# ictnlp/StreamSpeech

Measured on AMD Instinct MI355X. Metric: real-time factor (RTFx = audio seconds / wall seconds) + utterances/sec, offline S2ST fr-en, higher is better.
Workload: dtype f32

## Files before the change

include/streamspeech_hip.h:

```cpp
#ifndef STREAMSPEECH_HIP_H
#define STREAMSPEECH_HIP_H

#include <stddef.h>
#include <stdint.h>

#ifdef __cplusplus
extern "C" {
#endif

#define SS_ABI_VERSION 2

typedef struct ss_model ss_model;
typedef struct ss_vocoder ss_vocoder;
typedef struct ss_scratch ss_scratch;
typedef struct ss_stream_pool ss_stream_pool;

typedef struct ss_config {
  int32_t input_feat, conv_channels, conv_kernel;
  int32_t enc_dim, enc_ffn, enc_heads, enc_layers, dw_kernel;
  int32_t src_vocab, tgt_vocab;
  int32_t mt_layers, dec_dim, dec_ffn, dec_heads;
  int32_t t2u_layers, unit_layers, unit_vocab, ctc_upsample;
  int32_t pad, eos, unk;
  int32_t max_rel_pos;
// ... 106 lines not shown
  int32_t history;
  int32_t dst;
  int32_t pad0;
} ss_mp3_stream_seg;

int ss_mp3_stream_synthesize(void* stream, const int16_t* d_q, const ss_mp3_granule* d_rec, int64_t n_rec,
                             const ss_mp3_stream_seg* h_segs, int n_segs, float* const* h_state, float* const* h_dst,
                             const int64_t* h_dst_cap, int n_dst, int mono, void* d_work, size_t* work_bytes);

typedef struct ss_flac_info {
  int32_t sample_rate, channels, bits_per_sample;
  int32_t frames;
  int64_t subframes;
  int64_t samples;
  int64_t total_samples;
  int32_t min_block, max_block;
  uint8_t md5[16];
} ss_flac_info;

enum { SS_FLAC_CONSTANT = 0, SS_FLAC_VERBATIM = 1, SS_FLAC_FIXED = 2, SS_FLAC_LPC = 3 };
enum { SS_FLAC_INDEPENDENT = 0, SS_FLAC_LEFT_SIDE = 1, SS_FLAC_RIGHT_SIDE = 2, SS_FLAC_MID_SIDE = 3 };

typedef struct ss_flac_subframe {
  int64_t res_offset;
  int64_t sample_start;
  int32_t block_size;
  uint8_t type;
  uint8_t order;
  uint8_t bps;
  uint8_t wasted;
  uint8_t shift;
  uint8_t assignment;
  uint8_t precision;
  uint8_t channel;
  int32_t reserved;
  int16_t coef[32];
} ss_flac_subframe;

typedef struct ss_flac_file {
  int64_t rec_offset;
  int64_t out_offset;
  int32_t frames;
  int32_t channels;
  int32_t bps;
  int32_t n_out;
} ss_flac_file;

int ss_flac_streaminfo(const uint8_t* h_data, size_t n_bytes, ss_flac_info* h_info);
int ss_flac_probe(const uint8_t* h_data, size_t n_bytes, ss_flac_info* h_info);
int ss_flac_unpack(const uint8_t* h_data, size_t n_bytes, int64_t cap, int32_t* h_res, ss_flac_subframe* h_rec, int64_t res_cap,
                   ss_flac_info* h_info);
int ss_flac_restore_host(const int32_t* h_res, const ss_flac_subframe* h_rec, int64_t n_rec, const ss_flac_file* h_files, int n_files,
                         int mono, float* h_out, int32_t* h_pcm);
int ss_flac_restore(void* stream, const int32_t* d_res, const ss_flac_subframe* d_rec, int64_t n_rec, int64_t n_res,
                    const ss_flac_file* h_files, int n_files, int mono, float* d_out, int64_t out_floats,
                    void* d_work, size_t* work_bytes);

enum { SS_PCM_F32LE = 0, SS_PCM_S16LE = 1, SS_PCM_ULAW = 2, SS_PCM_ALAW = 3 };

typedef struct ss_pcm_seg {
  int64_t src_offset;
  int64_t dst_offset;
  int32_t frames;
  int32_t fmt, channels, dst;
} ss_pcm_seg;

int ss_pcm_scatter(void* stream, const void* d_stage, int64_t stage_bytes, const ss_pcm_seg* h_segs, int n_segs,
                   float* const* h_dst, const int64_t* h_dst_cap, int n_dst);
int ss_pcm_pack_s16(void* stream, const float* d_src, int64_t n, int16_t* d_out);
int ss_pcm_decode_host(const void* h_src, int fmt, int channels, int64_t frames, float* h_dst);
int ss_pcm_pack_s16_host(const float* h_src, int64_t n, int16_t* h_out);

typedef struct ss_pcm_emit_seg {
  float* carry;
  const float* tail;
  const float* taps;
  int64_t n_before;
  int64_t k0, k1;
  int64_t out_offset;
  int32_t carry_len;
  int32_t n_new;
  int32_t up, down, half;
  int32_t fmt;
  int32_t finished;
  int32_t reserved;
} ss_pcm_emit_seg;

int64_t ss_pcm_emit_count(int64_t n, int up, int down, int half, int finished);
int ss_pcm_emit(void* stream, const ss_pcm_emit_seg* h_segs, int n_segs, void* d_out, int64_t out_bytes);
int ss_pcm_emit_host(const ss_pcm_emit_seg* h_segs, int n_segs, void* h_out, int64_t out_bytes);
int ss_pcm_encode_host(const float* h_src, int64_t n, int fmt, void* h_out);

enum { SS_VAD_IDLE = 0, SS_VAD_SPEECH = 1 };
enum { SS_VAD_START = 1, SS_VAD_END = 2, SS_VAD_FORCED = 4 };

typedef struct ss_vad_state {
  int64_t onset;
  int64_t last_speech;
  int64_t utt_first_frame;
  float floor;
  int32_t mode;
  int32_t run;
  int32_t reserved;
} ss_vad_state;

typedef struct ss_vad_seg {
  const float* hist;
  ss_vad_state* state;
  float* powers;
  int64_t hist_first;
  int64_t n_hist;
  int64_t first_frame;
  int32_t n_frames;
  int32_t H, W;
  float p_abs, p_min, snr, rise;
  int32_t min_speech, end_silence, post_roll, max_frames;
  int32_t reserved;
} ss_vad_seg;

typedef struct ss_vad_result {
  int64_t consumed;
  int64_t start_frame;
  int64_t cut_sample;
  int64_t last_speech;
  int32_t events;
  int32_t mode;
} ss_vad_result;

int ss_vad_scan(void* stream, const ss_vad_seg* h_segs, int n_segs, ss_vad_result* d_results);
int ss_vad_scan_host(const ss_vad_seg* h_segs, int n_segs, ss_vad_result* h_results);

int ss_row_max_logprob(void* stream, const float* d_logits, int rows, int vocab, int mask0, int mask1, int mask2,
                       float* d_out);

int ss_log_softmax(void* stream, const float* d_logits, int rows, int vocab, int mask0, int mask1, int as_probs,
                   float* d_out);

int ss_encoder_out_len(int T);
int ss_encoder_forward(ss_model* m, void* stream, const float* d_fbank, int T, int attn_chunk,
                       int conv_chunk, float* d_enc_out);

int ss_encoder_stream_reset(ss_model* m);
int ss_encoder_stream_set_tail(ss_model* m, int unsettled_fbank_frames);
int ss_encoder_stream_forward(ss_model* m, void* stream, const float* d_fbank, int T, int attn_chunk,
                              int conv_chunk, float* d_enc_out, int32_t* n_final, int32_t* n_computed);
int ss_encoder_stream_set_deferred(ss_model* m, int on);
int ss_encoder_stream_status(ss_model* m, void* stream, int32_t* repeat);

int ss_stream_pool_create(ss_model* m, int max_sessions, int max_rows, ss_stream_pool** out);
void ss_stream_pool_destroy(ss_stream_pool* p);
int ss_stream_pool_reset(ss_stream_pool* p, int slot);
int ss_stream_pool_set_tail(ss_stream_pool* p, int slot, int unsettled_fbank_frames);
int ss_encoder_stream_forward_batch(ss_model* m, void* stream, ss_stream_pool* p, int n, const int32_t* h_slots,
                                    const float* const* h_fbank, const int32_t* h_T, const int32_t* h_attn_chunk,
                                    const int32_t* h_conv_chunk, float* d_enc_packed, int32_t* h_n_final, int32_t* h_n_computed);
int ss_stream_pool_ctc(ss_model* m, void* stream, ss_stream_pool* p, int head, int n, const int32_t* h_slots,
                       const float* d_enc_packed, int32_t* d_raw, int32_t* d_tokens, int32_t* d_index, int32_t* d_counts);
int ss_stream_pool_stats(ss_stream_pool* p, int64_t* launches, int64_t* head_rows);

int ss_ctc_greedy(ss_model* m, void* stream, int head, const float* d_enc_out, int Tp,
                  int32_t* d_raw, int32_t* d_tokens, int32_t* d_index, int32_t* d_count,
                  float* d_logits);

int ss_mt_set_persistent(ss_model* m, int workgroups);
int ss_mt_get_persistent(ss_model* m);

int ss_mt_begin(ss_model* m, void* stream, const float* d_enc_out, int Tp);
int ss_mt_append(ss_model* m, void* stream, const int32_t* d_tokens, int n, int pos0, int ban_eos,
                 int force_eos, float* d_feats, int32_t* d_next, int n_tail_pad);
int ss_mt_greedy(ss_model* m, void* stream, const float* d_enc_out, int Tp, const int32_t* h_prefix,
                 int n_prefix, int max_len, int min_len, int32_t* h_out_tokens, int* h_n_out,
                 float* d_feats, int* h_n_feats);
int ss_mt_truncate(ss_model* m, int len);

int ss_t2u_units(ss_model* m, void* stream, const float* d_mt_feats, int n, int t2u_causal,
                 int mask_eos, int32_t* d_raw, int32_t* d_tokens, int32_t* d_count, float* d_logits,
                 int n_tail_pad);

int ss_vocoder_create(const ss_vocoder_config* cfg, const float* d_blob, size_t blob_floats,
                      const char* const* names, const int64_t* offsets, const int64_t* numels,
                      int n_slots, ss_vocoder** out);
void ss_vocoder_destroy(ss_vocoder* v);
int ss_vocoder_set_bf16x3(ss_vocoder* v, int on);
int ss_vocoder_set_f16(ss_vocoder* v, int on);
int ss_vocoder_forward(ss_vocoder* v, void* stream, const int32_t* d_codes, int K, int dur_prediction,
                       const int32_t* d_forced_dur, float* d_wav, int64_t wav_capacity,
                       int32_t* d_dur, int64_t* h_n_samples);
int ss_vocoder_num_speakers(const ss_vocoder* v);
int ss_vocoder_forward_spkr(ss_vocoder* v, void* stream, const int32_t* d_codes, int K, int dur_prediction,
                            const int32_t* d_forced_dur, float* d_wav, int64_t wav_capacity,
                            int32_t* d_dur, int64_t* h_n_samples, int32_t spkr);

int ss_batch_fbank_cmvn(ss_model* m, void* stream, int B, const float* d_pcm, const int64_t* h_pcm_start,
                        const int32_t* h_n_samples, float pcm_scale, float* d_feat, int32_t* h_T);
int ss_batch_cmvn(ss_model* m, void* stream, const float* d_in, int64_t rows, float* d_out);
int ss_batch_encoder_forward(ss_model* m, void* stream, int B, const float* d_fbank, const int32_t* h_T,
                             int attn_chunk, int conv_chunk, float* d_enc_out, int32_t* h_Tp);
int ss_batch_ctc_greedy(ss_model* m, void* stream, int head, int B, const float* d_enc_out,
                        const int32_t* h_Tp, int32_t* d_raw, int32_t* d_tokens, int32_t* d_index,
                        int32_t* d_counts);
int ss_batch_mt_greedy(ss_model* m, void* stream, int B, const float* d_enc_out, const int32_t* h_Tp,
                       const int32_t* h_max_len, int min_len, int32_t* h_out_tokens, int out_stride,
                       int32_t* h_n_out, float* d_feats, int feat_rows);
int ss_batch_mt_beam(ss_model* m, void* stream, int B, int beam, const float* d_enc_out, const int32_t* h_Tp,
                     const int32_t* h_max_len, int min_len, float unk_penalty, int normalize, int32_t* h_out_tokens,
                     int out_stride, int32_t* h_n_out, float* h_scores, float* h_pos_scores, float* d_feats, int feat_rows);
int ss_batch_mt_continue(ss_model* m, void* stream, int B, const float* d_enc_out, const int32_t* h_Tp, const int32_t* h_prefix,
                         const int32_t* h_n_prefix, const int32_t* h_max_len, int min_len, int32_t* h_out_tokens, int out_stride,
                         int32_t* h_n_out, float* d_feats, int feat_rows, int32_t* h_n_feats);
int ss_batch_mt_continue_plan(int B, const int32_t* h_Tp, const int32_t* h_prefix, const int32_t* h_n_prefix, const int32_t* h_max_len,
                              int min_len, int out_stride, int feat_rows, int max_tgt_pos, int vocab, int eos, int32_t* h_dims,
                              int32_t* h_tables, int64_t tables_cap, int64_t* h_n_tables);
int ss_batch_mt_beam_continue(ss_model* m, void* stream, int B, int beam, const float* d_enc_out, const int32_t* h_Tp,
                              const int32_t* h_prefix, const int32_t* h_n_prefix, const int32_t* h_max_len, int min_len,
                              float unk_penalty, int normalize, int32_t* h_out_tokens, int out_stride, int32_t* h_n_out,
                              float* h_scores, float* h_pos_scores, float* d_feats, int feat_rows);
int ss_batch_mt_beam_continue_plan(int B, int beam, const int32_t* h_Tp, const int32_t* h_prefix, const int32_t* h_n_prefix,
                                   const int32_t* h_max_len, int min_len, int out_stride, int feat_rows, int max_tgt_pos, int vocab,
                                   int eos, int pad, int32_t* h_dims, int32_t* h_tables, int64_t tables_cap, int64_t* h_n_tables);
int ss_batch_fbank_frames(ss_model* m, void* stream, int B, const float* const* h_pcm, const int32_t* h_first, const int32_t* h_n,
                          float pcm_scale, float* const* h_feat);
int ss_batch_fbank_frames_sr(ss_model* m, void* stream, int B, const float* const* h_pcm, const int32_t* h_n_in, const int32_t* h_up,
                             const int32_t* h_down, const float* const* h_taps, const int32_t* h_half_len, const int32_t* h_first,
                             const int32_t* h_n, float pcm_scale, float* const* h_feat);
int ss_fbank_sr_rows(int64_t n_in, int up, int down, int half_len, int32_t* h_n_rows, int32_t* h_n_final);
int ss_batch_t2u_units(ss_model* m, void* stream, int B, const float* d_feats, int feat_rows,
                       const int32_t* h_n, int t2u_causal, int mask_eos, int32_t* d_raw, int32_t* d_tokens,
                       int32_t* d_counts);
int ss_batch_vocoder_forward(ss_vocoder* v, void* stream, int B, const int32_t* d_codes, const int32_t* h_K,
                             int dur_prediction, const int32_t* d_forced_dur, float* d_wav,
                             int64_t wav_capacity, int32_t* d_dur, int64_t* h_wav_start,
                             int64_t* h_n_samples);
int ss_batch_vocoder_forward_spkr(ss_vocoder* v, void* stream, int B, const int32_t* d_codes, const int32_t* h_K,
                                  int dur_prediction, const int32_t* d_forced_dur, float* d_wav,
                                  int64_t wav_capacity, int32_t* d_dur, int64_t* h_wav_start,
                                  int64_t* h_n_samples, const int32_t* h_spkr );
int ss_batch_t2u_units_pad(ss_model* m, void* stream, int B, const float* d_feats, int feat_rows, const int32_t* h_n,
                           const int32_t* h_n_tail_pad, int t2u_causal, int mask_eos, int32_t* d_raw, int32_t* d_tokens,
                           int32_t* d_counts);
int ss_batch_mt_features(ss_model* m, void* stream, int B, const float* d_enc_out, const int32_t* h_Tp, const int32_t* h_tokens,
                         const int32_t* h_n_tokens, const int32_t* h_n_tail_pad, float* d_feats, int feat_rows);
int ss_batch_vocoder_tail(ss_vocoder* v, void* stream, int B, const int32_t* d_codes, const int32_t* h_K, const int32_t* h_n_new,
                          const int32_t* h_ctx, const int32_t* h_rf, int dur_prediction, float* d_out, int64_t out_capacity,
                          int32_t* h_win_first, int32_t* h_dur, int64_t* h_out_start, int64_t* h_n_out);
int ss_batch_vocoder_tail_spkr(ss_vocoder* v, void* stream, int B, const int32_t* d_codes, const int32_t* h_K, const int32_t* h_n_new,
                               const int32_t* h_ctx, const int32_t* h_rf, int dur_prediction, float* d_out, int64_t out_capacity,
                               int32_t* h_win_first, int32_t* h_dur, int64_t* h_out_start, int64_t* h_n_out,
                               const int32_t* h_spkr );

int ss_prof_enable(int cls_mask);
int ss_prof_enable_hi(int cls_mask);
int ss_prof_reset(void);
int ss_prof_read(int cls, double* h_ms_total, double* h_flops_total, int64_t* h_launches,
                 double* h_bytes_total);
int ss_prof_totals(int cls, double* h_flops_total, double* h_bytes_total, int64_t* h_launches);
int ss_prof_read_issued(int cls, double* h_issued_flops_total);
int ss_prof_shape_log(int on);
int ss_prof_shape_dump(char* buf, int cap);
int ss_prof_num_classes(void);
const char* ss_prof_class_name(int cls);

int ss_model_set_pack_invariant(ss_model* m, int on);
int ss_model_get_pack_invariant(ss_model* m);
int ss_debug_canon(int mode);

int ss_debug_last_logits(ss_model* m, void* stream, float* d_out, int64_t cap_floats, int* h_rows, int* h_cols);

int ss_op_ffn_fused(void* stream, const float* dX, int ldx, float* dY, int ldy, const float* ln_g, const float* ln_b,
                    const float* dW1, const float* db1, const float* dW2, const float* db2, float alpha,
                    const float* ln2_g, const float* ln2_b, int M, int D, int F);
int ss_debug_ffn(int grid, int row_tiles_per_wave, int enable);
int ss_debug_rtlin(int grid, int enable);
int ss_debug_conv_c64(int enable);
int ss_debug_conv_c32(int enable);
int ss_debug_conv_c16(int enable);
int64_t ss_debug_enc_step_launches(void);
int ss_op_ln_linear(void* stream, const float* dX, int ldx, const float* ln_g, const float* ln_b, const float* dW,
                    const float* dbias, const float* dR, int ldr, float* dC, int ldc, int M, int N, int K, int act, float alpha,
                    int glu);

int ss_debug_force_tile(int bm, int bn, int ks);
int ss_debug_sk_errors(void);
int ss_debug_attention_split(int v);
int ss_debug_attention_q16(int v);
int ss_debug_enc_step_inject_timeout(ss_model* m);
int ss_debug_scratch_audit(ss_scratch* sc, size_t* booked, size_t* held);
int ss_debug_mt_inject_timeout(ss_model* m);

int ss_op_conv_gemm(void* stream, const float* dA, int lda, const float* dW, const float* dbias,
                    const float* dR, int ldr, const float* dR2, int ldr2, float* dC, int ldc,
                    int M, int N, int Cin, int taps, int dil, int stride, int pad, int in_len,
                    int chunk, int in_act, float in_slope, int act, float alpha, float div, int glu);
typedef struct ss_op_conv_args {
  const float* A; const float* W; const float* bias; const float* R; const float* R2; float* C; float* C2;
  int32_t lda, ldc, ldr, ldr2, ldc2;
  int32_t M, N, Cin, taps, dil, stride, pad, in_len, chunk;
  int32_t in_act; float in_slope;
  int32_t act; float act_slope, alpha, div, c2_slope;
  int32_t glu;
  const int32_t* segs; int32_t nseg, max_seg_out;
  int32_t same_rows;
} ss_op_conv_args;
int ss_op_conv_gemm_ex(void* stream, const ss_op_conv_args* a);
int ss_op_conv_pair(void* stream, const float* dA, int lda, const float* dW1, const float* db1, const float* dW2, const float* db2,
                    float* dC, int ldc, const float* dR2, int ldr2, float div, float* dC2, int ldc2, float c2_slope, int C, int taps,
                    int dil, int M, int in_len, float slope, const int32_t* d_segs, int nseg);
int ss_op_resblock_fused(void* stream, const float* dX, int ldx, const float* const* dW1, const float* const* dB1,
                         const float* const* dW2, const float* const* dB2, const int32_t* dil, float* dY, int ldy, const float* dR2,
                         int ldr2, float div, int C, int taps, int M, float slope, const int32_t* d_segs, int nseg);
int ss_debug_slab(int grid, long long min_rows);
int ss_op_conv_f16(void* stream, const float* dA, const float* dW, const float* dbias, const float* dR, const float* dR2,
                   float* dC, float* dC2, int M, int C, int taps, int dil, int in_act, float in_slope, int act, float div,
                   const int32_t* d_segs, int nseg);
int ss_op_layernorm(void* stream, const float* dx, int ldx, float* dy, int ldy, const float* dg,
                    const float* db, int M, int D, float eps);
int ss_op_attention(void* stream, const float* dQ, int ldq, const float* dK, int ldk, const float* dV,
                    int ldv, float* dO, int ldo, int Tq, int Tk, int H, float scale, int causal,
                    int chunk, const float* dP, int ldp, const float* du, const float* dv);
typedef struct ss_op_attn_args {
  const float* Q; const float* K; const float* V; float* O;
  int32_t ldq, ldk, ldv, ldo;
  int32_t Tq, Tk, H;
  float scale;
  int32_t causal, chunk, q0, k_mask_tail;
  const float* P; int32_t ldp;
  const float* bias_u; const float* bias_v;
  const int32_t* segs; int32_t nseg, max_q, p_tmax;
  const int32_t* seg_tail;
  int32_t no_decode_kernel;
  const int32_t* anc; int32_t anc_ld, anc_slots;
  int32_t use_split;
} ss_op_attn_args;
int ss_op_attention_ex(void* stream, const ss_op_attn_args* a);
typedef struct ss_op_pool_attn_args {
  const float* Qs; float* cache; float* O;
  int32_t ld, ldo, slot_rows;
  const float* P; int32_t ldp, p_tmax;
  const float* bias_u; const float* bias_v;
  const int32_t* sess; const int32_t* qt_pre;
  int32_t nsess, qtiles, H;
  float scale;
} ss_op_pool_attn_args;
int ss_op_attention_pool(void* stream, const ss_op_pool_attn_args* a);
int ss_debug_attention_no_mfma(int v);
int ss_op_dwconv_bn_silu(void* stream, const float* dx, int ldx, float* dy, int ldy, const float* dwt,
                         int K, const float* mean, const float* var, const float* gamma,
                         const float* beta, float eps, int T, int C, int chunk);

int ss_op_masked_argmax(void* stream, const float* logits, int ld, int M, int N, int mask0, int mask1, int mask2, int force,
                        int32_t* ids, const int32_t* row_max_len, int step, int force_id, const int32_t* row_min_len, int ban_id);
int ss_op_ctc_collapse(void* stream, const int32_t* raw, int T, int blank, int pad, int32_t* tokens, int32_t* index, int32_t* count,
                       const int32_t* segs, int nseg);
int ss_op_dur_predict(void* stream, const float* logdur, const int32_t* forced, int K, int32_t* dur, int32_t* cum,
                      const int32_t* segs, int nseg);
int ss_op_repeat_rows(void* stream, const float* emb, const int32_t* cum, int K, int D, float* out, int F, const int32_t* segs,
                      int nseg);
int ss_op_embed_tokens(void* stream, const int32_t* tok, const float* emb, const float* pos_table, float scale, int pos0, float* out,
                       int n, int D, int pos_stride, int pad_id, int vocab);
int ss_op_embed_tokens_rows(void* stream, const int32_t* tok, const float* emb, const float* pos_table, int pos_rows, float scale,
                            int pos0, const int32_t* row_pos, float* out, int n, int D, int pad_id, int vocab);
int ss_op_upsample_add_pos(void* stream, const float* src, int n, int up, const float* pos_row, float pad_value, float* out, int D);
int ss_op_gather_rows(void* stream, const int32_t* idx, const float* table, int D, float* out, int n, int rows);
int ss_op_scatter_rows(void* stream, const int32_t* dst_row, const float* src, int lds, float* dst, int ldd, int D, int n,
                       int dst_rows);
int ss_op_conv_post_tanh(void* stream, const float* x, int T, int C, const float* w, const float* bias, float slope, float* wav,
                         const int32_t* segs, int nseg);
int ss_op_conv_post_tanh_crop(void* stream, const float* x, int C, const float* w, const float* bias, float slope, float* wav,
                              const int32_t* segs, int nseg, int max_keep);
int ss_op_spkr_pre_add(void* stream, const float* x, float* y, int ld, int C0, const float* table, const int32_t* spkr, int spkr0,
                       const int32_t* segs, int nseg, int max_seg_out, int M, int act, float slope);

#define SS_OP_BEAM_CAND 64
int ss_op_beam_topk(void* stream, const float* logits, int R, int V, int k, int t_step, int min_len, const int32_t* max_len,
                    const int32_t* npre, const int32_t* done, const float* cum, int pad, int unk, int eos, float unk_pen,
                    float* cand_s, int32_t* cand_t);
typedef struct ss_op_beam_state {
  int32_t* tok; float* cum; int32_t* anc; float* cand_s; int32_t* cand_t; int32_t* ignore; int32_t* done; int32_t* max_len;
  int32_t* npre;
  int32_t* fin_cnt; float* fin_score; int32_t* fin_len; int32_t* fin_tok; float* fin_pos; int32_t* fin_anc;
} ss_op_beam_state;
int ss_op_beam_merge(void* stream, const ss_op_beam_state* st, int B, int k, int Lc, int V, int t_step, int c0, int eos,
                     int normalize);
int ss_op_beam_prefix_score(void* stream, const float* logits, int rows, int V, const int32_t* ftok, int pad, int unk, float unk_pen,
                            float* lp);
int ss_op_beam_prefix_chain(void* stream, const float* lp, const int32_t* row0, const int32_t* npre, int B, int k, float* cum0,
                            float* pos);

#ifdef __cplusplus
}
#endif
#endif
```

streamspeech_amd/csrc/conv_c64w.hip:

```cpp
#include "slab_common.hpp"

#include <type_traits>

namespace ss {

using u32x4 = __attribute__((ext_vector_type(4))) unsigned;

#ifndef CW_TIMING
#define CW_TIMING 0
#endif
#if CW_TIMING
__device__ unsigned long long g_cw_dbg[1024 * 8];
#define CW_STAMP(k) do { if (t == 0) { const unsigned long long _n = __builtin_amdgcn_s_memtime(); cw_acc[k] += _n - cw_last; cw_last = _n; } } while (0)
#else
#define CW_STAMP(k) do { } while (0)
#endif

namespace {
constexpr int CW_MAXSEG = 256;
constexpr int CW_MAXROWS = 320;
[[maybe_unused]] constexpr int CW_NUM_RECORDS = 0x7ffffff0;
constexpr int cw_bme(int dil) { return dil == 1 ? 256 : dil == 3 ? 252 : 240; }
[[maybe_unused]] __host__ __device__ constexpr int cw_nc(int kind) { return kind == 0 ? 4 : kind == 1 ? 2 : 3; }
[[maybe_unused]] __host__ __device__ constexpr int cw_slot(int kind, int n) { return kind == 0 ? n : kind == 1 ? (n == 0 ? 0 : 3) : (n == 2 ? 3 : n); }
[[maybe_unused]] __host__ __device__ constexpr int cw_ja(int kind, int n) { return kind == 0 ? (n == 3 ? 1 : n) : kind == 1 ? n : (n == 0 ? 0 : 1); }
[[maybe_unused]] __host__ __device__ constexpr int cw_jb(int kind, int n) { return kind == 0 ? (n == 2 ? 1 : n == 3 ? 3 : 2) : kind == 1 ? n : (n == 2 ? 2 : 1); }
[[maybe_unused]] __host__ __device__ constexpr int cw_op(int kind, int n) { return kind == 0 ? (n == 1 ? 1 : -1) : kind == 1 ? 0 : (n == 1 ? 0 : -1); }
}

__global__ void wino_pack_kernel(const float* __restrict__ W, float* __restrict__ WW, int C, int taps, int groups) {
  const int n = C * groups * C;
  for (int idx = blockIdx.x * blockDim.x + threadIdx.x; idx < n; idx += gridDim.x * blockDim.x) {
    const int ci = idx % C, g = (idx / C) % groups, co = idx / (C * groups);
    const float* w = W + (size_t)co * taps * C + ci;
    const float w0 = 3 * g < taps ? w[(size_t)(3 * g) * C] : 0.f;
    const float w1 = 3 * g + 1 < taps ? w[(size_t)(3 * g + 1) * C] : 0.f;
    const float w2 = 3 * g + 2 < taps ? w[(size_t)(3 * g + 2) * C] : 0.f;
    float* o = WW + (size_t)co * groups * 4 * C + (size_t)g * 4 * C + ci;
    const int left = taps - 3 * g;
    if (left >= 3) {
      o[0] = w0;
      o[C] = 0.5f * ((w0 + w1) + w2);
      o[2 * C] = 0.5f * ((w0 - w1) + w2);
      o[3 * C] = w2;
    } else if (left == 2) {
      o[0] = w0; o[C] = w0 + w1; o[2 * C] = 0.f; o[3 * C] = w1;
    } else {
      o[0] = w0; o[C] = 0.f; o[2 * C] = 0.f; o[3 * C] = -w0;
    }
  }
}

template <int DIL, int CH, int TAIL>
__global__ __launch_bounds__(CH >= 128 ? 512 : 256, CH >= 128 ? 1 : CH == 64 ? 2 : 3) void conv_c64w_kernel(const GemmArgs p, const int groups, const int slab_rows) {
#if __HIP_DEVICE_COMPILE__
  constexpr int CS = CH == 256 ? 128 : CH;
  constexpr int KH = CH / CS;
  constexpr int C = CH, LDA = CS + 4, CT = CH >= 64 ? 4 : CH / 16, CB = CS / 16, RING = 2 * CT, TPR = CS / 4;
  constexpr int NT = CH >= 128 ? 512 : 256, RPP = NT / TPR;
  constexpr int NP = (CW_MAXROWS + RPP - 1) / RPP, NPC = CH == 256 ? 10 : NP < 20 ? NP : 20, BME = cw_bme(DIL), NPAIR = BME / 2;
  extern __shared__ __attribute__((aligned(16))) float smem[];
  float* sA = smem;
  int* s_blk = reinterpret_cast<int*>(smem + ((slab_rows * LDA + 3) & ~3));

  const int t = threadIdx.x, lane = t & 63;
  const int wave = __builtin_amdgcn_readfirstlane((t >> 6) & 3);
  const int cs = CH <= 64 ? 0 : __builtin_amdgcn_readfirstlane(t >> 8);
  const int colh = CH == 256 ? (int)((blockIdx.x >> 3) & 1) : 0;
  const int col0 = colh * 128 + cs * 64;
  const int r = lane & 15, g = lane >> 4;
  const int Kw = groups * 4 * C;

  SlabWalk<GemmArgs> w(p, s_blk, BME);
  __syncthreads();
  const int nblocks = w.nblocks();
  const float slope = p.in_act == ACT_LRELU ? p.in_slope : 1.0f;

  const __amdgpu_buffer_rsrc_t rsW = __builtin_amdgcn_make_buffer_rsrc((void*)p.W, 0, CW_NUM_RECORDS, 0x00020000);
  const int vo = (r * Kw + 4 * g) * 4;
  auto wload = [&](int idx, int cc, int ct, int kh) -> f32x4 {
    const int so = __builtin_amdgcn_readfirstlane(((col0 + ct * 16) * Kw + idx * C + kh * CS + cc * 16) * 4);
    const u32x4 v = __builtin_amdgcn_raw_buffer_load_b128(rsW, vo, so, 0);
    return f32x4{__uint_as_float(v[0]), __uint_as_float(v[1]), __uint_as_float(v[2]), __uint_as_float(v[3])};
  };

  int blk = CH == 256 ? (int)((blockIdx.x & 7) + 8 * (blockIdx.x >> 4)) : (int)blockIdx.x;
  const int blk_stride = CH == 256 ? (int)(gridDim.x >> 1) : (int)gridDim.x;
  if (blk >= nblocks) return;
  f32x4 ring[RING];
#pragma unroll
  for (int q = 0; q < RING; ++q) ring[q] = wload(q / CT, 0, q % CT, 0);

  int toff[2];
  bool pv[2];
#pragma unroll
  for (int i = 0; i < 2; ++i) {
    const int pp = wave * 32 + i * 16 + r;
    pv[i] = pp < NPAIR;
    const int pc = pv[i] ? pp : NPAIR - 1;
    toff[i] = 2 * DIL * (pc / DIL) + pc % DIL;
  }

#if CW_TIMING
  unsigned long long cw_acc[4] = {0, 0, 0, 0}, cw_last = __builtin_amdgcn_s_memtime(), cw_begin = cw_last, cw_blocks = 0;
#endif
  for (; blk < nblocks; blk += blk_stride) {
#if CW_TIMING
    ++cw_blocks;
#endif
    w.locate(blk, p.in_len);
    const int m0 = w.m0, seg_lo = w.seg_lo, seg_hi = w.seg_hi;
    const int m_hi = p.nseg > 0 ? seg_hi : min(seg_hi, p.M);
    const bool edge = (m0 - p.pad < seg_lo) || (m0 - p.pad + slab_rows > seg_hi);
    f32x4 acc[4][2][CT];
#pragma unroll
    for (int f = 0; f < 4; ++f)
#pragma unroll
      for (int i = 0; i < 2; ++i)
#pragma unroll
        for (int j = 0; j < CT; ++j) acc[f][i][j] = f32x4{0.f, 0.f, 0.f, 0.f};
#pragma unroll 1
    for (int kh = 0; kh < KH; ++kh) {
    const int kh_wrap = kh + 1 < KH ? kh + 1 : 0;
    __syncthreads();
    CW_STAMP(kh == 0 ? 3 : 1);
#pragma unroll 1
    for (int u0 = 0; u0 < NP; u0 += NPC) {
      f32x4 pre[NPC];
#pragma unroll
      for (int u = 0; u < NPC; ++u) {
        const int rho = t / TPR + RPP * (u0 + u);
        const int gc = min(max(m0 - p.pad + rho, seg_lo), seg_hi - 1);
        pre[u] = *reinterpret_cast<const f32x4*>(p.A + (size_t)gc * p.lda + kh * CS + (t % TPR) * 4);
      }
      float* dst = sA + (t / TPR + RPP * u0) * LDA + (t % TPR) * 4;
#pragma unroll
      for (int u = 0; u < NPC; ++u) {
        const int rho = t / TPR + RPP * (u0 + u);
        f32x4 v = pre[u];
        if (edge) {
          const int gin = m0 - p.pad + rho;
          const bool ok = gin >= seg_lo && gin < seg_hi;
#pragma unroll
          for (int e = 0; e < 4; ++e) v[e] = ok ? v[e] : 0.f;
        }
#pragma unroll
        for (int e = 0; e < 4; ++e) v[e] = fmaxf(v[e], v[e] * slope);
        if (rho < slab_rows) *reinterpret_cast<f32x4*>(dst + u * RPP * LDA) = v;
      }
    }
    __syncthreads();
    CW_STAMP(0);

    const float* pa0 = sA + toff[0] * LDA + 4 * g;
    const float* pa1 = sA + toff[1] * LDA + 4 * g;
    auto rd = [&](const float* base, int j, int cc) -> f32x4 { return *reinterpret_cast<const f32x4*>(base + j * DIL * LDA + cc * 16); };
    auto xform = [&](int op, const f32x4 a, const f32x4 b) -> f32x4 { return op == 1 ? a + b : op == 0 ? a : a - b; };
    f32x4 xa[2];
    xa[0] = xform(-1, rd(pa0, 0, 0), rd(pa0, 2, 0));
    xa[1] = xform(-1, rd(pa1, 0, 0), rd(pa1, 2, 0));
    auto group = [&](auto KIND, const int grp, const int kind_next, const float* pn0, const float* pn1, const int grp_next, const int kh_next) __attribute__((always_inline)) {
      constexpr int K = decltype(KIND)::value, NC = cw_nc(K), NS = CB * NC;
      static_assert(NS % 2 == 0 && NS >= 2, "ring slots keep their parity across groups");
#pragma unroll
      for (int ss = 0; ss < NS; ++ss) {
        const int slot = cw_slot(K, ss % NC);
        f32x4 na0, nb0, na1, nb1;
        if (ss + 1 < NS) {
          const int ccn = (ss + 1) / NC, nn = (ss + 1) % NC;
          na0 = rd(pa0, cw_ja(K, nn), ccn); nb0 = rd(pa0, cw_jb(K, nn), ccn);
          na1 = rd(pa1, cw_ja(K, nn), ccn); nb1 = rd(pa1, cw_jb(K, nn), ccn);
        } else {
          const int jb = kind_next == 0 ? 2 : 1;
          na0 = rd(pn0, 0, 0); nb0 = *reinterpret_cast<const f32x4*>(pn0 + jb * (DIL * LDA));
          na1 = rd(pn1, 0, 0); nb1 = *reinterpret_cast<const f32x4*>(pn1 + jb * (DIL * LDA));
        }
        f32x4 wf[CT];
#pragma unroll
        for (int j = 0; j < CT; ++j) {
          const int q = ss * CT + j;
          wf[j] = ring[q % RING];
          const int s2 = ss + 2;
          if (s2 < NS) ring[q % RING] = wload(grp * 4 + cw_slot(K, s2 % NC), s2 / NC, j, kh);
          else ring[q % RING] = wload(grp_next * 4 + (s2 == NS ? 0 : (kind_next == 1 ? 3 : 1)), 0, j, kh_next);
        }
#pragma unroll
        for (int e = 0; e < 4; ++e)
#pragma unroll
          for (int i = 0; i < 2; ++i)
#pragma unroll
            for (int j = 0; j < CT; ++j)
              acc[slot][i][j] = __builtin_amdgcn_mfma_f32_16x16x4f32(wf[j][e], xa[i][e], acc[slot][i][j], 0, 0, 0);
        if (ss + 1 < NS) {
          xa[0] = xform(cw_op(K, (ss + 1) % NC), na0, nb0);
          xa[1] = xform(cw_op(K, (ss + 1) % NC), na1, nb1);
        } else {
          xa[0] = kind_next == 1 ? na0 : na0 - nb0;
          xa[1] = kind_next == 1 ? na1 : na1 - nb1;
        }
        __builtin_amdgcn_sched_barrier(0);
      }
    };
    constexpr int tail = TAIL;
    const int groups_full = groups - (tail ? 1 : 0);
#pragma unroll 1
    for (int grp = 0; grp < groups_full; ++grp) {
      const bool more = grp + 1 < groups;
      const float* pn0 = more ? pa0 + 3 * DIL * LDA : pa0;
      const float* pn1 = more ? pa1 + 3 * DIL * LDA : pa1;
      group(std::integral_constant<int, 0>{}, grp, (more && grp + 1 == groups_full) ? tail : 0, pn0, pn1, more ? grp + 1 : 0, more ? kh : kh_wrap);
      pa0 = pn0;
      pa1 = pn1;
    }
    if constexpr (TAIL == 1) group(std::integral_constant<int, 1>{}, groups_full, 0, pa0, pa1, 0, kh_wrap);
    if constexpr (TAIL == 2) group(std::integral_constant<int, 2>{}, groups_full, 0, pa0, pa1, 0, kh_wrap);
    CW_STAMP(1);
    }

    int le = lane;
    asm volatile("" : "+v"(le));
    const int g_e = le >> 4;
    const int cole = col0 + g_e * 4;
    f32x4 y[4 * CT];
    int mrow[4];
#pragma unroll
    for (int i = 0; i < 2; ++i) {
#pragma unroll
      for (int j = 0; j < CT; ++j) {
        y[(i * 2) * CT + j] = (acc[0][i][j] + acc[1][i][j]) + acc[2][i][j];
        y[(i * 2 + 1) * CT + j] = (acc[1][i][j] - acc[2][i][j]) - acc[3][i][j];
      }
      mrow[i * 2] = m0 + toff[i];
      mrow[i * 2 + 1] = m0 + toff[i] + DIL;
    }
#pragma unroll
    for (int n = 0; n < 4 * CT; ++n) asm volatile("" : "+v"(y[n]));
    f32x4 bb[CT];
#pragma unroll
    for (int j = 0; j < CT; ++j) bb[j] = f32x4{0.f, 0.f, 0.f, 0.f};
    if (p.bias) {
#pragma unroll
      for (int j = 0; j < CT; ++j) bb[j] = *reinterpret_cast<const f32x4*>(p.bias + cole + j * 16);
    }
    slab_epi_batch(p, y, bb, [&](int q, int n) -> size_t {
      return (size_t)min(mrow[n / CT], m_hi - 1) * (q == 0 ? p.ldr : p.ldr2) + cole + (n % CT) * 16;
    });
#pragma unroll
    for (int q = 0; q < 4; ++q) {
      if (pv[q / 2] && mrow[q] < m_hi) {
#pragma unroll
        for (int j = 0; j < CT; ++j) slab_epi_store<CH >= 128>(p, mrow[q], cole + j * 16, y[q * CT + j]);
      }
    }
    CW_STAMP(2);
  }
#if CW_TIMING
  if (t == 0) {
    unsigned long long* d = g_cw_dbg + (size_t)(blockIdx.x & 1023) * 8;
    d[0] = cw_acc[0]; d[1] = cw_acc[1]; d[2] = cw_acc[2]; d[3] = cw_acc[3]; d[4] = cw_blocks; d[5] = cw_begin; d[6] = __builtin_amdgcn_s_memtime(); d[7] = 1;
  }
#endif
#endif
}

#if CW_TIMING
extern "C" int ss_debug_cw_timing(unsigned long long* h_out, int cap_wgs) {
  const int n = cap_wgs < 1024 ? cap_wgs : 1024;
  if (hipMemcpyFromSymbol(h_out, HIP_SYMBOL(g_cw_dbg), (size_t)n * 8 * sizeof(unsigned long long)) != hipSuccess) return -1;
  static unsigned long long zeros[1024 * 8];
  (void)hipMemcpyToSymbol(HIP_SYMBOL(g_cw_dbg), zeros, sizeof(zeros));
  return n;
}
#endif

void conv_c64w_debug(int enable) { if (enable >= 0) dispatch_edit([enable](Dispatch& d) { d.c64w_on = enable ? 1 : 0; }); }
bool conv_c64w_enabled() { return disp().c64w_on != 0; }
void conv_c128w_debug(int enable) { if (enable >= 0) dispatch_edit([enable](Dispatch& d) { d.c128w_on = enable ? 1 : 0; }); }
bool conv_c128w_enabled() { return disp().c128w_on != 0; }

void conv_c256w_debug(int enable) { if (enable >= 0) dispatch_edit([enable](Dispatch& d) { d.c256w_on = enable ? 1 : 0; }); }
bool conv_c256w_enabled() { return disp().c256w_on != 0; }

static int cw_groups(const GemmArgs& a) { return (a.taps + 2) / 3; }
static size_t cw_lds(const GemmArgs& a, int ch) { return slab_lds_bytes(cw_bme(a.dil) + 3 * cw_groups(a) * a.dil, ch + 4, CW_MAXSEG); }

bool conv_c64w_eligible(const GemmArgs& a) {
  if (!disp().c64w_on || !a.Wwino || a.taps < disp().c64w_min_k || a.taps < 3 || (a.dil != 1 && a.dil != 3 && a.dil != 5) || a.C2) return false;
  if (a.pad != a.dil * (a.taps - 1) / 2) return false;
  if (a.taps <= 8 && a.taps > 3 && a.dil == 5) return false;
  const int slab_rows = cw_bme(a.dil) + 3 * cw_groups(a) * a.dil;
  return slab_rows <= CW_MAXROWS && 2 * cw_lds(a, 64) <= 158 * 1024 && (size_t)cw_groups(a) * 4 * 64 * 64 * 4 < 0x7ff00000ull;
}

bool conv_wide_winograd_eligible(const GemmArgs& a, int ch) {
  if (ch != 128 && ch != 256) return false;
  const Dispatch& d = disp();
  if (!(ch == 128 ? d.c128w_on : d.c256w_on) || !a.Wwino || !slab_conv_ok(a, ch)) return false;
  if (a.taps < 3 || (a.dil != 1 && a.dil != 3 && a.dil != 5) || a.pad != a.dil * (a.taps - 1) / 2) return false;
  if (a.nseg > CW_MAXSEG || a.M < (ch == 128 ? d.c128w_min_rows : d.c256w_min_rows) || !slab_rows_ok(a.M)) return false;
  if (ch == 256 && (size_t)256 * cw_groups(a) * 4 * 256 * 4 >= 0x7ff00000ull) return false;
  const int slab_rows = cw_bme(a.dil) + 3 * cw_groups(a) * a.dil;
  return slab_rows <= CW_MAXROWS && cw_lds(a, 128) <= 160 * 1024;
}

int launch_wino_pack(const float* W, float* WW, int C, int taps, hipStream_t stream) {
  const int groups = (taps + 2) / 3, n = C * groups * C;
  hipLaunchKernelGGL(wino_pack_kernel, dim3((n + 255) / 256), dim3(256), 0, stream, W, WW, C, taps, groups);
  SS_LAUNCH_CHECK();
  return SS_OK;
}

template <int DIL, int CH, int TAIL>
static int launch_cw_t(GemmArgs a, hipStream_t stream) {
  constexpr int BME = cw_bme(DIL);
  const int groups = cw_groups(a);
  const int slab_rows = BME + 3 * groups * DIL;
  const size_t lds = cw_lds(a, CH == 256 ? 128 : CH);
  SS_MAX_LDS_ONCE((&conv_c64w_kernel<DIL, CH, TAIL>), CH >= 128 ? 160 * 1024 : 96 * 1024);
  SkWorkspace* st = nullptr;
  int rc = sk_workspace_acquire(stream, &st);
  if (rc != SS_OK) return rc;
  int grid = slab_grid(CH >= 128 ? 1 : CH == 64 ? 2 : 3, st->cus, a.M, BME, a.nseg);
  if (CH == 256) {
    long long want = std::min<long long>(st->cus, 2 * ((slab_max_blocks(a.M, BME, a.nseg) + 7) / 8 * 8));
    if (disp().slab_grid_cap > 0) want = std::min<long long>(want, disp().slab_grid_cap);
    grid = (int)std::max<long long>(16, want / 16 * 16);
  }
  ProfRec rec{}; bool prof = false;
  rc = prof_begin(a, stream, CH == 64 ? PROF_CONV_C64W : CH == 128 ? PROF_CONV_C128W : CH == 256 ? PROF_CONV_C256W : PROF_CONV_C32W, rec, prof);
  if (rc != SS_OK) return rc;
  a.W = a.Wwino;
  hipLaunchKernelGGL((conv_c64w_kernel<DIL, CH, TAIL>), dim3(grid), dim3(CH >= 128 ? 512 : 256), lds, stream, a, groups, slab_rows);
  SS_LAUNCH_CHECK();
  return prof_end(stream, rec, prof);
}

template <int CH>
static int launch_cw(const GemmArgs& a, hipStream_t stream) {
  if (a.in_act != ACT_NONE && a.in_act != ACT_LRELU) return SS_ERR_ARG;
  const int key = a.dil * 10 + a.taps % 3;
  switch (key) {
    case 10: return launch_cw_t<1, CH, 0>(a, stream);
    case 11: return launch_cw_t<1, CH, 1>(a, stream);
    case 12: return launch_cw_t<1, CH, 2>(a, stream);
    case 30: return launch_cw_t<3, CH, 0>(a, stream);
    case 31: return launch_cw_t<3, CH, 1>(a, stream);
    case 32: return launch_cw_t<3, CH, 2>(a, stream);
    case 50: return launch_cw_t<5, CH, 0>(a, stream);
    case 51: return launch_cw_t<5, CH, 1>(a, stream);
    case 52: return launch_cw_t<5, CH, 2>(a, stream);
    default: return SS_ERR_ARG;
  }
}

int launch_conv_c64w(const GemmArgs& a, hipStream_t stream) {
  if (!conv_c64_eligible(a) || !conv_c64w_eligible(a)) return SS_ERR_ARG;
  return launch_cw<64>(a, stream);
}
void conv_c32w_debug(int enable) { if (enable >= 0) dispatch_edit([enable](Dispatch& d) { d.c32w_on = enable ? 1 : 0; }); }
bool conv_c32w_enabled() { return disp().c32w_on != 0; }
bool conv_c32w_eligible(const GemmArgs& a) {
  if (!disp().c32w_on || !a.Wwino || a.taps < 3 || (a.dil != 1 && a.dil != 3 && a.dil != 5) || a.C2) return false;
  if (a.pad != a.dil * (a.taps - 1) / 2) return false;
  const int slab_rows = cw_bme(a.dil) + 3 * cw_groups(a) * a.dil;
  return slab_rows <= CW_MAXROWS && 3 * cw_lds(a, 32) <= 158 * 1024;
}
int launch_conv_c32w(const GemmArgs& a, hipStream_t stream) {
  if (!conv_c32_eligible(a) || !conv_c32w_eligible(a)) return SS_ERR_ARG;
  return launch_cw<32>(a, stream);
}
int launch_conv_c128w(const GemmArgs& a, hipStream_t stream) {
  if (!conv_wide_winograd_eligible(a, 128)) return SS_ERR_ARG;
  return launch_cw<128>(a, stream);
}
int launch_conv_c256w(const GemmArgs& a, hipStream_t stream) {
  if (!conv_wide_winograd_eligible(a, 256)) return SS_ERR_ARG;
  return launch_cw<256>(a, stream);
}

}
```

streamspeech_amd/csrc/debug_ops.hip:

```cpp
#include "model_internal.hpp"

static int op_bind_wino(GemmArgs& a, void* stream) {
  static thread_local std::map<hipStream_t, DevBuf> wino_tmps;
  DevBuf& wino_tmp = wino_tmps[(hipStream_t)stream];
  const int N = a.N, Cin = a.Cin, taps = a.taps;
  if ((conv_c64w_enabled() && N == 64 && Cin == 64 && taps >= 3 && conv_c64_eligible(a)) ||
      (conv_c128w_enabled() && N == 128 && Cin == 128 && taps >= 3 && a.same_rows && !a.glu) ||
      (conv_c256w_enabled() && N == 256 && Cin == 256 && taps >= 3 && a.same_rows && !a.glu) ||
      (conv_c32w_enabled() && N == 32 && Cin == 32 && taps >= 3 && conv_c32_eligible(a))) {
    RET(wino_tmp.ensure((size_t)N * ((taps + 2) / 3) * 4 * N * sizeof(float)));
    RET(launch_wino_pack(a.W, wino_tmp.f(), N, taps, (hipStream_t)stream));
    a.Wwino = wino_tmp.f();
  }
  return SS_OK;
}

extern "C" int ss_op_conv_gemm(void* stream, const float* dA, int lda, const float* dW, const float* dbias,
                               const float* dR, int ldr, const float* dR2, int ldr2, float* dC, int ldc, int M,
                               int N, int Cin, int taps, int dil, int stride, int pad, int in_len, int chunk,
                               int in_act, float in_slope, int act, float alpha, float div, int glu) {
  GemmArgs a;
  a.A = dA; a.lda = lda; a.W = dW; a.bias = dbias; a.R = dR; a.ldr = ldr; a.R2 = dR2; a.ldr2 = ldr2; a.C = dC; a.ldc = ldc;
  a.M = M; a.N = N; a.Cin = Cin; a.taps = taps; a.dil = dil; a.stride = stride; a.pad = pad; a.in_len = in_len;
  a.chunk = chunk; a.in_act = in_act; a.in_slope = in_slope; a.act = act; a.alpha = alpha; a.div = div; a.glu = glu;
  a.same_rows = (stride == 1 && M == in_len) ? 1 : 0;
  RET(op_bind_wino(a, stream));
  return launch_conv_gemm(a, (hipStream_t)stream);
}

extern "C" int ss_op_conv_gemm_ex(void* stream, const ss_op_conv_args* x) {
  if (!x) return SS_ERR_ARG;
  GemmArgs a;
  a.A = x->A; a.W = x->W; a.bias = x->bias; a.R = x->R; a.R2 = x->R2; a.C = x->C; a.C2 = x->C2;
  a.lda = x->lda; a.ldc = x->ldc; a.ldr = x->ldr; a.ldr2 = x->ldr2; a.ldc2 = x->ldc2;
  a.M = x->M; a.N = x->N; a.Cin = x->Cin; a.taps = x->taps; a.dil = x->dil; a.stride = x->stride; a.pad = x->pad;
  a.in_len = x->in_len; a.chunk = x->chunk;
  a.in_act = x->in_act; a.in_slope = x->in_slope; a.act = x->act; a.act_slope = x->act_slope; a.alpha = x->alpha; a.div = x->div;
  a.c2_slope = x->c2_slope; a.glu = x->glu;
  a.segs = x->segs; a.nseg = x->nseg; a.max_seg_out = x->max_seg_out; a.same_rows = x->same_rows;
  if (a.W && a.N > 0 && a.taps > 0) RET(op_bind_wino(a, stream));
  return launch_conv_gemm(a, (hipStream_t)stream);
}
extern "C" int ss_op_conv_pair(void* stream, const float* dA, int lda, const float* dW1, const float* db1, const float* dW2,
                               const float* db2, float* dC, int ldc, const float* dR2, int ldr2, float div, float* dC2, int ldc2,
                               float c2_slope, int Cch, int taps, int dil, int M, int in_len, float slope, const int32_t* d_segs,
                               int nseg) {
  return launch_conv_pair(dA, lda, dW1, db1, dW2, db2, dC, ldc, dR2, ldr2, div, dC2, ldc2, c2_slope, Cch, taps, dil, M, in_len, slope,
                          d_segs, nseg, (hipStream_t)stream);
}
extern "C" int ss_op_resblock_fused(void* stream, const float* dX, int ldx, const float* const* dW1, const float* const* dB1,
                                    const float* const* dW2, const float* const* dB2, const int32_t* dil, float* dY, int ldy,
                                    const float* dR2, int ldr2, float div, int Cch, int taps, int M, float slope,
                                    const int32_t* d_segs, int nseg) {
  if (!dW1 || !dB1 || !dW2 || !dB2 || !dil) return SS_ERR_ARG;
  return launch_resblock_fused(dX, ldx, dW1, dB1, dW2, dB2, dil, dY, ldy, dR2, ldr2, div, Cch, taps, M, slope, d_segs, nseg,
                               (hipStream_t)stream);
}
extern "C" int ss_debug_slab(int grid, long long min_rows) {
  if (grid < 0) return SS_ERR_ARG;
  slab_debug(grid, min_rows);
  return SS_OK;
}

extern "C" int ss_op_conv_f16(void* stream, const float* dA, const float* dW, const float* dbias, const float* dR, const float* dR2,
                              float* dC, float* dC2, int M, int Cch, int taps, int dil, int in_act, float in_slope, int act, float div,
                              const int32_t* d_segs, int nseg) {
  if (!dA || !dW || !dC || M <= 0 || taps < 1 || dil < 1 || nseg < 0 || (nseg > 0 && !d_segs)) return SS_ERR_ARG;
  if (!(Cch == 64 || Cch == 128 || Cch == 256)) return SS_ERR_ARG;
  static thread_local std::map<hipStream_t, DevBuf> f16_tmps;
  DevBuf& wh = f16_tmps[(hipStream_t)stream];
  RET(wh.ensure(f16_pack_halves(Cch, taps) * sizeof(uint16_t)));
  RET(launch_f16_pack(dW, wh.p, Cch, taps, (hipStream_t)stream));
  GemmArgs a;
  a.A = dA; a.lda = Cch; a.W = dW; a.Wf16 = wh.p; a.bias = dbias; a.R = dR; a.ldr = Cch; a.R2 = dR2; a.ldr2 = Cch;
  a.C = dC; a.ldc = Cch; a.C2 = dC2; a.ldc2 = Cch; a.c2_slope = 0.1f;
  a.M = M; a.N = Cch; a.Cin = Cch; a.taps = taps; a.dil = dil; a.stride = 1; a.pad = dil * (taps - 1) / 2; a.in_len = M;
  a.same_rows = 1; a.in_act = in_act; a.in_slope = in_slope; a.act = act; a.act_slope = 0.1f; a.div = div;
  a.segs = d_segs; a.nseg = nseg;
  return launch_conv_f16(a, (hipStream_t)stream);
}

extern "C" int ss_debug_last_logits(ss_model* m, void* stream, float* d_out, int64_t cap_floats, int* h_rows, int* h_cols) {
  if (!m || !h_rows || !h_cols) return SS_ERR_ARG;
  *h_rows = m->sc->dbg_rows; *h_cols = m->sc->dbg_cols;
  if (!d_out) return SS_OK;
  if (!m->sc->dbg_logits || cap_floats < (int64_t)m->sc->dbg_rows * m->sc->dbg_cols) return SS_ERR_CAPACITY;
  SS_HIP_CHECK(hipMemcpyAsync(d_out, m->sc->dbg_logits, (size_t)m->sc->dbg_rows * m->sc->dbg_cols * sizeof(float), hipMemcpyDeviceToDevice,
                              (hipStream_t)stream));
  return SS_OK;
}

extern "C" int ss_op_ffn_fused(void* stream, const float* dX, int ldx, float* dY, int ldy, const float* ln_g, const float* ln_b,
                               const float* dW1, const float* db1, const float* dW2, const float* db2, float alpha,
                               const float* ln2_g, const float* ln2_b, int M, int D, int F) {
  return launch_ffn_fused(dX, ldx, dY, ldy, ln_g, ln_b, dW1, db1, dW2, db2, alpha, ln2_g, ln2_b, M, D, F, (hipStream_t)stream,
                          canon_mode() == CANON_SEQ);
}
extern "C" int ss_debug_canon(int mode) {
  if (mode < 0 || mode > 2) return SS_ERR_ARG;
  canon_debug_set(mode);
  return SS_OK;
}
extern "C" int ss_op_ln_linear(void* stream, const float* dX, int ldx, const float* ln_g, const float* ln_b, const float* dW,
                               const float* dbias, const float* dR, int ldr, float* dC, int ldc, int M, int N, int K, int act,
                               float alpha, int glu) {
  GemmArgs a;
  a.A = dX; a.lda = ldx; a.W = dW; a.bias = dbias; a.R = dR; a.ldr = ldr; a.C = dC; a.ldc = ldc;
  a.M = M; a.N = N; a.Cin = K; a.in_len = M; a.act = act; a.alpha = alpha; a.glu = glu; a.same_rows = 1;
  a.ln_g = ln_g; a.ln_b = ln_b;
  return launch_conv_gemm(a, (hipStream_t)stream);
}
extern "C" int ss_debug_conv_c64(int enable) {
  if (enable == 4 || enable == 5) { conv_c64w_debug(enable == 5); return SS_OK; }
  if (enable == 6 || enable == 7) { conv_c128w_debug(enable == 7); return SS_OK; }
  if (enable == 8 || enable == 9) { conv_c256w_debug(enable == 9); return SS_OK; }
  conv_c64_debug(enable);
  return SS_OK;
}
extern "C" int ss_debug_conv_c32(int enable) {
  if (enable == 4 || enable == 5) { conv_c32w_debug(enable == 5); return SS_OK; }
  conv_c32_debug(enable);
  return SS_OK;
}
extern "C" int ss_debug_conv_c16(int enable) { conv_c16_debug(enable); return SS_OK; }
extern "C" int64_t ss_debug_enc_step_launches(void) { return (int64_t)enc_step_launch_count(); }
extern "C" int ss_debug_scratch_audit(ss_scratch* sc, size_t* booked, size_t* held) {
  if (!sc || !booked || !held) return SS_ERR_ARG;
  size_t sum = 0;
  bool foreign = false;
  for (DevBuf* b : sc->all()) {
    sum += b->bytes;
    if (b->acct != &sc->acct) foreign = true;
  }
  *booked = sc->acct.used;
  *held = sum;
  return foreign ? SS_ERR_ARG : SS_OK;
}
extern "C" int ss_debug_rtlin(int grid, int enable) {
  if (grid < 0) return SS_ERR_ARG;
  rtlin_debug(grid, enable);
  return SS_OK;
}
extern "C" int ss_debug_ffn(int grid, int row_tiles_per_wave, int enable) {
  if (grid < 0 || row_tiles_per_wave < -1 || row_tiles_per_wave > 4) return SS_ERR_ARG;
  ffn_fused_debug_grid(grid);
  ffn_fused_debug_rows(row_tiles_per_wave);
  if (enable >= 0) dispatch_edit([enable](Dispatch& d) { d.ffn_fusion = enable ? 1 : 0; });
  return SS_OK;
}

extern "C" int ss_op_layernorm(void* stream, const float* dx, int ldx, float* dy, int ldy, const float* dg,
                               const float* db, int M, int D, float eps) {
  return launch_layernorm(dx, ldx, dy, ldy, dg, db, M, D, eps, (hipStream_t)stream);
}

extern "C" int ss_op_masked_argmax(void* stream, const float* logits, int ld, int M, int N, int mask0, int mask1, int mask2, int force,
                                   int32_t* ids, const int32_t* row_max_len, int step, int force_id, const int32_t* row_min_len,
                                   int ban_id) {
  return launch_masked_argmax(logits, ld, M, N, mask0, mask1, mask2, force, ids, (hipStream_t)stream, row_max_len, step, force_id,
                              row_min_len, ban_id);
}
extern "C" int ss_op_ctc_collapse(void* stream, const int32_t* raw, int T, int blank, int pad, int32_t* tokens, int32_t* index,
                                  int32_t* count, const int32_t* segs, int nseg) {
  return launch_ctc_collapse(raw, T, blank, pad, tokens, index, count, (hipStream_t)stream, segs, nseg);
}
extern "C" int ss_op_dur_predict(void* stream, const float* logdur, const int32_t* forced, int K, int32_t* dur, int32_t* cum,
                                 const int32_t* segs, int nseg) {
  return launch_dur_predict(logdur, forced, K, dur, cum, (hipStream_t)stream, segs, nseg);
}
extern "C" int ss_op_repeat_rows(void* stream, const float* emb, const int32_t* cum, int K, int D, float* out, int F,
                                 const int32_t* segs, int nseg) {
  return launch_repeat_rows(emb, cum, K, D, out, F, (hipStream_t)stream, segs, nseg);
}
extern "C" int ss_op_embed_tokens(void* stream, const int32_t* tok, const float* emb, const float* pos_table, float scale, int pos0,
                                  float* out, int n, int D, int pos_stride, int pad_id, int vocab) {
  return launch_embed_tokens(tok, emb, pos_table, scale, pos0, out, n, D, (hipStream_t)stream, pos_stride, pad_id, vocab);
}
extern "C" int ss_op_embed_tokens_rows(void* stream, const int32_t* tok, const float* emb, const float* pos_table, int pos_rows,
                                       float scale, int pos0, const int32_t* row_pos, float* out, int n, int D, int pad_id, int vocab) {
  return launch_embed_tokens_rows(tok, emb, pos_table, pos_rows, scale, pos0, row_pos, out, n, D, (hipStream_t)stream, pad_id, vocab);
}
extern "C" int ss_op_upsample_add_pos(void* stream, const float* src, int n, int up, const float* pos_row, float pad_value, float* out,
                                      int D) {
  return launch_upsample_add_pos(src, n, up, pos_row, pad_value, out, D, (hipStream_t)stream);
}
extern "C" int ss_op_gather_rows(void* stream, const int32_t* idx, const float* table, int D, float* out, int n, int rows) {
  return launch_gather_rows(idx, table, D, out, n, (hipStream_t)stream, rows);
}
extern "C" int ss_op_scatter_rows(void* stream, const int32_t* dst_row, const float* src, int lds, float* dst, int ldd, int D, int n,
                                  int dst_rows) {
  return launch_scatter_rows(dst_row, src, lds, dst, ldd, D, n, dst_rows, (hipStream_t)stream);
}
extern "C" int ss_op_conv_post_tanh(void* stream, const float* x, int T, int C, const float* w, const float* bias, float slope,
                                    float* wav, const int32_t* segs, int nseg) {
  return launch_conv_post_tanh(x, T, C, w, bias, slope, wav, (hipStream_t)stream, segs, nseg);
}
extern "C" int ss_op_conv_post_tanh_crop(void* stream, const float* x, int C, const float* w, const float* bias, float slope, float* wav,
                                         const int32_t* segs, int nseg, int max_keep) {
  return launch_conv_post_tanh_crop(x, C, w, bias, slope, wav, segs, nseg, max_keep, (hipStream_t)stream);
}
extern "C" int ss_op_spkr_pre_add(void* stream, const float* x, float* y, int ld, int C0, const float* table, const int32_t* spkr,
                                   int spkr0, const int32_t* segs, int nseg, int max_seg_out, int M, int act, float slope) {
  return launch_spkr_pre_add(x, y, ld, C0, table, spkr, spkr0, segs, nseg, max_seg_out, M, act, slope, (hipStream_t)stream);
}

static int op_attn_bind_split(AttnArgs& a) {
  static void* scratch = nullptr;
  if (!scratch) {
    SS_HIP_CHECK(hipMalloc(&scratch, attention_split_bytes()));
    SS_HIP_CHECK(hipMemset(scratch, 0, attention_split_bytes()));
  }
  attention_bind_split(a, scratch);
  return SS_OK;
}

extern "C" int ss_op_attention(void* stream, const float* dQ, int ldq, const float* dK, int ldk, const float* dV,
                               int ldv, float* dO, int ldo, int Tq, int Tk, int H, float scale, int causal, int chunk,
                               const float* dP, int ldp, const float* du, const float* dv) {
  AttnArgs a;
  a.Q = dQ; a.ldq = ldq; a.K = dK; a.ldk = ldk; a.V = dV; a.ldv = ldv; a.O = dO; a.ldo = ldo;
  a.Tq = Tq; a.Tk = Tk; a.H = H; a.scale = scale; a.causal = causal; a.chunk = chunk;
  a.P = dP; a.ldp = ldp; a.bias_u = du; a.bias_v = dv;
  if (dP) RET(op_attn_bind_split(a));
  return launch_attention(a, (hipStream_t)stream);
}

extern "C" int ss_op_attention_ex(void* stream, const ss_op_attn_args* x) {
  if (!x) return SS_ERR_ARG;
  AttnArgs a;
  a.Q = x->Q; a.K = x->K; a.V = x->V; a.O = x->O;
  a.ldq = x->ldq; a.ldk = x->ldk; a.ldv = x->ldv; a.ldo = x->ldo;
  a.Tq = x->Tq; a.Tk = x->Tk; a.H = x->H; a.scale = x->scale;
  a.causal = x->causal; a.chunk = x->chunk; a.q0 = x->q0; a.k_mask_tail = x->k_mask_tail;
  a.P = x->P; a.ldp = x->ldp; a.bias_u = x->bias_u; a.bias_v = x->bias_v;
  a.segs = x->segs; a.nseg = x->nseg; a.max_q = x->max_q; a.p_tmax = x->p_tmax;
  a.seg_tail = x->seg_tail;
  a.no_decode_kernel = x->no_decode_kernel;
  a.anc = x->anc; a.anc_ld = x->anc_ld; a.anc_slots = x->anc_slots;
  if (x->use_split) RET(op_attn_bind_split(a));
  return launch_attention(a, (hipStream_t)stream);
}

extern "C" int ss_op_attention_pool(void* stream, const ss_op_pool_attn_args* x) {
  if (!x) return SS_ERR_ARG;
  PoolAttnArgs a;
  a.Qs = x->Qs; a.cache = x->cache; a.O = x->O;
  a.ld = x->ld; a.ldo = x->ldo; a.slot_rows = x->slot_rows;
  a.P = x->P; a.ldp = x->ldp; a.p_tmax = x->p_tmax;
  a.bias_u = x->bias_u; a.bias_v = x->bias_v;
  a.sess = x->sess; a.qt_pre = x->qt_pre;
  a.nsess = x->nsess; a.qtiles = x->qtiles; a.H = x->H; a.scale = x->scale;
  return launch_attention_pool(a, (hipStream_t)stream);
}

extern "C" int ss_debug_attention_split(int v) { attention_debug_split(v); return SS_OK; }
extern "C" int ss_debug_attention_q16(int v) { attention_debug_q16(v); return SS_OK; }
extern "C" int ss_debug_attention_no_mfma(int v) { attention_debug_no_mfma(v); return SS_OK; }

extern "C" int ss_op_dwconv_bn_silu(void* stream, const float* dx, int ldx, float* dy, int ldy, const float* dwt,
                                    int K, const float* mean, const float* var, const float* gamma,
                                    const float* beta, float eps, int T, int C, int chunk) {
  return launch_dwconv_bn_silu(dx, ldx, dy, ldy, dwt, K, mean, var, gamma, beta, eps, T, C, chunk, (hipStream_t)stream);
}

extern "C" int ss_prof_enable(int cls_mask) { prof_enable(cls_mask); return SS_OK; }
extern "C" int ss_prof_enable_hi(int cls_mask) { prof_enable_hi(cls_mask); return SS_OK; }
extern "C" int ss_prof_reset(void) { prof_reset(); return SS_OK; }
extern "C" int ss_prof_read(int cls, double* ms, double* flops, int64_t* launches, double* bytes) {
  long long n = 0;
  int rc = prof_read(cls, ms, flops, &n, bytes);
  if (launches) *launches = n;
  return rc;
}
extern "C" int ss_prof_totals(int cls, double* flops, double* bytes, int64_t* launches) {
  long long n = 0;
  int rc = prof_totals(cls, flops, bytes, &n);
  if (launches) *launches = n;
  return rc;
}
extern "C" int ss_prof_read_issued(int cls, double* issued_flops) { return prof_read_issued(cls, issued_flops); }
extern "C" int ss_prof_shape_log(int on) { prof_shape_log(on); return SS_OK; }
extern "C" int ss_prof_shape_dump(char* buf, int cap) { return prof_shape_dump(buf, cap); }
extern "C" int ss_prof_num_classes(void) { return kNumTileCfg; }
extern "C" const char* ss_prof_class_name(int cls) { return prof_cfg_name(cls); }

extern "C" int ss_debug_force_tile(int bm, int bn, int ks) {
  if (!(bm >= 0 && bm <= 6) && bm != 32 && bm != 64 && bm != 128) return SS_ERR_ARG;
  if (bm == 6 || bm == 0) dispatch_edit([bm](Dispatch& d) { d.no_resblock_fusion = (bm == 6); });
  if (bm == 3 || bm == 0) dispatch_edit([bm](Dispatch& d) { d.no_pair_fusion = (bm == 3); });
  debug_force_tile((bm == 3 || bm == 6) ? 0 : bm, bn, ks);
  return SS_OK;
}
extern "C" int ss_debug_sk_errors(void) { return conv_sk_error_count() + conv_sk2_error_count() + g_mt_timeouts.load(std::memory_order_relaxed); }
```

streamspeech_amd/csrc/dispatch.hpp:

```cpp
#pragma once
#include <functional>

namespace ss {

struct Dispatch {
  int attn_no_mfma = 0;
  int attn_q16 = 1;
  int attn_split = 0;
  int c16_off = 0, c32_off = 0, c64_off = 0;
  long long c16_min_rows = 131072, c32_min_rows = 65536, c64_min_rows = 32768;
  int c64w_on = 1, c128w_on = 1, c256w_on = 1, c32w_on = 1;
  int c64w_min_k = 3;
  long long c128w_min_rows = 65536, c256w_min_rows = 32768;
  int slab_grid_cap = 0;
  int sk_groups = 0;
  int ffn_force_g = 0;
  int ffn_wm = 3, ffn_wm_forced = 0;
  int ffn_fusion = 1;
  int ffn_min_rows = 1000;
  int force_bm = 0, force_bn = 0, force_ks = 0;
  double sk_min_flops = 4e9;
  int no_resblock_fusion = 0, no_pair_fusion = 0;
  int rt_off = 0, rt_min_rows = 193, rt_force_g = 0;
  long long rt_min_units = 4000;
  long long rt_kb_min_units = 256;
  int rt_kb_xmap = 1;
  int rt_kb_uw = 0;
};

const Dispatch& disp();
void dispatch_edit(const std::function<void(Dispatch&)>& fn);

struct CtxDispatch {
  Dispatch d;
  unsigned gen = 0xffffffffu;
  const Dispatch* refresh();
};
struct DispatchScope {
  explicit DispatchScope(const Dispatch* d);
  ~DispatchScope();
  const Dispatch* prev;
};

}
```

streamspeech_amd/csrc/gemm.hip:

```cpp
#include "gemm.hpp"

#include <atomic>
#include <cstdio>
#include <cstdlib>
#include <cstring>
#include <map>
#include <string>
#include <mutex>
#include <tuple>
#include <type_traits>
#include <utility>
#include <vector>

namespace ss {

using f32x4 = __attribute__((ext_vector_type(4))) float;

template <int BM, int BN, int BK, int WM, int WN, int KS, int PD, bool BLK = false>
__global__ __launch_bounds__(256 * KS) void conv_gemm_kernel(const GemmArgs p) {
  static_assert(WM * WN == 4, "4 waves per k-group");
  static_assert(!BLK || KS == 1, "the blocked chain is the KS = 1 form");
  constexpr int LDK = BK + 8;
  constexpr int WTM = BM / WM, WTN = BN / WN;
  constexpr int TM = WTM / 16, TN = WTN / 16;
// ... 490 lines not shown
      float sm = 0.f;
#pragma unroll
      for (int it = 0; it < 8; ++it) {
        xv[it] = f32x4{0.f, 0.f, 0.f, 0.f};
        if (it * 256 < K) xv[it] = *reinterpret_cast<const f32x4*>(xrow + it * 256 + 4 * lane);
        sm += (xv[it][0] + xv[it][1]) + (xv[it][2] + xv[it][3]);
      }
      mean = wave_sum(sm) / (float)K;
      float q = 0.f;
#pragma unroll
      for (int it = 0; it < 8; ++it)
        if (it * 256 < K) {
#pragma unroll
          for (int e = 0; e < 4; ++e) { const float d = xv[it][e] - mean; q += d * d; }
        }
      rstd = 1.0f / sqrtf(wave_sum(q) / (float)K + 1e-5f);
    }
    float a0 = 0.f, a1 = 0.f, a2 = 0.f, a3 = 0.f;
#pragma unroll
    for (int it = 0; it < 8; ++it)
      if (it < nit) {
        f32x4 x = *reinterpret_cast<const f32x4*>(xrow + k0 + it * 256 + 4 * lane);
        if (LNORM) {
          const f32x4 gm = *reinterpret_cast<const f32x4*>(p.ln_g + k0 + it * 256 + 4 * lane);
          const f32x4 bt = *reinterpret_cast<const f32x4*>(p.ln_b + k0 + it * 256 + 4 * lane);
#pragma unroll
          for (int e = 0; e < 4; ++e) x[e] = (x[e] - mean) * rstd * gm[e] + bt[e];
          if (p.ln_out && blockIdx.x == 0 && wave < KS)
            *reinterpret_cast<f32x4*>(p.ln_out + (size_t)m * K + k0 + it * 256 + 4 * lane) = x;
        }
        a0 = fmaf(x[0], wv[it][0], a0); a1 = fmaf(x[1], wv[it][1], a1);
        a2 = fmaf(x[2], wv[it][2], a2); a3 = fmaf(x[3], wv[it][3], a3);
      }
    acc[m] = wave_sum((a0 + a1) + (a2 + a3));
  }
  if (KS > 1) {
    if (lane == 0) {
#pragma unroll
      for (int m = 0; m < MR; ++m) part[wave][m] = acc[m];
    }
    __syncthreads();
    if (ks != 0) return;
#pragma unroll
    for (int m = 0; m < MR; ++m)
#pragma unroll
      for (int s2 = 1; s2 < KS; ++s2) acc[m] += part[wave + s2][m];
  }
  if (lane != 0 || !col_ok) return;
  const float b = p.bias ? p.bias[col] : 0.f;
#pragma unroll
  for (int m = 0; m < MR; ++m) {
    if (m >= p.M) continue;
    float v = acc[m] + b;
    switch (p.act) {
      case ACT_SILU: v = v / (1.0f + expf(-v)); break;
      case ACT_RELU: v = fmaxf(v, 0.f); break;
      default: break;
    }
    v *= p.alpha;
    if (p.R) v += p.R[(size_t)m * p.ldr + col];
    p.C[(size_t)m * p.ldc + col] = v;
  }
}

bool gemv_eligible(const GemmArgs& a) {
  return smallm_eligible(a) && !a.glu && a.M <= 4 && a.Cin % 256 == 0 && a.Cin <= 2048;
}

template <int KS>
static int launch_gemv_ks(const GemmArgs& a, hipStream_t stream) {
  dim3 grid(cdiv(a.N, 4 / KS));
  ProfRec rec{}; bool prof = false;
  int rc = prof_begin(a, stream, PROF_SMALLM_4x1, rec, prof);
  if (rc != SS_OK) return rc;
  if (a.ln_g) hipLaunchKernelGGL((gemv_kernel<4, KS, true>), grid, dim3(256), 0, stream, a);
  else hipLaunchKernelGGL((gemv_kernel<4, KS, false>), grid, dim3(256), 0, stream, a);
  SS_LAUNCH_CHECK();
  return prof_end(stream, rec, prof);
}

static int launch_gemv(const GemmArgs& a, hipStream_t stream) {
  const int kq = a.Cin / 256;
  if (a.N * 1 >= 2048 || kq % 2 != 0) return launch_gemv_ks<1>(a, stream);
  if (a.N * 2 >= 2048 || kq % 4 != 0) return launch_gemv_ks<2>(a, stream);
  return launch_gemv_ks<4>(a, stream);
}

static const char* kTileNames[] = {
    "conv_gemm<128,16,16,4,1>", "conv_gemm<128,32,32,4,1>", "conv_gemm<128,32,16,4,1>", "conv_gemm<16,128,32,1,4>",
    "conv_gemm<16,128,16,1,4>", "conv_gemm<128,128,16,2,2>", "conv_gemm<128,64,32,2,2>", "conv_gemm<64,64,32,2,2>",
    "conv_gemm<64,64,16,2,2>", "conv_gemm<32,64,32,2,2>", "conv_gemm<32,64,16,2,2>", "conv_gemm<32,32,32,2,2>",
    "smallm_gemm<4,1>", "smallm_gemm<2,2>", "smallm_gemm<1,4>", "conv_sk<128,BN,32>",
    "conv_slab<32>", "conv_slab<16>", "conv_sk2<256,128,32>", "conv_sk2_bf16x3<256,128,32>",
    "resblock_fused<32>", "resblock_fused<16>", "ffn_fused<256,2048>", "rt_linear<48,256>", "conv_c64<256,64>", "conv_c32<256,32>", "conv_c16<256,16>", "conv_c64w<256,64>", "conv_c128w<256,128>", "conv_c32w<256,32>", "conv_c256w<256,128>", "rt_linear_kb<48,256>",
    "conv_f16<64>", "conv_f16<128>", "conv_f16<256>"};
static_assert(sizeof(kTileNames) / sizeof(kTileNames[0]) == kNumTileCfg, "one name per ProfCls, in enum order");
static std::atomic<int> g_prof_mask{0};
static std::atomic<int> g_prof_mask_hi{0};
static std::vector<ProfRec> g_prof_recs;
static std::vector<std::pair<hipEvent_t, hipEvent_t>> g_prof_pool;
static std::mutex g_prof_mu;

void prof_enable(int cls_mask) { g_prof_mask.store(cls_mask, std::memory_order_relaxed); }
void prof_enable_hi(int cls_mask) { g_prof_mask_hi.store(cls_mask, std::memory_order_relaxed); }
const char* prof_cfg_name(int cls) { return (cls >= 0 && cls < kNumTileCfg) ? kTileNames[cls] : "?"; }
void prof_reset() {
  for (auto& r : g_prof_recs) g_prof_pool.push_back({r.e0, r.e1});
  g_prof_recs.clear();
}
int prof_read_issued(int cls, double* issued) {
  double v = 0;
  for (auto& r : g_prof_recs) if (r.cls == cls) v += r.issued;
  if (issued) *issued = v;
  return SS_OK;
}
int prof_read(int cls, double* ms_total, double* flops_total, long long* launches, double* bytes_total) {
  double ms = 0, fl = 0, by = 0; long long n = 0;
  for (auto& r : g_prof_recs) {
    if (r.cls != cls) continue;
    if (hipEventSynchronize(r.e1) != hipSuccess) return SS_ERR_HIP;
    float t = 0.f;
    if (hipEventElapsedTime(&t, r.e0, r.e1) != hipSuccess) return SS_ERR_HIP;
    ms += t; fl += r.flops; by += r.bytes; ++n;
  }
  if (ms_total) *ms_total = ms;
  if (flops_total) *flops_total = fl;
  if (launches) *launches = n;
  if (bytes_total) *bytes_total = by;
  return SS_OK;
}

struct ProfTotals { std::atomic<unsigned long long> flops{0}, bytes{0}, launches{0}; };
static ProfTotals g_prof_totals[kNumTileCfg];
static std::mutex g_tot_mu;
struct ShapeTot { long launches = 0; double rows = 0, flops = 0, bytes = 0; };
using ShapeKey = std::tuple<int, int, int, int, int>;
static std::map<ShapeKey, ShapeTot>* g_shapes = nullptr;
static std::string shape_table() {
  std::string out = "class N taps Cin operands launches mean_rows gflop_per_launch mbyte_per_launch\n";
  if (!g_shapes) return out;
  char line[256];
  for (auto& kv : *g_shapes) {
    const ShapeTot& z = kv.second;
    snprintf(line, sizeof line, "%d %d %d %d %d %ld %.0f %.3f %.2f\n", std::get<0>(kv.first), std::get<1>(kv.first), std::get<2>(kv.first),
             std::get<3>(kv.first), std::get<4>(kv.first), z.launches, z.rows / z.launches, z.flops / z.launches * 1e-9, z.bytes / z.launches * 1e-6);
    out += line;
  }
  return out;
}
static void shape_log_dump() {
  const char* path = getenv("SS_SHAPE_LOG");
  FILE* f = path ? fopen(path, "w") : nullptr;
  if (!f) return;
  std::lock_guard<std::mutex> lk(g_tot_mu);
  fputs(shape_table().c_str(), f);
  fclose(f);
}
static std::atomic<int> g_shape_log{getenv("SS_SHAPE_LOG") != nullptr ? 1 : 0};
void prof_shape_log(int on) {
  std::lock_guard<std::mutex> lk(g_tot_mu);
  if (on && g_shapes && !getenv("SS_SHAPE_LOG")) g_shapes->clear();
  g_shape_log.store(on ? 1 : 0, std::memory_order_relaxed);
}
int prof_shape_dump(char* buf, int cap) {
  std::lock_guard<std::mutex> lk(g_tot_mu);
  const std::string t = shape_table();
  if (buf && cap > 0) { const int n = (int)std::min<size_t>(t.size(), (size_t)cap - 1); memcpy(buf, t.data(), n); buf[n] = 0; }
  return (int)t.size() + 1;
}
int prof_totals(int cls, double* flops, double* bytes, long long* launches) {
  if (cls < 0 || cls >= kNumTileCfg) return SS_ERR_ARG;
  if (flops) *flops = (double)g_prof_totals[cls].flops.load(std::memory_order_relaxed);
  if (bytes) *bytes = (double)g_prof_totals[cls].bytes.load(std::memory_order_relaxed);
  if (launches) *launches = (long long)g_prof_totals[cls].launches.load(std::memory_order_relaxed);
  return SS_OK;
}
static void algo_work(const GemmArgs& a, double& flops, double& bytes) {
  flops = a.algo_flops > 0 ? a.algo_flops : 2.0 * (double)a.M * a.N * a.taps * a.Cin;
  const double ncols = a.glu ? a.N / 2 : a.N;
  bytes = 4.0 * ((double)a.N * a.taps * a.Cin + (a.bias ? a.N : 0) + (double)a.in_len * a.Cin +
                 (double)a.M * ncols * (1 + (a.R ? 1 : 0) + (a.R2 ? 1 : 0)));
  if (a.algo_bytes > 0) bytes = a.algo_bytes;
}

static bool prof_cls_winograd(ProfCls cls) { return cls >= PROF_CONV_C64W && cls <= PROF_CONV_C256W; }

int prof_begin(const GemmArgs& a, hipStream_t stream, ProfCls cls, ProfRec& rec, bool& prof) {
  {
    double fl, by;
    algo_work(a, fl, by);
    g_prof_totals[cls].flops.fetch_add((unsigned long long)(fl + 0.5), std::memory_order_relaxed);
    g_prof_totals[cls].bytes.fetch_add((unsigned long long)(by + 0.5), std::memory_order_relaxed);
    g_prof_totals[cls].launches.fetch_add(1ull, std::memory_order_relaxed);
    if (g_shape_log.load(std::memory_order_relaxed)) {
      std::lock_guard<std::mutex> lk(g_tot_mu);
      if (!g_shapes) { g_shapes = new std::map<ShapeKey, ShapeTot>(); if (getenv("SS_SHAPE_LOG")) atexit(shape_log_dump); }
      const int ops = (a.R ? 1 : 0) | (a.R2 ? 2 : 0) | (a.C2 ? 4 : 0) | (a.in_act != ACT_NONE ? 8 : 0) | (a.act != ACT_NONE ? 16 : 0) | (a.glu ? 32 : 0) | (a.nseg > 0 ? 64 : 0);
      ShapeTot& z = (*g_shapes)[ShapeKey(cls, a.N, a.taps, a.Cin, ops)];
      z.launches += 1; z.rows += a.M; z.flops += fl; z.bytes += by;
    }
  }
  prof = cls < 32 ? ((unsigned)g_prof_mask.load(std::memory_order_relaxed) >> cls) & 1u
                  : ((unsigned)g_prof_mask_hi.load(std::memory_order_relaxed) >> (cls - 32)) & 1u;
  if (!prof) return SS_OK;
  std::lock_guard<std::mutex> lk(g_prof_mu);
  if (!g_prof_pool.empty()) { rec.e0 = g_prof_pool.back().first; rec.e1 = g_prof_pool.back().second; g_prof_pool.pop_back(); }
  else { SS_HIP_CHECK(hipEventCreate(&rec.e0)); SS_HIP_CHECK(hipEventCreate(&rec.e1)); }
  rec.cls = cls;
  algo_work(a, rec.flops, rec.bytes);
  rec.issued = (prof_cls_winograd(cls) && a.taps >= 3) ? rec.flops * (4.0 * (a.taps / 3) + (a.taps % 3 ? a.taps % 3 + 1 : 0)) / (2.0 * a.taps) : rec.flops;
  SS_HIP_CHECK(hipEventRecord(rec.e0, stream));
  return SS_OK;
}
int prof_end(hipStream_t stream, ProfRec& rec, bool prof) {
  if (prof) {
    std::lock_guard<std::mutex> lk(g_prof_mu);
    SS_HIP_CHECK(hipEventRecord(rec.e1, stream));
    g_prof_recs.push_back(rec);
  }
  return SS_OK;
}

constexpr int default_pd(int, int) { return 1; }

template <int BM, int BN, int BK, int WM, int WN, int KS = 1, int PD = default_pd(BM, BN), bool BLK = false>
static int launch_cfg(const GemmArgs& a, hipStream_t stream, ProfCls cls) {
  constexpr size_t kLds = (size_t)KS * 2 * (BM + BN) * (BK + 8) * sizeof(float);
  static_assert(kLds <= 160 * 1024, "LDS budget");
  static_assert((size_t)(KS - 1) * BM * BN * sizeof(float) <= kLds, "reduction scratch fits the staging buffers");
  if constexpr (kLds > 64 * 1024) SS_MAX_LDS_ONCE((&conv_gemm_kernel<BM, BN, BK, WM, WN, KS, PD, BLK>), kLds);
  const int mmax = (a.nseg > 0 ? a.max_seg_out : a.M) - a.m_begin;
  dim3 grid(cdiv(mmax, BM), cdiv(a.N, BN), a.nseg > 0 ? a.nseg : 1);
  if (grid.x >= 32 && grid.y * grid.z > 1) grid.x = (grid.x + 7) & ~7u;
  ProfRec rec{}; bool prof = false;
  int rc = prof_begin(a, stream, cls, rec, prof);
  if (rc != SS_OK) return rc;
  hipLaunchKernelGGL((conv_gemm_kernel<BM, BN, BK, WM, WN, KS, PD, BLK>), grid, dim3(256 * KS), kLds, stream, a);
  SS_LAUNCH_CHECK();
  return prof_end(stream, rec, prof);
}

template <int BM, int BN, int BK, int WM, int WN, int MAXKS>
static int launch_cfg_ks(const GemmArgs& a, hipStream_t stream, ProfCls cls, long tiles) {
  const int nk = a.taps * (a.Cin / BK);
  int ks = 1;
  while (ks < MAXKS && tiles * 4 * ks < 1024 && nk / (ks * 2) >= 2) ks *= 2;
  if constexpr (MAXKS >= 4) { if (ks >= 4) return launch_cfg<BM, BN, BK, WM, WN, 4>(a, stream, cls); }
  if constexpr (MAXKS >= 2) { if (ks >= 2) return launch_cfg<BM, BN, BK, WM, WN, 2>(a, stream, cls); }
  return launch_cfg<BM, BN, BK, WM, WN, 1>(a, stream, cls);
}

template <int SK, int WN, bool GLU = false>
static int launch_smallm(const GemmArgs& a, hipStream_t stream, ProfCls cls) {
  dim3 grid((cdiv(a.N, 16 * WN) + 7) & ~7, cdiv(a.M, 16));
  ProfRec rec{}; bool prof = false;
  int rc = prof_begin(a, stream, cls, rec, prof);
  if (rc != SS_OK) return rc;
  if (a.ln_g && a.Cin > 512) return SS_ERR_ARG;
  if (a.ln_g) hipLaunchKernelGGL((smallm_gemm_kernel<SK, WN, true, GLU>), grid, dim3(256), 0, stream, a);
  else hipLaunchKernelGGL((smallm_gemm_kernel<SK, WN, false, GLU>), grid, dim3(256), 0, stream, a);
  SS_LAUNCH_CHECK();
  return prof_end(stream, rec, prof);
}

constexpr size_t SKW_SYNC_BYTES = (16 + 1024) * sizeof(unsigned) + 256;
static std::mutex g_skw_mu;
static std::vector<SkWorkspace*> g_skw_live;
static std::map<std::pair<int, hipStream_t>, SkWorkspace*> g_skw_fallback;
static thread_local SkWorkspace* t_skw = nullptr;

SkWorkspace* sk_workspace_new() {
  SkWorkspace* w = new SkWorkspace();
  std::lock_guard<std::mutex> lk(g_skw_mu);
  g_skw_live.push_back(w);
  return w;
}
void sk_workspace_free(SkWorkspace* w) {
  if (!w) return;
  {
    std::lock_guard<std::mutex> lk(g_skw_mu);
    for (size_t i = 0; i < g_skw_live.size(); ++i)
      if (g_skw_live[i] == w) { g_skw_live.erase(g_skw_live.begin() + i); break; }
  }
  if (w->ws) (void)hipFree(w->ws);
  if (w->sync1) (void)hipFree(w->sync1);
  if (w->sync2) (void)hipFree(w->sync2);
  if (w->sync3) (void)hipFree(w->sync3);
  if (w->dbg) (void)hipFree(w->dbg);
  delete w;
}
namespace {
std::mutex g_disp_mu;
std::atomic<unsigned> g_disp_gen{1};
Dispatch env_defaults() {
  Dispatch d;
  auto I = [](const char* k, int dflt) { const char* e = getenv(k); return e ? atoi(e) : dflt; };
  auto L = [](const char* k, long long dflt) { const char* e = getenv(k); return e ? atoll(e) : dflt; };
  d.attn_split = I("SS_ATTN_NO_SPLIT", 0) ? -1 : 0; d.attn_q16 = I("SS_ATTN_Q16", d.attn_q16);
  d.c16_off = I("SS_NO_CONV_C16", 0) ? 1 : 0; d.c32_off = I("SS_NO_CONV_C32", 0) ? 1 : 0; d.c64_off = I("SS_NO_CONV_C64", 0) ? 1 : 0;
  d.c16_min_rows = L("SS_CONV_C16_MIN_ROWS", d.c16_min_rows); d.c32_min_rows = L("SS_CONV_C32_MIN_ROWS", d.c32_min_rows);
  d.c64_min_rows = L("SS_CONV_C64_MIN_ROWS", d.c64_min_rows);
  d.c64w_on = I("SS_CONV_C64_WINOGRAD", 1); d.c128w_on = I("SS_CONV_C128_WINOGRAD", 1); d.c256w_on = I("SS_CONV_C256_WINOGRAD", 1);
  d.c32w_on = I("SS_CONV_C32_WINOGRAD", 1); d.c64w_min_k = I("SS_CONV_C64_WINOGRAD_MIN_K", 3);
  d.c128w_min_rows = L("SS_CONV_C128_MIN_ROWS", d.c128w_min_rows); d.c256w_min_rows = L("SS_CONV_C256_MIN_ROWS", d.c256w_min_rows);
  if (getenv("SS_FFN_WM")) { d.ffn_wm = I("SS_FFN_WM", 3); d.ffn_wm_forced = 1; }
  d.ffn_fusion = I("SS_NO_FFN_FUSION", 0) ? 0 : 1; d.ffn_min_rows = I("SS_FFN_MIN_ROWS", d.ffn_min_rows);
  if (getenv("SS_SK_MIN_GFLOP")) d.sk_min_flops = 1e9 * atof(getenv("SS_SK_MIN_GFLOP"));
  d.no_resblock_fusion = I("SS_NO_RESBLOCK_FUSION", 0); d.no_pair_fusion = I("SS_NO_PAIR_FUSION", 0);
  d.rt_off = I("SS_NO_RTLIN", 0) ? 1 : 0; d.rt_min_rows = I("SS_RTLIN_MIN_ROWS", d.rt_min_rows); d.rt_min_units = L("SS_RTLIN_MIN_UNITS", d.rt_min_units);
  d.rt_kb_min_units = L("SS_RTLIN_KB_MIN_UNITS", d.rt_kb_min_units); d.rt_kb_uw = I("SS_RTLIN_KB_UW", d.rt_kb_uw); d.rt_kb_xmap = I("SS_RTLIN_KB_XMAP", d.rt_kb_xmap);
  return d;
}
Dispatch& process_settings() { static Dispatch d = env_defaults(); return d; }
thread_local const Dispatch* t_disp = nullptr;
thread_local CtxDispatch t_disp_own;
}
void dispatch_edit(const std::function<void(Dispatch&)>& fn) {
  std::lock_guard<std::mutex> lk(g_disp_mu);
  fn(process_settings());
  g_disp_gen.fetch_add(1, std::memory_order_release);
}
void slab_debug(int grid, long long min_rows) {
  const Dispatch dflt = env_defaults();
  dispatch_edit([=](Dispatch& d) {
    d.slab_grid_cap = grid > 0 ? grid : 0;
    const bool set = min_rows >= 0;
    d.c16_min_rows = set ? min_rows : dflt.c16_min_rows; d.c32_min_rows = set ? min_rows : dflt.c32_min_rows;
    d.c64_min_rows = set ? min_rows : dflt.c64_min_rows;
    d.c128w_min_rows = set ? min_rows : dflt.c128w_min_rows; d.c256w_min_rows = set ? min_rows : dflt.c256w_min_rows;
  });
}
const Dispatch* CtxDispatch::refresh() {
  const unsigned now = g_disp_gen.load(std::memory_order_acquire);
  if (gen != now) {
    std::lock_guard<std::mutex> lk(g_disp_mu);
    d = process_settings();
    gen = g_disp_gen.load(std::memory_order_relaxed);
  }
  return &d;
}
const Dispatch& disp() { return t_disp ? *t_disp : *t_disp_own.refresh(); }
DispatchScope::DispatchScope(const Dispatch* d) : prev(t_disp) { t_disp = d; }
DispatchScope::~DispatchScope() { t_disp = prev; }

SkScope::SkScope(SkWorkspace* w) : prev(t_skw), prev_disp(t_disp) { t_skw = w; t_disp = w ? w->disp.refresh() : nullptr; }
SkScope::~SkScope() { t_skw = prev; t_disp = prev_disp; }

int sk_workspace_acquire(hipStream_t stream, SkWorkspace** out) {
  *out = nullptr;
  int dev = 0;
  SS_HIP_CHECK(hipGetDevice(&dev));
  SkWorkspace* w = t_skw;
  if (!w) {
    std::lock_guard<std::mutex> lk(g_skw_mu);
    SkWorkspace*& slot = g_skw_fallback[std::make_pair(dev, stream)];
    if (!slot) { slot = new SkWorkspace(); g_skw_live.push_back(slot); }
    w = slot;
  }
  if (!w->ws) {
    int cus = 0;
    SS_HIP_CHECK(hipDeviceGetAttribute(&cus, hipDeviceAttributeMultiprocessorCount, dev));
    if (cus <= 0) cus = 256;
    if (cus > 512) cus = 512;
    w->dev = dev; w->cus = cus;
    SS_HIP_CHECK(hipMalloc(&w->ws, (size_t)cus * 256 * 128 * sizeof(float)));
    SS_HIP_CHECK(hipMalloc(&w->sync1, SKW_SYNC_BYTES));
    SS_HIP_CHECK(hipMalloc(&w->sync2, SKW_SYNC_BYTES));
    SS_HIP_CHECK(hipMemsetAsync(w->sync1, 0, SKW_SYNC_BYTES, stream));
    SS_HIP_CHECK(hipMemsetAsync(w->sync2, 0, SKW_SYNC_BYTES, stream));
    SS_HIP_CHECK(hipMalloc(&w->sync3, 4096 * sizeof(unsigned)));
    SS_HIP_CHECK(hipMemsetAsync(w->sync3, 0, 4096 * sizeof(unsigned), stream));
    SS_HIP_CHECK(hipStreamSynchronize(stream));
  } else if (w->dev != dev) {
    return SS_ERR_ARG;
  }
  *out = w;
  return SS_OK;
}

int device_cus(int& cus) {
  static std::mutex mu;
  static int n[128] = {0};
  int dev = 0;
  SS_HIP_CHECK(hipGetDevice(&dev));
  if (dev < 0 || dev >= 128) return SS_ERR_ARG;
  std::lock_guard<std::mutex> lk(mu);
  if (n[dev] == 0) {
    int v = 0;
    SS_HIP_CHECK(hipDeviceGetAttribute(&v, hipDeviceAttributeMultiprocessorCount, dev));
    n[dev] = v > 0 ? v : 256;
  }
  cus = n[dev];
  return SS_OK;
}

bool slab_layout_ok(const GemmArgs& a) {
  return a.same_rows && a.stride == 1 && a.chunk == 0 && !a.glu && !a.ln_g && a.lda == a.Cin && (a.ldc & 3) == 0 &&
         (!a.R || (a.ldr & 3) == 0) && (!a.R2 || (a.ldr2 & 3) == 0) && (!a.C2 || (a.ldc2 & 3) == 0);
}
bool slab_conv_ok(const GemmArgs& a, int c) {
  return slab_layout_ok(a) && !a.x3 && a.Cin == c && a.N == c &&
         (a.in_act == ACT_NONE || (a.in_act == ACT_LRELU && a.in_slope > 0.f && a.in_slope < 1.f)) &&
         (a.act == ACT_NONE || a.act == ACT_LRELU);
}

int sk_workspace_error_count() {
  std::lock_guard<std::mutex> lk(g_skw_mu);
  int total = 0;
  for (SkWorkspace* w : g_skw_live)
    for (unsigned* sy : {w->sync1, w->sync2}) {
      unsigned v = 0;
      if (sy && hipMemcpy(&v, sy + 8, sizeof(v), hipMemcpyDeviceToHost) == hipSuccess) total += (int)v;
    }
  return total;
}

void debug_force_tile(int bm, int bn, int ks) {
  dispatch_edit([=](Dispatch& d) { d.force_bm = bm; d.force_bn = bn; d.force_ks = ks; d.sk_groups = (bm == 1 && bn == 8); });
}
bool debug_tile_forced() { return disp().force_bm != 0; }

static thread_local int t_canon = CANON_NONE;
CanonScope::CanonScope(int mode) : prev(t_canon) { t_canon = mode; }
CanonScope::~CanonScope() { t_canon = prev; }
int canon_mode() { return t_canon; }
void canon_debug_set(int mode) { t_canon = mode; }

static bool smallm_shape_ok(const GemmArgs& a) {
  const bool glu_ok = !a.glu || (a.N % 32 == 0 && a.act == ACT_NONE && a.alpha == 1.f && !a.R);
  return a.taps == 1 && a.stride == 1 && a.pad == 0 && glu_ok && a.nseg == 0 && a.chunk == 0 && a.in_act == ACT_NONE && !a.R2 &&
         !a.C2 && a.div == 0.f && !a.ln_out && (a.act == ACT_NONE || a.act == ACT_SILU || a.act == ACT_RELU) && a.M > 0 &&
         a.M <= 1024 && a.Cin % 64 == 0 && (a.lda & 3) == 0 && (!a.ln_g || a.Cin <= 512);
}

static int launch_canon(const GemmArgs& a, hipStream_t stream) {
  const int M = a.nseg > 0 ? a.max_seg_out : a.M;
  const bool k32 = (a.Cin % 32) == 0;
  const int nseg = a.nseg > 0 ? a.nseg : 1;
  if (a.ln_out) return SS_ERR_ARG;
  if (a.canon == CANON_SMALLM) {
    if (!smallm_shape_ok(a)) return SS_ERR_ARG;
    if (a.glu) return launch_smallm<2, 2, true>(a, stream, PROF_SMALLM_2x2);
    if (a.Cin >= 1024 || a.N <= 4096) return launch_smallm<4, 1>(a, stream, PROF_SMALLM_4x1);
    return launch_smallm<2, 2>(a, stream, PROF_SMALLM_2x2);
  }
  if (a.seg_mb || a.seg_A) {
    if (a.nseg <= 0 || a.ln_g) return SS_ERR_ARG;
    return k32 ? launch_cfg<32, 64, 32, 2, 2, 1, 1, true>(a, stream, PROF_GEMM_32x64x32) : launch_cfg<32, 64, 16, 2, 2, 1, 1, true>(a, stream, PROF_GEMM_32x64x16);
  }
  if (rtlin_shape_ok(a) && (a.ln_g || rtlin_eligible(a))) return launch_rtlin(a, stream);
  if (a.ln_g) return SS_ERR_ARG;
  if (rtlin_kb_eligible(a)) return launch_rtlin_kb(a, stream);
  if (a.N <= 16) return launch_cfg<128, 16, 16, 4, 1, 1, 1, true>(a, stream, PROF_GEMM_128x16x16);
  if (a.N <= 32 && !a.glu) return k32 ? launch_cfg<128, 32, 32, 4, 1, 1, 1, true>(a, stream, PROF_GEMM_128x32x32) : launch_cfg<128, 32, 16, 4, 1, 1, 1, true>(a, stream, PROF_GEMM_128x32x16);
  if (M <= 16) return k32 ? launch_cfg<16, 128, 32, 1, 4, 1, 1, true>(a, stream, PROF_GEMM_16x128x32) : launch_cfg<16, 128, 16, 1, 4, 1, 1, true>(a, stream, PROF_GEMM_16x128x16);
  const long t3264 = (long)cdiv(M, 32) * cdiv(a.N, 64) * nseg;
  if (!k32) return launch_cfg<32, 64, 16, 2, 2, 1, 1, true>(a, stream, PROF_GEMM_32x64x16);
  if (a.glu || t3264 >= 768) return launch_cfg<32, 64, 32, 2, 2, 1, 1, true>(a, stream, PROF_GEMM_32x64x32);
  return launch_cfg<32, 32, 32, 2, 2, 1, 1, true>(a, stream, PROF_GEMM_32x32x32);
}

bool smallm_eligible(const GemmArgs& a) {
  if (disp().force_bm > 1) return false;
  const int M = a.nseg > 0 ? a.max_seg_out : a.M;
  const bool glu_ok = !a.glu || (a.N % 32 == 0 && a.act == ACT_NONE && a.alpha == 1.f && !a.R);
  const bool plain_linear = a.taps == 1 && a.stride == 1 && a.pad == 0 && glu_ok && a.nseg == 0 && a.chunk == 0 &&
                            a.in_act == ACT_NONE && !a.R2 && !a.C2 && a.div == 0.f &&
                            (a.act == ACT_NONE || a.act == ACT_SILU || a.act == ACT_RELU);
  static const int max_rows = getenv("SS_SMALLM_MAX_ROWS") ? atoi(getenv("SS_SMALLM_MAX_ROWS")) : 192;
  return plain_linear && M <= max_rows && M > 0 && a.Cin % 64 == 0 && (a.lda & 3) == 0;
}


int launch_conv_gemm(const GemmArgs& a_in, hipStream_t stream) {
  GemmArgs a = a_in;
  const int M = a.nseg > 0 ? a.max_seg_out : a.M;
  if (M <= 0 || a.N <= 0) return SS_OK;
  if (a.Wf16) return launch_conv_f16(a, stream);
  if (a.Cin % 16 != 0 || (a.lda & 3) != 0 || a.taps < 1) return SS_ERR_ARG;
  if (a.glu && (a.N % 32 != 0 || a.C2)) return SS_ERR_ARG;
  const bool k32 = (a.Cin % 32) == 0;
  const int nseg = a.nseg > 0 ? a.nseg : 1;
  if (a.canon == CANON_NONE) a.canon = t_canon;
  if (a.canon != CANON_NONE && !disp().force_bm) { a.m_begin = 0; return launch_canon(a, stream); }
  if (a.seg_mb || a.seg_A) return SS_ERR_ARG;
  if (a.m_begin > 0) {
    if (a.nseg > 0 || a.m_begin >= a.M || a.ln_g || a.ln_out || a.N <= 32) return SS_ERR_ARG;
    const long t = (long)cdiv(a.M - a.m_begin, 32) * cdiv(a.N, 64);
    if (k32 && t >= 768) return launch_cfg<32, 64, 32, 2, 2, 1>(a, stream, PROF_GEMM_32x64x32);
    return k32 ? launch_cfg_ks<32, 64, 32, 2, 2, 4>(a, stream, PROF_GEMM_32x64x32, t) : launch_cfg_ks<32, 64, 16, 2, 2, 4>(a, stream, PROF_GEMM_32x64x16, t);
  }
  if ((!disp().force_bm || a.ln_out) && gemv_eligible(a)) return launch_gemv(a, stream);
  if (a.ln_out) return SS_ERR_ARG;
  if (smallm_eligible(a)) {
    if (a.glu) return launch_smallm<2, 2, true>(a, stream, PROF_SMALLM_2x2);
    const long wgs16 = (long)cdiv(M, 16) * cdiv(a.N, 16);
    if (a.Cin >= 1024 || wgs16 <= 1024) return launch_smallm<4, 1>(a, stream, PROF_SMALLM_4x1);
    if (wgs16 <= 4096) return launch_smallm<2, 2>(a, stream, PROF_SMALLM_2x2);
    return launch_smallm<1, 4>(a, stream, PROF_SMALLM_1x4);
  }
  if (!disp().force_bm && conv_c64_eligible(a)) return conv_c64w_eligible(a) ? launch_conv_c64w(a, stream) : launch_conv_c64(a, stream);
  if (!disp().force_bm && conv_wide_winograd_eligible(a, 128)) return launch_conv_c128w(a, stream);
  if (!disp().force_bm && conv_wide_winograd_eligible(a, 256)) return launch_conv_c256w(a, stream);
  if (!disp().force_bm && conv_c32_eligible(a)) return conv_c32w_eligible(a) ? launch_conv_c32w(a, stream) : launch_conv_c32(a, stream);
  if (!disp().force_bm && conv_c16_eligible(a)) return launch_conv_c16(a, stream);
  if (!disp().force_bm && rtlin_eligible(a)) return launch_rtlin(a, stream);
  if (a.ln_g) return SS_ERR_ARG;
  if (disp().force_bm == 1 && conv_sk_eligible(a)) return launch_conv_sk(a, stream, disp().force_ks);
  if (disp().force_bm == 4 && conv_sk2_eligible(a)) return launch_conv_sk2(a, stream, disp().force_ks);
  if (disp().force_bm == 5 && conv_sk2_eligible(a)) { GemmArgs b = a; b.x3 = 1; return launch_conv_sk2(b, stream, disp().force_ks); }
  if (!disp().force_bm && conv_sk_eligible(a) && 2.0 * (double)a.M * a.N * a.taps * a.Cin >= disp().sk_min_flops) {
    const long long nk = (long long)a.taps * (a.Cin / 32);
    const bool wide = a.N % 128 == 0;
    const long long units = (long long)cdiv(a.M, 128) * (a.N / (wide ? 128 : 64)) * nk;
    static const long long min_units = getenv("SS_SK_MIN_UNITS") ? atoll(getenv("SS_SK_MIN_UNITS")) : 12 * 512;
    static const bool no_sk2 = getenv("SS_NO_SK2") && atoi(getenv("SS_NO_SK2"));
    static const int sk2_min_k64 = getenv("SS_SK2_MINK64") ? atoi(getenv("SS_SK2_MINK64")) : 192;
    if (!no_sk2 && conv_sk2_eligible(a) && (wide ? units >= min_units : a.taps * a.Cin >= sk2_min_k64)) return launch_conv_sk2(a, stream);
    if (wide ? units >= min_units : a.taps * a.Cin >= 448) return launch_conv_sk(a, stream);
  }
  if (disp().force_bm && a.N > 32 && k32) {
    const int f = disp().force_bm * 10000 + (disp().force_bn % 100) * 100 + disp().force_ks;
    switch (f) {
#define SS_CASE(BM_, BN_, KS_, PD_, CLS_) case BM_ * 10000 + BN_ * 100 + KS_ * 10 + PD_: return launch_cfg<BM_, BN_, 32, 2, 2, KS_, PD_>(a, stream, CLS_);
      SS_CASE(64, 64, 1, 1, PROF_GEMM_64x64x32) SS_CASE(64, 64, 1, 2, PROF_GEMM_64x64x32) SS_CASE(64, 64, 1, 3, PROF_GEMM_64x64x32)
      SS_CASE(64, 64, 2, 2, PROF_GEMM_64x64x32) SS_CASE(64, 64, 2, 3, PROF_GEMM_64x64x32)
      SS_CASE(32, 64, 1, 1, PROF_GEMM_32x64x32) SS_CASE(32, 64, 1, 2, PROF_GEMM_32x64x32) SS_CASE(32, 64, 1, 3, PROF_GEMM_32x64x32) SS_CASE(32, 64, 1, 4, PROF_GEMM_32x64x32)
      SS_CASE(32, 64, 2, 3, PROF_GEMM_32x64x32) SS_CASE(32, 64, 4, 3, PROF_GEMM_32x64x32)
      SS_CASE(32, 32, 1, 1, PROF_GEMM_32x32x32) SS_CASE(32, 32, 1, 2, PROF_GEMM_32x32x32) SS_CASE(32, 32, 1, 3, PROF_GEMM_32x32x32) SS_CASE(32, 32, 1, 4, PROF_GEMM_32x32x32)
      SS_CASE(32, 32, 2, 3, PROF_GEMM_32x32x32) SS_CASE(32, 32, 4, 3, PROF_GEMM_32x32x32)
#undef SS_CASE
      case 128 * 10000 + 28 * 100 + 11: return launch_cfg<128, 128, 16, 2, 2, 1, 1>(a, stream, PROF_GEMM_128x128x16);
      case 128 * 10000 + 64 * 100 + 11: return launch_cfg<128, 64, 32, 2, 2, 1, 1>(a, stream, PROF_GEMM_128x64x32);
      default: break;
    }
  }
  if (disp().force_bm != 2 && conv_slab_eligible(a) && a.M >= 2048) return launch_conv_slab(a, stream);
  if (a.N <= 16) return launch_cfg_ks<128, 16, 16, 4, 1, 2>(a, stream, PROF_GEMM_128x16x16, (long)cdiv(M, 128) * nseg);
  if (a.N <= 32 && !a.glu) {
    const long tl = (long)cdiv(M, 128) * nseg;
    return k32 ? launch_cfg_ks<128, 32, 32, 4, 1, 2>(a, stream, PROF_GEMM_128x32x32, tl) : launch_cfg_ks<128, 32, 16, 4, 1, 2>(a, stream, PROF_GEMM_128x32x16, tl);
  }
  if (M <= 16) {
    return k32 ? launch_cfg<16, 128, 32, 1, 4>(a, stream, PROF_GEMM_16x128x32) : launch_cfg<16, 128, 16, 1, 4>(a, stream, PROF_GEMM_16x128x16);
  }
  const long t128 = (long)cdiv(M, 128) * cdiv(a.N, 128) * nseg;
  const long t3232 = (long)cdiv(M, 32) * cdiv(a.N, 32) * nseg;
  const long t3264 = (long)cdiv(M, 32) * cdiv(a.N, 64) * nseg;
  (void)t128;
  if (k32 && t3264 >= 768) return launch_cfg<32, 64, 32, 2, 2, 1>(a, stream, PROF_GEMM_32x64x32);
  if (!k32 || a.glu) {
    return k32 ? launch_cfg_ks<32, 64, 32, 2, 2, 4>(a, stream, PROF_GEMM_32x64x32, t3264) : launch_cfg_ks<32, 64, 16, 2, 2, 4>(a, stream, PROF_GEMM_32x64x16, t3264);
  }
  const int nk = a.taps * (a.Cin / 32);
  if (t3232 >= 700 || nk < 4) return launch_cfg<32, 32, 32, 2, 2, 1>(a, stream, PROF_GEMM_32x32x32);
  if (t3232 >= 300 || nk < 8) return launch_cfg<32, 32, 32, 2, 2, 2>(a, stream, PROF_GEMM_32x32x32);
  return launch_cfg<32, 32, 32, 2, 2, 4>(a, stream, PROF_GEMM_32x32x32);
}

}
```

streamspeech_amd/csrc/gemm.hpp:

```cpp
#pragma once
#include "common.hpp"
#include "dispatch.hpp"

namespace ss {

struct GemmArgs {
  const float* A = nullptr;
  const float* W = nullptr;
  const float* Wwino = nullptr;
  const void* Wf16 = nullptr;
  const float* bias = nullptr;
  const float* R = nullptr;
  const float* R2 = nullptr;
  float* C = nullptr;
  int lda = 0, ldc = 0, ldr = 0, ldr2 = 0;
  int M = 0, N = 0, Cin = 0;
  int taps = 1, dil = 1, stride = 1, pad = 0;
  int in_len = 0;
  int chunk = 0;
  int m_begin = 0;
  int in_act = ACT_NONE;
  float in_slope = 0.1f;
  int act = ACT_NONE;
  float alpha = 1.0f;
  float div = 0.0f;
  float act_slope = 0.1f;
  float* C2 = nullptr;
  int ldc2 = 0;
  float c2_slope = 0.1f;
  int glu = 0;
  const int* segs = nullptr;
  int nseg = 0;
  int max_seg_out = 0;
  const int* seg_mb = nullptr;
  const float* const* seg_A = nullptr;
  double algo_flops = 0.0;
  double algo_bytes = 0.0;
  const float* ln_g = nullptr;
  const float* ln_b = nullptr;
  float* ln_out = nullptr;
  int same_rows = 0;
  int x3 = 0;
  int canon = 0;
};
constexpr int CANON_NONE = 0, CANON_SEQ = 1, CANON_SMALLM = 2;
constexpr int CANON_KBLOCK = 64;
struct CanonScope {
  explicit CanonScope(int mode);
  ~CanonScope();
  int prev;
};
int canon_mode();
void canon_debug_set(int mode);

enum ProfCls : int {
  PROF_GEMM_128x16x16 = 0, PROF_GEMM_128x32x32 = 1, PROF_GEMM_128x32x16 = 2, PROF_GEMM_16x128x32 = 3, PROF_GEMM_16x128x16 = 4,
  PROF_GEMM_128x128x16 = 5, PROF_GEMM_128x64x32 = 6, PROF_GEMM_64x64x32 = 7, PROF_GEMM_64x64x16 = 8, PROF_GEMM_32x64x32 = 9,
  PROF_GEMM_32x64x16 = 10, PROF_GEMM_32x32x32 = 11,
  PROF_SMALLM_4x1 = 12, PROF_SMALLM_2x2 = 13, PROF_SMALLM_1x4 = 14,
  PROF_CONV_SK = 15, PROF_CONV_SLAB32 = 16, PROF_CONV_SLAB16 = 17, PROF_CONV_SK2 = 18, PROF_CONV_SK2_BF16X3 = 19,
  PROF_RESBLOCK32 = 20, PROF_RESBLOCK16 = 21, PROF_FFN = 22, PROF_RTLIN = 23,
  PROF_CONV_C64 = 24, PROF_CONV_C32 = 25, PROF_CONV_C16 = 26,
  PROF_CONV_C64W = 27, PROF_CONV_C128W = 28, PROF_CONV_C32W = 29, PROF_CONV_C256W = 30,
  PROF_RTLIN_KB = 31,
  PROF_CONV_F16_64 = 32, PROF_CONV_F16_128 = 33, PROF_CONV_F16_256 = 34,
};
constexpr int kNumTileCfg = PROF_CONV_F16_256 + 1;
void prof_enable(int cls_mask);
void prof_enable_hi(int cls_mask);
void prof_reset();
int prof_read(int cls, double* ms_total, double* flops_total, long long* launches, double* bytes_total = nullptr);
const char* prof_cfg_name(int cls);
int prof_totals(int cls, double* flops, double* bytes, long long* launches);
int prof_read_issued(int cls, double* issued_flops_total);
void prof_shape_log(int on);
int prof_shape_dump(char* buf, int cap);

struct ProfRec { hipEvent_t e0, e1; double flops, bytes, issued; int cls; };
int prof_begin(const GemmArgs& a, hipStream_t stream, ProfCls cls, ProfRec& rec, bool& prof);
int prof_end(hipStream_t stream, ProfRec& rec, bool prof);

struct SkWorkspace {
  int dev = -1, cus = 0;
  float* ws = nullptr;
  unsigned* sync1 = nullptr;
  unsigned* sync2 = nullptr;
  unsigned* sync3 = nullptr;
  unsigned base1[8] = {0, 0, 0, 0, 0, 0, 0, 0}, epoch1 = 0;
  unsigned base2 = 0, epoch2 = 0;
  unsigned long long* dbg = nullptr;
  CtxDispatch disp;
};
SkWorkspace* sk_workspace_new();
void sk_workspace_free(SkWorkspace* w);
struct SkScope {
  explicit SkScope(SkWorkspace* w);
  ~SkScope();
  SkWorkspace* prev;
  const Dispatch* prev_disp;
};
int sk_workspace_acquire(hipStream_t stream, SkWorkspace** out);
int sk_workspace_error_count();

bool conv_sk_eligible(const GemmArgs& a);
int launch_conv_sk(const GemmArgs& a, hipStream_t stream, int g_force = 0);
int conv_sk_error_count();
void conv_sk_set_groups(int on);

bool conv_sk2_eligible(const GemmArgs& a);
int launch_conv_sk2(const GemmArgs& a, hipStream_t stream, int g_force = 0);
int conv_sk2_error_count();

inline bool slab_rows_ok(long long rows) { return rows > 0 && rows < (1ll << 30); }

inline size_t slab_lds_bytes(int slab_rows, int lda, int maxseg) {
  return (size_t)((slab_rows * lda + 3) & ~3) * sizeof(float) + (maxseg + 2) * sizeof(int);
}
inline long long slab_max_blocks(int M, int bm, int nseg) { return (long long)cdiv(M, bm) + (nseg > 0 ? nseg : 1); }
inline int slab_grid(int occ, int cus, int M, int bm, int nseg) {
  const long long g = std::min<long long>((long long)occ * cus, std::max<long long>(1, slab_max_blocks(M, bm, nseg)));
  const int cap = disp().slab_grid_cap;
  return (int)(cap > 0 ? std::min<long long>(g, cap) : g);
}
void slab_debug(int grid, long long min_rows);
bool slab_layout_ok(const GemmArgs& a);
bool slab_conv_ok(const GemmArgs& a, int c);
int device_cus(int& cus);

bool conv_slab_eligible(const GemmArgs& a);
int launch_conv_slab(const GemmArgs& a, hipStream_t stream);

bool conv_pair_eligible(int C, int taps, int dil, int lda, int ldc, int nseg, long long M);
int launch_conv_pair(const float* A, int lda, const float* W1, const float* b1, const float* W2, const float* b2, float* C,
                     int ldc, const float* R2, int ldr2, float div, float* C2, int ldc2, float c2_slope, int Cch, int taps,
                     int dil, int M, int in_len, float slope, const int* segs, int nseg, hipStream_t stream);

bool resblock_fused_eligible(int C, int taps, const int* dil, int ldx, int ldy, int nseg, long long M);
int launch_resblock_fused(const float* X, int ldx, const float* const* W1, const float* const* B1, const float* const* W2,
                          const float* const* B2, const int* dil, float* Y, int ldy, const float* R2, int ldr2, float div, int C,
                          int taps, int M, float slope, const int* segs, int nseg, hipStream_t stream);

bool conv_c64_eligible(const GemmArgs& a);
bool conv_c64_enabled();
int launch_conv_c64(const GemmArgs& a, hipStream_t stream);
bool conv_c64w_eligible(const GemmArgs& a);
int launch_conv_c64w(const GemmArgs& a, hipStream_t stream);
int launch_wino_pack(const float* W, float* WW, int C, int taps, hipStream_t stream);
void conv_c64w_debug(int enable);
bool conv_c64w_enabled();
bool conv_wide_winograd_eligible(const GemmArgs& a, int ch);
int launch_conv_c128w(const GemmArgs& a, hipStream_t stream);
void conv_c128w_debug(int enable);
bool conv_c128w_enabled();
int launch_conv_c256w(const GemmArgs& a, hipStream_t stream);
void conv_c256w_debug(int enable);
bool conv_c256w_enabled();
bool conv_c32w_eligible(const GemmArgs& a);
int launch_conv_c32w(const GemmArgs& a, hipStream_t stream);
void conv_c32w_debug(int enable);
bool conv_c32w_enabled();
void conv_c64_debug(int enable);

bool conv_c32_eligible(const GemmArgs& a);
bool conv_c32_enabled();
int launch_conv_c32(const GemmArgs& a, hipStream_t stream);
void conv_c32_debug(int enable);

bool conv_c16_eligible(const GemmArgs& a);
bool conv_c16_enabled();
int launch_conv_c16(const GemmArgs& a, hipStream_t stream);
void conv_c16_debug(int enable);

bool conv_f16_eligible(const GemmArgs& a);
bool conv_f16_geometry_ok(int C, int taps, int dil);
int launch_conv_f16(const GemmArgs& a, hipStream_t stream);
size_t f16_pack_halves(int C, int taps);
int launch_f16_pack(const float* W, void* Wf, int C, int taps, hipStream_t stream);

bool rtlin_eligible(const GemmArgs& a);
bool rtlin_shape_ok(const GemmArgs& a);
int launch_rtlin(const GemmArgs& a, hipStream_t stream);
void rtlin_debug(int grid, int enable);
bool rtlin_kb_shape_ok(const GemmArgs& a);
bool rtlin_kb_eligible(const GemmArgs& a);
int launch_rtlin_kb(const GemmArgs& a, hipStream_t stream);

bool ffn_fused_eligible(int D, int F, int act, int M, int ldx, int ldy, bool canon = false);
int launch_ffn_fused(const float* X, int ldx, float* Y, int ldy, const float* ln_g, const float* ln_b, const float* W1,
                     const float* b1, const float* W2, const float* b2, float alpha, const float* ln2_g, const float* ln2_b,
                     int M, int D, int F, hipStream_t stream, int canon = 0);
void ffn_fused_debug_grid(int g);
void ffn_fused_debug_rows(int wm);

bool gemv_eligible(const GemmArgs& a);
bool smallm_eligible(const GemmArgs& a);

void debug_force_tile(int bm, int bn, int ks);
bool debug_tile_forced();

int launch_conv_gemm(const GemmArgs& a, hipStream_t stream);

}
```

streamspeech_amd/csrc/vocoder.hip:

```cpp
#include "model_internal.hpp"

#include <cstdint>
#include <tuple>


namespace {
struct WinoShared { DevBuf buf; size_t floats = 0; int refs = 0; };
struct WinoKey {
  int dev; const float* blob; uint64_t sig;
  bool operator<(const WinoKey& o) const { return std::tie(dev, blob, sig) < std::tie(o.dev, o.blob, o.sig); }
};
std::mutex g_wino_mu;
std::map<WinoKey, WinoShared> g_wino;
inline uint64_t fnv(uint64_t h, uint64_t v) { for (int i = 0; i < 8; ++i) { h ^= (v >> (8 * i)) & 0xff; h *= 1099511628211ull; } return h; }
uint64_t blob_sig(const ss_vocoder* v, const float* d_blob) {
  const ss_vocoder_config* cfg = &v->cfg;
  uint64_t sig = fnv(fnv(fnv(14695981039346656037ull, (uint64_t)cfg->upsample_initial_channel), (uint64_t)cfg->n_up), (uint64_t)cfg->n_res);
  for (int j = 0; j < cfg->n_res; ++j) sig = fnv(sig, (uint64_t)cfg->resblock_kernel_sizes[j]);
  for (size_t i = 0; i < v->rb_c1.size(); ++i) sig = fnv(fnv(sig, (uint64_t)(v->rb_c1[i].w - d_blob)), (uint64_t)(v->rb_c2[i].w - d_blob));
  return sig;
}
std::mutex g_f16_mu;
std::map<WinoKey, WinoShared> g_f16;
bool f16_stage(int ch) { return ch == 64 || ch == 128 || ch == 256; }
// ... 6 lines not shown
  ss_vocoder* v = new ss_vocoder();
  v->cfg = *cfg;
  v->blob = d_blob;
  v->sc = new ss_scratch();
  int rc = v->wt.build(d_blob, blob_floats, names, offsets, numels, n_slots);
  if (rc != SS_OK) { scratch_unref(v->sc); delete v; return rc; }
  WeightTable& w = v->wt;
  const int E = cfg->embedding_dim, Hd = cfg->dur_hidden, kd = cfg->dur_kernel;
  v->dict = w.get("voc.dict", (int64_t)cfg->num_embeddings * E);
  v->dur_c1 = {w.get("voc.dur.conv1.w", (int64_t)Hd * kd * E), w.get("voc.dur.conv1.b", Hd)};
  v->dur_ln1 = {w.get("voc.dur.ln1.g", Hd), w.get("voc.dur.ln1.b", Hd)};
  v->dur_c2 = {w.get("voc.dur.conv2.w", (int64_t)Hd * kd * Hd), w.get("voc.dur.conv2.b", Hd)};
  v->dur_ln2 = {w.get("voc.dur.ln2.g", Hd), w.get("voc.dur.ln2.b", Hd)};
  v->dur_proj = {w.get("voc.dur.proj.w", Hd), w.get("voc.dur.proj.b", 1)};
  const int C0 = cfg->upsample_initial_channel;
  v->pre = {w.get("voc.pre.w", (int64_t)C0 * 7 * cfg->model_in_dim), w.get("voc.pre.b", C0)};
  int C = C0;
  for (int i = 0; i < cfg->n_up; ++i) {
    const int Co = C / 2, st = cfg->upsample_rates[i];
    v->ups.push_back({w.get("voc.up" + std::to_string(i) + ".w", (int64_t)st * Co * 3 * C),
                      w.get("voc.up" + std::to_string(i) + ".b", (int64_t)st * Co)});
    for (int j = 0; j < cfg->n_res; ++j) {
      const int kr = cfg->resblock_kernel_sizes[j];
      for (int dd = 0; dd < 3; ++dd) {
        const std::string p = "voc.rb" + std::to_string(i * cfg->n_res + j);
        v->rb_c1.push_back({w.get(p + ".c1." + std::to_string(dd) + ".w", (int64_t)Co * kr * Co),
                            w.get(p + ".c1." + std::to_string(dd) + ".b", Co)});
        v->rb_c2.push_back({w.get(p + ".c2." + std::to_string(dd) + ".w", (int64_t)Co * kr * Co),
                            w.get(p + ".c2." + std::to_string(dd) + ".b", Co)});
      }
    }
    C = Co;
  }
  v->post = {w.get("voc.post.w", (int64_t)7 * C), w.get("voc.post.b", 1)};
  {
    auto it = w.map.find("voc.spkr.table");
    if (it != w.map.end()) {
      const int64_t per = (int64_t)16 * C0;
      if (it->second.n <= 0 || it->second.n % per || it->second.n / per > INT32_MAX || (C0 & 3)) { scratch_unref(v->sc); delete v; return SS_ERR_ARG; }
      v->spk_table = it->second.p;
      v->n_spk = (int)(it->second.n / per);
    }
  }
  if (!w.missing.empty()) { scratch_unref(v->sc); delete v; return SS_ERR_MISSING_WEIGHT; }
  {
    auto wino_stage = [](int ch) { return ch == 32 || ch == 64 || ch == 128 || ch == 256; };
    size_t need = 0;
    int Cs = C0;
    for (int i = 0; i < cfg->n_up; ++i) {
      Cs /= 2;
      if (wino_stage(Cs)) for (int j = 0; j < cfg->n_res; ++j) need += 6 * (size_t)Cs * ((cfg->resblock_kernel_sizes[j] + 2) / 3) * 4 * Cs;
    }
    if (need) {
      int dev = 0;
      if (hipGetDevice(&dev) != hipSuccess) { scratch_unref(v->sc); delete v; return SS_ERR_HIP; }
      std::lock_guard<std::mutex> lk(g_wino_mu);
      const WinoKey key{dev, d_blob, blob_sig(v, d_blob)};
      WinoShared& sh = g_wino[key];
      const bool fresh = sh.refs == 0;
      if (!fresh && sh.floats != need) { scratch_unref(v->sc); delete v; return SS_ERR_ARG; }
      if (fresh) {
        rc = sh.buf.ensure(need * sizeof(float));
        if (rc != SS_OK) { g_wino.erase(key); scratch_unref(v->sc); delete v; return rc; }
        sh.floats = need;
      }
      float* dst = sh.buf.f();
      Cs = C0;
      for (int i = 0; i < cfg->n_up && rc == SS_OK; ++i) {
        Cs /= 2;
        if (!wino_stage(Cs)) continue;
        for (int j = 0; j < cfg->n_res && rc == SS_OK; ++j) {
          const int kr = cfg->resblock_kernel_sizes[j];
          const size_t n = (size_t)Cs * ((kr + 2) / 3) * 4 * Cs;
          for (int dd = 0; dd < 3 && rc == SS_OK; ++dd) {
            const int idx = (i * cfg->n_res + j) * 3 + dd;
            if (fresh) rc = launch_wino_pack(v->rb_c1[idx].w, dst, Cs, kr, nullptr);
            v->rb_c1[idx].ww = dst; dst += n;
            if (fresh && rc == SS_OK) rc = launch_wino_pack(v->rb_c2[idx].w, dst, Cs, kr, nullptr);
            v->rb_c2[idx].ww = dst; dst += n;
          }
        }
      }
      if (fresh && rc == SS_OK && hipDeviceSynchronize() != hipSuccess) rc = SS_ERR_HIP;
      if (rc != SS_OK) {
        if (fresh) { sh.buf.release(); g_wino.erase(key); }
        scratch_unref(v->sc); delete v; return rc;
      }
      ++sh.refs;
      v->wino = sh.buf.f(); v->wino_key = d_blob;
    }
  }
  *out = v;
  return SS_OK;
}

extern "C" int ss_vocoder_num_speakers(const ss_vocoder* v) { return v ? v->n_spk : 0; }

extern "C" int ss_vocoder_set_bf16x3(ss_vocoder* v, int on) {
  if (!v) return SS_ERR_ARG;
  v->x3 = on ? 1 : 0;
  return SS_OK;
}

static int f16_take(ss_vocoder* v) {
  const ss_vocoder_config& c = v->cfg;
  size_t need = 0;
  for (int i = 0, Cs = c.upsample_initial_channel; i < c.n_up; ++i) {
    Cs /= 2;
    if (f16_stage(Cs)) for (int j = 0; j < c.n_res; ++j) need += 6 * f16_pack_halves(Cs, c.resblock_kernel_sizes[j]);
  }
  if (!need) return SS_OK;
  for (int i = 0, Cs = c.upsample_initial_channel; i < c.n_up; ++i) {
    Cs /= 2;
    if (!f16_stage(Cs)) continue;
    for (int j = 0; j < c.n_res; ++j)
      for (int dd = 0; dd < 3; ++dd)
        if (!conv_f16_geometry_ok(Cs, c.resblock_kernel_sizes[j], c.resblock_dilations[j][dd]) ||
            !conv_f16_geometry_ok(Cs, c.resblock_kernel_sizes[j], 1))
          return SS_ERR_ARG;
  }
  int dev = 0;
  if (hipGetDevice(&dev) != hipSuccess) return SS_ERR_HIP;
  std::lock_guard<std::mutex> lk(g_f16_mu);
  const WinoKey key{dev, v->blob, blob_sig(v, v->blob)};
  WinoShared& sh = g_f16[key];
  const bool fresh = sh.refs == 0;
  if (!fresh && sh.floats != need) return SS_ERR_ARG;
  int rc = SS_OK;
  if (fresh) {
    rc = sh.buf.ensure(need * sizeof(uint16_t));
    if (rc != SS_OK) { g_f16.erase(key); return rc; }
    sh.floats = need;
  }
  char* dst = static_cast<char*>(sh.buf.p);
  std::vector<ConvW> rb1 = v->rb_c1, rb2 = v->rb_c2;
  for (int i = 0, Cs = c.upsample_initial_channel; i < c.n_up && rc == SS_OK; ++i) {
    Cs /= 2;
    if (!f16_stage(Cs)) continue;
    for (int j = 0; j < c.n_res && rc == SS_OK; ++j) {
      const int kr = c.resblock_kernel_sizes[j];
      const size_t n = f16_pack_halves(Cs, kr) * sizeof(uint16_t);
      for (int dd = 0; dd < 3 && rc == SS_OK; ++dd) {
        const int idx = (i * c.n_res + j) * 3 + dd;
        if (fresh) rc = launch_f16_pack(rb1[idx].w, dst, Cs, kr, nullptr);
        rb1[idx].wh = dst; dst += n;
        if (fresh && rc == SS_OK) rc = launch_f16_pack(rb2[idx].w, dst, Cs, kr, nullptr);
        rb2[idx].wh = dst; dst += n;
      }
    }
  }
  if (fresh && rc == SS_OK && hipDeviceSynchronize() != hipSuccess) rc = SS_ERR_HIP;
  if (rc != SS_OK) {
    if (fresh) { sh.buf.release(); g_f16.erase(key); }
    return rc;
  }
  ++sh.refs;
  v->rb_c1.swap(rb1); v->rb_c2.swap(rb2);
  v->f16w = sh.buf.p;
  return SS_OK;
}

extern "C" int ss_vocoder_set_f16(ss_vocoder* v, int on) {
  if (!v) return SS_ERR_ARG;
  if (on && !v->f16w) RET(f16_take(v));
  v->f16 = on ? 1 : 0;
  return SS_OK;
}

extern "C" void ss_vocoder_destroy(ss_vocoder* v) {
  if (!v) return;
  if (v->f16w) {
    std::lock_guard<std::mutex> lk(g_f16_mu);
    for (auto it = g_f16.begin(); it != g_f16.end(); ++it)
      if (it->first.blob == v->blob && it->second.buf.p == v->f16w) {
        if (--it->second.refs == 0) { it->second.buf.release(); g_f16.erase(it); }
        break;
      }
  }
  if (v->wino_key) {
    std::lock_guard<std::mutex> lk(g_wino_mu);
    for (auto it = g_wino.begin(); it != g_wino.end(); ++it)
      if (it->first.blob == v->wino_key && it->second.buf.f() == v->wino) {
        if (--it->second.refs == 0) { it->second.buf.release(); g_wino.erase(it); }
        break;
      }
  }
  scratch_unref(v->sc);
  delete v;
}

extern "C" int ss_vocoder_bind_scratch(ss_vocoder* v, ss_scratch* sc) {
  if (!v || !sc) return SS_ERR_ARG;
  if (sc != v->sc) {
    sc->refs.fetch_add(1);
    scratch_unref(v->sc);
    v->sc = sc;
  }
  return SS_OK;
}

struct GenBufs { float *bx, *bt, *br, *bs, *bxa, *bra, *bsa, *br2; };
struct SpkSel { const int* seg = nullptr; int one = 0; int max_frames = 0; };

template <class ConvFn, class StageFn, class GeomFn>
static int hifigan_stack(const ss_vocoder* v, hipStream_t s, ConvFn&& conv, StageFn&& on_stage, GeomFn&& geom,
                         const float* frames, int Ft, const GenBufs& b, int* out_scale, int* out_C, const SpkSel* spk = nullptr) {
  const ss_vocoder_config& c = v->cfg;
  const bool f16 = v->f16 && v->f16w;
  const bool x3 = v->x3 && !f16;
  auto slab_stage = [&](int channels) {
    if (x3 || !(channels == 64 ? conv_c64_enabled() : channels == 32 ? conv_c32_enabled() : channels == 16 ? conv_c16_enabled() : false)) return false;
    long long rows = Ft; int ch = c.upsample_initial_channel; bool found = false;
    for (int i = 0; i < c.n_up && !found; ++i) { rows *= c.upsample_rates[i]; ch /= 2; found = ch == channels; }
    if (!found || rows >= (1ll << 30)) return false;
    GemmArgs probe;
    probe.same_rows = 1; probe.Cin = probe.N = probe.lda = probe.ldc = channels; probe.taps = 3; probe.dil = 1; probe.pad = 1;
    probe.M = probe.in_len = (int)rows; probe.in_act = ACT_LRELU;
    return channels == 64 ? conv_c64_eligible(probe) : channels == 32 ? conv_c32_eligible(probe) : conv_c16_eligible(probe);
  };
  const bool c64 = slab_stage(64), c32 = slab_stage(32), c16 = slab_stage(16);
  auto wino_slab_stage = [&](int channels) {
    if (f16 || x3 || !(channels == 128 ? conv_c128w_enabled() : conv_c256w_enabled())) return false;
    long long rows = Ft; int ch = c.upsample_initial_channel, stage = -1;
    for (int i = 0; i < c.n_up && stage < 0; ++i) { rows *= c.upsample_rates[i]; ch /= 2; if (ch == channels) stage = i; }
    if (stage < 0 || rows >= (1ll << 30)) return false;
    int sc = 1, gM = 0, gnseg = 0; const int* gsegs = nullptr;
    for (int i = 0; i <= stage; ++i) sc *= c.upsample_rates[i];
    geom(sc, gM, gsegs, gnseg);
    for (int j = 0; j < c.n_res; ++j)
      for (int dd = 0; dd < 3; ++dd)
        for (int which = 0; which < 2; ++which) {
          const int idx = (stage * c.n_res + j) * 3 + dd;
          GemmArgs probe;
          probe.same_rows = 1; probe.Cin = probe.N = probe.lda = probe.ldc = probe.ldr = probe.ldr2 = probe.ldc2 = channels;
          probe.taps = c.resblock_kernel_sizes[j]; probe.dil = which ? 1 : c.resblock_dilations[j][dd];
          probe.pad = probe.dil * (probe.taps - 1) / 2; probe.M = probe.in_len = gM; probe.nseg = gnseg; probe.in_act = ACT_LRELU;
          probe.Wwino = which ? v->rb_c2[idx].ww : v->rb_c1[idx].ww;
          if (!conv_wide_winograd_eligible(probe, channels)) return false;
        }
    return true;
  };
  const bool c128 = wino_slab_stage(128), c256 = wino_slab_stage(256);
  auto preact = [c64, c128, c256, f16](int channels) {
    return channels >= 64 && !(c64 && channels == 64) && !(c128 && channels == 128) && !(c256 && channels == 256) && !(f16 && f16_stage(channels));
  };
  auto up_preact = [c64](int channels) { return channels >= 64 && !(c64 && channels == 64); };
  auto mk = [x3, f16](const float* A, int Cin, const ConvW& cw, int Cout, int k, int dil, float* Cc, int ldc) {
    GemmArgs a;
    a.A = A; a.lda = Cin; a.W = cw.w; a.Wwino = cw.ww; a.bias = cw.b; a.C = Cc; a.ldc = ldc; a.ldr = ldc; a.ldr2 = ldc; a.ldc2 = ldc;
    a.N = Cout; a.Cin = Cin; a.taps = k; a.dil = dil; a.stride = 1; a.pad = dil * (k - 1) / 2; a.same_rows = 1;
    a.x3 = x3;
    if (f16) a.Wf16 = cw.wh;
    return a;
  };
  int scale = 1, C = c.upsample_initial_channel;
  RET(on_stage(scale));
  {
    GemmArgs a = mk(frames, c.model_in_dim, v->pre, C, 7, 1, b.bx, C);
    if (up_preact(C) && !spk) a.C2 = b.bxa;
    if (f16) a.canon = CANON_SEQ;
    RET(conv(a, scale));
    if (spk) {
      int gM = 0, gnseg = 0; const int* gsegs = nullptr;
      geom(scale, gM, gsegs, gnseg);
      const bool pa0 = up_preact(C);
      RET(launch_spkr_pre_add(b.bx, pa0 ? b.bxa : b.bx, C, C, v->spk_table, spk->seg, spk->one, gsegs, gnseg, spk->max_frames, gM, pa0 ? 1 : 0,
                              0.1f, s));
    }
  }
  for (int i = 0; i < c.n_up; ++i) {
    const int st = c.upsample_rates[i], Co = C / 2;
    const bool pa_in = up_preact(C), pa = preact(Co);
    {
      GemmArgs a = mk(pa_in ? b.bxa : b.bx, C, v->ups[i], st * Co, 3, 1, b.bs, st * Co);
      if (!pa_in) { a.in_act = ACT_LRELU; a.in_slope = 0.1f; }
      if (pa) a.C2 = b.bsa;
      a.algo_flops = 2.0 * Ft * scale * C * Co * c.upsample_kernel_sizes[i];
      if (f16 && Co >= 64) a.canon = CANON_SEQ;
      RET(conv(a, scale));
    }
    scale *= st; C = Co;
    RET(on_stage(scale));
    const bool pa_next = (i + 1 < c.n_up) && up_preact(C);
    for (int j = 0; j < c.n_res; ++j) {
      const int kr = c.resblock_kernel_sizes[j];
      int gM = 0, gnseg = 0; const int* gsegs = nullptr;
      geom(scale, gM, gsegs, gnseg);
      static const int c32_min_k = getenv("SS_CONV_C32_MIN_K") ? atoi(getenv("SS_CONV_C32_MIN_K")) : 7;
      static const int c16_min_k = getenv("SS_CONV_C16_MIN_K") ? atoi(getenv("SS_CONV_C16_MIN_K")) : 11;
      const bool per_conv = (c32 && C == 32 && kr >= c32_min_k) || (c16 && C == 16 && kr >= c16_min_k);
      if (!pa && !per_conv && !disp().no_resblock_fusion && resblock_fused_eligible(C, kr, c.resblock_dilations[j], C, C, gnseg, gM)) {
        const float *W1[3], *B1[3], *W2[3], *B2[3];
        for (int dd = 0; dd < 3; ++dd) {
          const int idx = (i * c.n_res + j) * 3 + dd;
          W1[dd] = v->rb_c1[idx].w; B1[dd] = v->rb_c1[idx].b; W2[dd] = v->rb_c2[idx].w; B2[dd] = v->rb_c2[idx].b;
        }
        RET(launch_resblock_fused(b.bs, C, W1, B1, W2, B2, c.resblock_dilations[j], b.bx, C, j > 0 ? b.bx : nullptr, C,
                                  j == c.n_res - 1 ? (float)c.n_res : 0.f, C, kr, gM, 0.1f, gsegs, gnseg, s));
        continue;
      }
      const bool fuse = !pa && !per_conv && !disp().no_pair_fusion && kr == 3 &&
                        conv_pair_eligible(C, kr, c.resblock_dilations[j][2], C, C, gnseg, gM);
      const float* cur = b.bs;
      for (int dd = 0; dd < 3; ++dd) {
        const int idx = (i * c.n_res + j) * 3 + dd;
        if (fuse) {
          float* out = dd == 0 ? b.br : dd == 1 ? b.br2 : b.bx;
          const float* R2 = (dd == 2 && j > 0) ? b.bx : nullptr;
          const float div = (dd == 2 && j == c.n_res - 1) ? (float)c.n_res : 0.f;
          RET(launch_conv_pair(cur, C, v->rb_c1[idx].w, v->rb_c1[idx].b, v->rb_c2[idx].w, v->rb_c2[idx].b, out, C, R2, C, div,
                               nullptr, C, 0.1f, C, kr, c.resblock_dilations[j][dd], gM, gM, 0.1f, gsegs, gnseg, s));
          cur = out;
          continue;
        }
        const float* rin = dd == 0 ? b.bs : b.br;
        const float* rin_act = dd == 0 ? b.bsa : b.bra;
        GemmArgs a1 = mk(pa ? rin_act : rin, C, v->rb_c1[idx], C, kr, c.resblock_dilations[j][dd], b.bt, C);
        if (pa) { a1.act = ACT_LRELU; a1.act_slope = 0.1f; }
        else { a1.in_act = ACT_LRELU; a1.in_slope = 0.1f; }
        RET(conv(a1, scale));
        GemmArgs a2 = mk(b.bt, C, v->rb_c2[idx], C, kr, 1, dd < 2 ? b.br : b.bx, C);
        if (!pa) { a2.in_act = ACT_LRELU; a2.in_slope = 0.1f; }
        a2.R = rin;
        if (dd < 2) {
          if (pa) a2.C2 = b.bra;
        } else {
          a2.R2 = j == 0 ? nullptr : b.bx;
          a2.div = (j == c.n_res - 1) ? (float)c.n_res : 0.f;
          if (pa_next && j == c.n_res - 1) a2.C2 = b.bxa;
        }
        RET(conv(a2, scale));
      }
    }
  }
  *out_scale = scale; *out_C = C;
  return SS_OK;
}

static int conv1d(hipStream_t s, const float* A, int T, int Cin, const ConvW& cw, int Cout, int k, int dil,
                  float* C, int in_act, float slope, int act, const float* R, const float* R2, float div) {
  GemmArgs a;
  a.A = A; a.lda = Cin; a.W = cw.w; a.bias = cw.b; a.C = C; a.ldc = Cout; a.R = R; a.ldr = Cout; a.R2 = R2; a.ldr2 = Cout;
  a.M = T; a.N = Cout; a.Cin = Cin; a.taps = k; a.dil = dil; a.stride = 1; a.pad = dil * (k - 1) / 2; a.in_len = T;
  a.in_act = in_act; a.in_slope = slope; a.act = act; a.div = div; a.same_rows = 1;
  return launch_conv_gemm(a, s);
}

static bool spkr_args_ok(const ss_vocoder* v, bool have, const int32_t* h_spkr, int B) {
  if (!have) return v->n_spk == 0;
  if (v->n_spk == 0 || !h_spkr) return false;
  for (int b = 0; b < B; ++b)
    if (h_spkr[b] < 0 || h_spkr[b] >= v->n_spk) return false;
  return true;
}

static int vocoder_forward(ss_vocoder* v, void* stream, const int32_t* d_codes, int K, int dur_prediction,
                           const int32_t* d_forced_dur, float* d_wav, int64_t wav_capacity,
                           int32_t* d_dur, int64_t* h_n_samples, const int32_t* h_spkr) {
  if (!v || K <= 0 || !d_codes || !d_wav || !d_dur) return SS_ERR_ARG;
  if (!spkr_args_ok(v, h_spkr != nullptr, h_spkr, 1)) return SS_ERR_ARG;
  SkScope sk_scope(v->sc->skws);
  hipStream_t s = (hipStream_t)stream;
  const ss_vocoder_config& c = v->cfg;
  const int E = c.embedding_dim, Hd = c.dur_hidden;
  RET(v->sc->v_small.ensure(((size_t)K * (E + 2 * Hd + 1) + 2 * (K + 2)) * sizeof(float)));
  float* emb = v->sc->v_small.f();
  float* t1 = emb + (size_t)K * E;
  float* t2 = t1 + (size_t)K * Hd;
  float* logdur = t2 + (size_t)K * Hd;
  int* cum = reinterpret_cast<int*>(logdur + K);
  int* ones = cum + K + 1;
  RET(launch_gather_rows(d_codes, v->dict, E, emb, K, s, v->cfg.num_embeddings));
  const int* forced = d_forced_dur;
  if (!forced && dur_prediction) {
    RET(conv1d(s, emb, K, E, v->dur_c1, Hd, c.dur_kernel, 1, t1, ACT_NONE, 0.f, ACT_RELU, nullptr, nullptr, 0.f));
    RET(launch_layernorm(t1, Hd, t1, Hd, v->dur_ln1.g, v->dur_ln1.b, K, Hd, 1e-5f, s));
    RET(conv1d(s, t1, K, Hd, v->dur_c2, Hd, c.dur_kernel, 1, t2, ACT_NONE, 0.f, ACT_RELU, nullptr, nullptr, 0.f));
    RET(launch_layernorm(t2, Hd, t2, Hd, v->dur_ln2.g, v->dur_ln2.b, K, Hd, 1e-5f, s));
    RET(conv1d(s, t2, K, Hd, v->dur_proj, 1, 1, 1, logdur, ACT_NONE, 0.f, ACT_NONE, nullptr, nullptr, 0.f));
  } else if (!forced) {
    SS_HIP_CHECK(hipMemsetD32Async(reinterpret_cast<hipDeviceptr_t>(ones), 1, K, s));
    forced = ones;
  }
  RET(launch_dur_predict(logdur, forced, K, d_dur, cum, s));
  int total = 0;
  SS_HIP_CHECK(hipMemcpyAsync(&total, cum + K, sizeof(int), hipMemcpyDeviceToHost, s));
  SS_HIP_CHECK(hipStreamSynchronize(s));
  const int Fr = total;
  int hop = 1;
  for (int i = 0; i < c.n_up; ++i) hop *= c.upsample_rates[i];
  const int64_t S = (int64_t)Fr * hop;
  if (h_n_samples) *h_n_samples = S;
  if (S > wav_capacity) return SS_ERR_CAPACITY;
  if (Fr <= 0) return SS_OK;

  size_t stage_max = (size_t)Fr * c.upsample_initial_channel;
  {
    int T = Fr, C = c.upsample_initial_channel;
    for (int i = 0; i < c.n_up; ++i) { T *= c.upsample_rates[i]; C /= 2; stage_max = std::max(stage_max, (size_t)T * C); }
  }
  RET(v->sc->v_ws.ensure((8 * stage_max + (size_t)Fr * E) * sizeof(float)));
  float* frames = v->sc->v_ws.f();
  GenBufs gb;
  gb.bx = frames + (size_t)Fr * E;
  gb.bt = gb.bx + stage_max;
  gb.br = gb.bt + stage_max;
  gb.bs = gb.br + stage_max;
  gb.bxa = gb.bs + stage_max;
  gb.bra = gb.bxa + stage_max;
  gb.bsa = gb.bra + stage_max;
  gb.br2 = gb.bsa + stage_max;
  RET(launch_repeat_rows(emb, cum, K, E, frames, Fr, s));
  int T = 1, C = 0;
  SpkSel sel;
  if (h_spkr) { sel.one = h_spkr[0]; sel.max_frames = Fr; }
  RET(hifigan_stack(v, s, [&](GemmArgs& a, int scale) { a.M = Fr * scale; a.in_len = Fr * scale; return launch_conv_gemm(a, s); },
                    [](int) { return SS_OK; },
                    [&](int scale, int& M, const int*& segs, int& nseg) { M = Fr * scale; segs = nullptr; nseg = 0; },
                    frames, Fr, gb, &T, &C, h_spkr ? &sel : nullptr));
  T *= Fr;
  float* bx = gb.bx;
  return launch_conv_post_tanh(bx, T, C, v->post.w, v->post.b, 0.01f, d_wav, s);
}

extern "C" int ss_vocoder_forward(ss_vocoder* v, void* stream, const int32_t* d_codes, int K, int dur_prediction,
                                  const int32_t* d_forced_dur, float* d_wav, int64_t wav_capacity,
                                  int32_t* d_dur, int64_t* h_n_samples) {
  return vocoder_forward(v, stream, d_codes, K, dur_prediction, d_forced_dur, d_wav, wav_capacity, d_dur, h_n_samples, nullptr);
}

extern "C" int ss_vocoder_forward_spkr(ss_vocoder* v, void* stream, const int32_t* d_codes, int K, int dur_prediction,
                                       const int32_t* d_forced_dur, float* d_wav, int64_t wav_capacity,
                                       int32_t* d_dur, int64_t* h_n_samples, int32_t spkr) {
  return vocoder_forward(v, stream, d_codes, K, dur_prediction, d_forced_dur, d_wav, wav_capacity, d_dur, h_n_samples, &spkr);
}


static int batch_vocoder_forward(ss_vocoder* v, void* stream, int B, const int32_t* d_codes, const int32_t* h_K,
                                 int dur_prediction, const int32_t* d_forced_dur, float* d_wav,
                                 int64_t wav_capacity, int32_t* d_dur, int64_t* h_wav_start,
                                 int64_t* h_n_samples, bool with_spkr, const int32_t* h_spkr) {
  if (!v || B <= 0 || !d_codes || !d_wav || !d_dur) return SS_ERR_ARG;
  if (!spkr_args_ok(v, with_spkr, h_spkr, B)) return SS_ERR_ARG;
  SkScope sk_scope(v->sc->skws);
  hipStream_t s = (hipStream_t)stream;
  const ss_vocoder_config& c = v->cfg;
  const int E = c.embedding_dim, Hd = c.dur_hidden;
  for (int b = 0; b < B; ++b)
    if (h_K[b] <= 0) return SS_ERR_ARG;
  const Offsets ok = prefix(h_K, B);
  const int Kt = ok.total;
  RET(v->sc->v_small.ensure(((size_t)Kt * (E + 2 * Hd + 1) + 2 * (Kt + B + 2)) * sizeof(float)));
  float* emb = v->sc->v_small.f();
  float* t1 = emb + (size_t)Kt * E;
  float* t2 = t1 + (size_t)Kt * Hd;
  float* logdur = t2 + (size_t)Kt * Hd;
  int* cum = reinterpret_cast<int*>(logdur + Kt);
  int* ones = cum + Kt + B + 1;
  std::vector<int> tk(6 * B);
  for (int b = 0; b < B; ++b) {
    int* a = &tk[4 * b]; a[0] = ok.off[b]; a[1] = h_K[b]; a[2] = ok.off[b]; a[3] = h_K[b];
    tk[4 * B + 2 * b] = ok.off[b]; tk[4 * B + 2 * b + 1] = h_K[b];
  }
  RET(v->sc->v_segs.ensure((6 * B + 16 * B + (with_spkr ? B : 0)) * sizeof(int)));
  int* dk = (int*)v->sc->v_segs.p;
  RET(upload(s, dk, tk));
  RET(launch_gather_rows(d_codes, v->dict, E, emb, Kt, s, v->cfg.num_embeddings));
  const int* forced = d_forced_dur;
  auto sconv = [&](const float* A, int Cin, const ConvW& cw, int Cout, int k, float* Cc, int act) {
    GemmArgs a;
    a.A = A; a.lda = Cin; a.W = cw.w; a.bias = cw.b; a.C = Cc; a.ldc = Cout; a.N = Cout; a.Cin = Cin; a.taps = k;
    a.pad = (k - 1) / 2; a.act = act; a.segs = dk; a.nseg = B; a.max_seg_out = ok.mx; a.M = Kt; a.in_len = Kt;
    a.canon = CANON_SEQ;
    return launch_conv_gemm(a, s);
  };
  if (!forced && dur_prediction) {
    RET(sconv(emb, E, v->dur_c1, Hd, c.dur_kernel, t1, ACT_RELU));
    RET(launch_layernorm(t1, Hd, t1, Hd, v->dur_ln1.g, v->dur_ln1.b, Kt, Hd, 1e-5f, s));
    RET(sconv(t1, Hd, v->dur_c2, Hd, c.dur_kernel, t2, ACT_RELU));
    RET(launch_layernorm(t2, Hd, t2, Hd, v->dur_ln2.g, v->dur_ln2.b, Kt, Hd, 1e-5f, s));
    RET(sconv(t2, Hd, v->dur_proj, 1, 1, logdur, ACT_NONE));
  } else if (!forced) {
    std::vector<int> one(Kt, 1);
    RET(upload(s, ones, one));
    forced = ones;
  }
  RET(launch_dur_predict(logdur, forced, 0, d_dur, cum, s, dk + 4 * B, B));
  std::vector<int> hcum(Kt + B);
  SS_HIP_CHECK(hipMemcpyAsync(hcum.data(), cum, (size_t)(Kt + B) * sizeof(int), hipMemcpyDeviceToHost, s));
  SS_HIP_CHECK(hipStreamSynchronize(s));
  int hop = 1;
  for (int i = 0; i < c.n_up; ++i) hop *= c.upsample_rates[i];
  std::vector<int> Fr(B);
  for (int b = 0; b < B; ++b) Fr[b] = hcum[ok.off[b] + b + h_K[b]];
  const Offsets of = prefix(Fr.data(), B);
  for (int b = 0; b < B; ++b) { h_wav_start[b] = (int64_t)of.off[b] * hop; h_n_samples[b] = (int64_t)Fr[b] * hop; }
  if ((int64_t)of.total * hop > wav_capacity) return SS_ERR_CAPACITY;
  if (of.total <= 0) return SS_OK;
  const int Ft = of.total;

  size_t stage_max = (size_t)Ft * c.upsample_initial_channel;
  {
    int T = Ft, C = c.upsample_initial_channel;
    for (int i = 0; i < c.n_up; ++i) { T *= c.upsample_rates[i]; C /= 2; stage_max = std::max(stage_max, (size_t)T * C); }
  }
  RET(v->sc->v_ws.ensure((8 * stage_max + (size_t)Ft * E) * sizeof(float)));
  float* frames = v->sc->v_ws.f();
  GenBufs gb;
  gb.bx = frames + (size_t)Ft * E;
  gb.bt = gb.bx + stage_max;
  gb.br = gb.bt + stage_max;
  gb.bs = gb.br + stage_max;
  gb.bxa = gb.bs + stage_max;
  gb.bra = gb.bxa + stage_max;
  gb.bsa = gb.bra + stage_max;
  gb.br2 = gb.bsa + stage_max;
  int* dseg = dk + 6 * B;
  int* drep = dseg + 4 * B;
  int* dwav = drep + 4 * B;
  auto stage_segs = [&](int scale) {
    std::vector<int> t(4 * B);
    for (int b = 0; b < B; ++b) { t[4 * b] = of.off[b] * scale; t[4 * b + 1] = Fr[b] * scale; t[4 * b + 2] = t[4 * b]; t[4 * b + 3] = t[4 * b + 1]; }
    return upload(s, dseg, t);
  };
  {
    std::vector<int> t(4 * B);
    for (int b = 0; b < B; ++b) { t[4 * b] = ok.off[b]; t[4 * b + 1] = h_K[b]; t[4 * b + 2] = of.off[b]; t[4 * b + 3] = Fr[b]; }
    RET(upload(s, drep, t));
  }
  RET(launch_repeat_rows(emb, cum, 0, E, frames, of.mx, s, drep, B));
  SpkSel sel;
  if (with_spkr) {
    int* dspk = dk + 6 * B + 16 * B;
    RET(upload(s, dspk, std::vector<int>(h_spkr, h_spkr + B)));
    sel.seg = dspk; sel.max_frames = of.mx;
  }
  int scale = 1, C = 0;
  RET(hifigan_stack(v, s,
                    [&](GemmArgs& a, int sc) {
                      a.segs = dseg; a.nseg = B; a.max_seg_out = of.mx * sc; a.M = Ft * sc; a.in_len = Ft * sc;
                      return launch_conv_gemm(a, s);
                    },
                    stage_segs,
                    [&](int sc, int& M, const int*& segs, int& nseg) { M = Ft * sc; segs = dseg; nseg = B; },
                    frames, Ft, gb, &scale, &C, with_spkr ? &sel : nullptr));
  float* bx = gb.bx;
  {
    std::vector<int> t(2 * B);
    for (int b = 0; b < B; ++b) { t[2 * b] = of.off[b] * scale; t[2 * b + 1] = Fr[b] * scale; }
    RET(upload(s, dwav, t));
  }
  return launch_conv_post_tanh(bx, of.mx * scale, C, v->post.w, v->post.b, 0.01f, d_wav, s, dwav, B);
}

extern "C" int ss_batch_vocoder_forward(ss_vocoder* v, void* stream, int B, const int32_t* d_codes, const int32_t* h_K,
                                        int dur_prediction, const int32_t* d_forced_dur, float* d_wav,
                                        int64_t wav_capacity, int32_t* d_dur, int64_t* h_wav_start,
                                        int64_t* h_n_samples) {
  return batch_vocoder_forward(v, stream, B, d_codes, h_K, dur_prediction, d_forced_dur, d_wav, wav_capacity, d_dur, h_wav_start,
                               h_n_samples, false, nullptr);
}

extern "C" int ss_batch_vocoder_forward_spkr(ss_vocoder* v, void* stream, int B, const int32_t* d_codes, const int32_t* h_K,
                                             int dur_prediction, const int32_t* d_forced_dur, float* d_wav,
                                             int64_t wav_capacity, int32_t* d_dur, int64_t* h_wav_start,
                                             int64_t* h_n_samples, const int32_t* h_spkr) {
  return batch_vocoder_forward(v, stream, B, d_codes, h_K, dur_prediction, d_forced_dur, d_wav, wav_capacity, d_dur, h_wav_start,
                               h_n_samples, true, h_spkr);
}


static int batch_vocoder_tail(ss_vocoder* v, void* stream, int B, const int32_t* d_codes, const int32_t* h_K,
                              const int32_t* h_n_new, const int32_t* h_ctx, const int32_t* h_rf, int dur_prediction,
                              float* d_out, int64_t out_capacity, int32_t* h_win_first, int32_t* h_dur, int64_t* h_out_start,
                              int64_t* h_n_out, bool with_spkr, const int32_t* h_spkr) {
  if (!v || B <= 0 || B > 32768 || !d_codes || !h_K || !h_n_new || !h_ctx || !h_rf || !d_out || !h_win_first || !h_dur ||
      !h_out_start || !h_n_out)
    return SS_ERR_ARG;
  if (!spkr_args_ok(v, with_spkr, h_spkr, B)) return SS_ERR_ARG;
  const ss_vocoder_config& c = v->cfg;
  const int E = c.embedding_dim, Hd = c.dur_hidden;
  for (int b = 0; b < B; ++b)
    if (h_K[b] <= 0 || h_n_new[b] <= 0 || h_n_new[b] > h_K[b] || h_ctx[b] < 0 || (h_ctx[b] > 0 && h_rf[b] < 0)) return SS_ERR_ARG;
  const Offsets ok = prefix(h_K, B);
  std::vector<int> cu, cl, csrc, fall(B, -1);
  for (int b = 0; b < B; ++b) {
    const bool win = h_ctx[b] > 0 && h_K[b] > h_n_new[b] + h_ctx[b];
    const int first = win ? h_K[b] - (h_n_new[b] + h_ctx[b]) : 0;
    csrc.push_back(ok.off[b] + first); cl.push_back(h_K[b] - first);
  }
  for (int b = 0; b < B; ++b)
    if (cl[b] < h_K[b]) { fall[b] = (int)cl.size(); csrc.push_back(ok.off[b]); cl.push_back(h_K[b]); }
  const int S = (int)cl.size();
  const Offsets oc = prefix(cl.data(), S);
  const int Kc = oc.total;
  cu.assign(oc.off.begin(), oc.off.end() - 1);
  const size_t n_small = (size_t)ok.total * E + (size_t)Kc * (E + 2 * Hd + 1) + 3 * ((size_t)Kc + S + 2);
  RET(v->sc->v_small.ensure(n_small * sizeof(float)));
  RET(v->sc->v_segs.ensure(((size_t)Kc + 6 * S + 12 * B + (with_spkr ? B : 0)) * sizeof(int)));
  SkScope sk_scope(v->sc->skws);
  hipStream_t s = (hipStream_t)stream;
  float* emb_all = v->sc->v_small.f();
  float* emb = emb_all + (size_t)ok.total * E;
  float* t1 = emb + (size_t)Kc * E;
  float* t2 = t1 + (size_t)Kc * Hd;
  float* logdur = t2 + (size_t)Kc * Hd;
  int* dur = reinterpret_cast<int*>(logdur + Kc);
  int* cum = dur + Kc;
  int* aux = cum + Kc + S + 2;
  int* dk = (int*)v->sc->v_segs.p;
  {
    std::vector<int> tk((size_t)Kc + 6 * S);
    for (int z = 0; z < S; ++z) {
      for (int i = 0; i < cl[z]; ++i) tk[cu[z] + i] = csrc[z] + i;
      int* a = &tk[Kc + 4 * z]; a[0] = cu[z]; a[1] = cl[z]; a[2] = cu[z]; a[3] = cl[z];
      tk[Kc + 4 * S + 2 * z] = cu[z]; tk[Kc + 4 * S + 2 * z + 1] = cl[z];
    }
    RET(upload(s, dk, tk));
  }
  const int* dmap = dk;
  const int* dconv = dk + Kc;
  const int* ddur = dconv + 4 * S;
  RET(launch_gather_rows(d_codes, v->dict, E, emb_all, ok.total, s, v->cfg.num_embeddings));
  RET(launch_gather_rows(dmap, emb_all, E, emb, Kc, s, ok.total));
  const int* forced = nullptr;
  if (dur_prediction) {
    int mx = 0;
    for (int z = 0; z < S; ++z) mx = std::max(mx, cl[z]);
    auto sconv = [&](const float* A, int Cin, const ConvW& cw, int Cout, int k, float* Cc, int act) {
      GemmArgs a;
      a.A = A; a.lda = Cin; a.W = cw.w; a.bias = cw.b; a.C = Cc; a.ldc = Cout; a.N = Cout; a.Cin = Cin; a.taps = k;
      a.pad = (k - 1) / 2; a.act = act; a.segs = dconv; a.nseg = S; a.max_seg_out = mx; a.M = Kc; a.in_len = Kc;
      a.canon = CANON_SEQ;
      return launch_conv_gemm(a, s);
// ... 130 lines not shown
```

streamspeech_amd/lib.py:

```python
import ctypes as C
import os

_HERE = os.path.dirname(os.path.abspath(__file__))
LIB_PATH = os.environ.get("SS_HIP_LIB") or os.path.join(_HERE, "libstreamspeech_hip.so")


class SSConfig(C.Structure):
    _fields_ = [(n, C.c_int32) for n in (
        "input_feat", "conv_channels", "conv_kernel", "enc_dim", "enc_ffn", "enc_heads", "enc_layers",
        "dw_kernel", "src_vocab", "tgt_vocab", "mt_layers", "dec_dim", "dec_ffn", "dec_heads",
        "t2u_layers", "unit_layers", "unit_vocab", "ctc_upsample", "pad", "eos", "unk",
        "max_rel_pos", "max_tgt_pos")]


class SSVocoderConfig(C.Structure):
    _fields_ = [
        ("num_embeddings", C.c_int32), ("embedding_dim", C.c_int32), ("model_in_dim", C.c_int32),
        ("upsample_initial_channel", C.c_int32),
        ("n_up", C.c_int32), ("upsample_rates", C.c_int32 * 8), ("upsample_kernel_sizes", C.c_int32 * 8),
        ("n_res", C.c_int32), ("resblock_kernel_sizes", C.c_int32 * 4), ("resblock_dilations", (C.c_int32 * 3) * 4),
        ("dur_hidden", C.c_int32), ("dur_kernel", C.c_int32)]


_vp, _i, _f, _i64 = C.c_void_p, C.c_int, C.c_float, C.c_int64


class SSPcmSeg(C.Structure):
    _fields_ = [("src_offset", C.c_int64), ("dst_offset", C.c_int64), ("frames", C.c_int32), ("fmt", C.c_int32),
                ("channels", C.c_int32), ("dst", C.c_int32)]


class SSPcmEmitSeg(C.Structure):
    _fields_ = [("carry", _vp), ("tail", _vp), ("taps", _vp), ("n_before", C.c_int64), ("k0", C.c_int64), ("k1", C.c_int64),
                ("out_offset", C.c_int64), ("carry_len", C.c_int32), ("n_new", C.c_int32), ("up", C.c_int32), ("down", C.c_int32),
                ("half", C.c_int32), ("fmt", C.c_int32), ("finished", C.c_int32), ("reserved", C.c_int32)]


class SSVadState(C.Structure):
    _fields_ = [("onset", C.c_int64), ("last_speech", C.c_int64), ("utt_first_frame", C.c_int64), ("floor", C.c_float),
                ("mode", C.c_int32), ("run", C.c_int32), ("reserved", C.c_int32)]


class SSVadSeg(C.Structure):
    _fields_ = [("hist", _vp), ("state", _vp), ("powers", _vp), ("hist_first", C.c_int64), ("n_hist", C.c_int64),
                ("first_frame", C.c_int64), ("n_frames", C.c_int32), ("H", C.c_int32), ("W", C.c_int32),
                ("p_abs", C.c_float), ("p_min", C.c_float), ("snr", C.c_float), ("rise", C.c_float),
                ("min_speech", C.c_int32), ("end_silence", C.c_int32), ("post_roll", C.c_int32), ("max_frames", C.c_int32),
                ("reserved", C.c_int32)]


class SSVadResult(C.Structure):
    _fields_ = [("consumed", C.c_int64), ("start_frame", C.c_int64), ("cut_sample", C.c_int64), ("last_speech", C.c_int64),
                ("events", C.c_int32), ("mode", C.c_int32)]


class SSOpAttnArgs(C.Structure):
    _fields_ = [
        ("Q", _vp), ("K", _vp), ("V", _vp), ("O", _vp),
        ("ldq", C.c_int32), ("ldk", C.c_int32), ("ldv", C.c_int32), ("ldo", C.c_int32),
        ("Tq", C.c_int32), ("Tk", C.c_int32), ("H", C.c_int32),
        ("scale", _f),
        ("causal", C.c_int32), ("chunk", C.c_int32), ("q0", C.c_int32), ("k_mask_tail", C.c_int32),
        ("P", _vp), ("ldp", C.c_int32),
        ("bias_u", _vp), ("bias_v", _vp),
        ("segs", _vp), ("nseg", C.c_int32), ("max_q", C.c_int32), ("p_tmax", C.c_int32),
        ("seg_tail", _vp),
        ("no_decode_kernel", C.c_int32),
        ("anc", _vp), ("anc_ld", C.c_int32), ("anc_slots", C.c_int32),
        ("use_split", C.c_int32)]


class SSOpConvArgs(C.Structure):
    _fields_ = [
        ("A", _vp), ("W", _vp), ("bias", _vp), ("R", _vp), ("R2", _vp), ("C", _vp), ("C2", _vp),
        ("lda", C.c_int32), ("ldc", C.c_int32), ("ldr", C.c_int32), ("ldr2", C.c_int32), ("ldc2", C.c_int32),
        ("M", C.c_int32), ("N", C.c_int32), ("Cin", C.c_int32), ("taps", C.c_int32), ("dil", C.c_int32), ("stride", C.c_int32),
        ("pad", C.c_int32), ("in_len", C.c_int32), ("chunk", C.c_int32),
        ("in_act", C.c_int32), ("in_slope", _f),
        ("act", C.c_int32), ("act_slope", _f), ("alpha", _f), ("div", _f), ("c2_slope", _f),
        ("glu", C.c_int32),
        ("segs", _vp), ("nseg", C.c_int32), ("max_seg_out", C.c_int32),
        ("same_rows", C.c_int32)]


class SSOpPoolAttnArgs(C.Structure):
    _fields_ = [
        ("Qs", _vp), ("cache", _vp), ("O", _vp),
        ("ld", C.c_int32), ("ldo", C.c_int32), ("slot_rows", C.c_int32),
        ("P", _vp), ("ldp", C.c_int32), ("p_tmax", C.c_int32),
        ("bias_u", _vp), ("bias_v", _vp),
        ("sess", _vp), ("qt_pre", _vp),
        ("nsess", C.c_int32), ("qtiles", C.c_int32), ("H", C.c_int32),
        ("scale", _f)]

class SSOpBeamState(C.Structure):
    _fields_ = [(n, _vp) for n in (
        "tok", "cum", "anc", "cand_s", "cand_t", "ignore", "done", "max_len", "npre",
        "fin_cnt", "fin_score", "fin_len", "fin_tok", "fin_pos", "fin_anc")]


SS_OP_BEAM_CAND = 64

SIGNATURES = {
    "ss_abi_version": (_i, []),
    "ss_error_string": (C.c_char_p, [_i]),
    "ss_model_create": (_i, [C.POINTER(SSConfig), _vp, C.c_size_t, C.POINTER(C.c_char_p), C.POINTER(_i64),
                             C.POINTER(_i64), _i, C.POINTER(_vp)]),
    "ss_model_destroy": (None, [_vp]),
    "ss_scratch_create": (_i, [C.POINTER(_vp)]),
    "ss_scratch_destroy": (None, [_vp]),
    "ss_scratch_set_cap": (_i, [_vp, C.c_size_t]),
    "ss_scratch_trim": (_i, [_vp, C.c_size_t]),
    "ss_scratch_bytes": (C.c_size_t, [_vp]),
    "ss_model_bind_scratch": (_i, [_vp, _vp]),
    "ss_vocoder_bind_scratch": (_i, [_vp, _vp]),
    "ss_fbank_num_frames": (_i, [_i]),
    "ss_fbank_cmvn": (_i, [_vp, _vp, _vp, _i, _f, _vp, C.POINTER(_i)]),
    "ss_encoder_out_len": (_i, [_i]),
    "ss_resample": (_i, [_vp, _vp, _i64, _i, _i, _vp, _i, _vp, _i64]),
    "ss_mp3_probe": (_i, [_vp, C.c_size_t, _vp]),
    "ss_mp3_unpack": (_i, [_vp, C.c_size_t, _i64, _vp, _vp, _vp]),
    "ss_mp3_synthesize": (_i, [_vp, _vp, _vp, _i64, _vp, _i, _i, _vp, _i64, _vp, C.POINTER(C.c_size_t)]),
    "ss_mp3_stream_create": (_i, [_i, C.POINTER(_vp)]),
    "ss_mp3_stream_destroy": (None, [_vp]),
    "ss_mp3_stream_reset": (_i, [_vp]),
    "ss_mp3_stream_bound": (_i64, [_vp, C.c_size_t]),
    "ss_mp3_stream_push": (_i, [_vp, _vp, C.c_size_t, _i, _i64, _vp, _vp, _vp, C.POINTER(_i64), _vp]),
    "ss_mp3_stream_query": (_i, [_vp, _vp]),
    "ss_mp3_stream_copy": (_i, [_vp, _vp]),
    "ss_mp3_stream_synthesize": (_i, [_vp, _vp, _vp, _i64, _vp, _i, C.POINTER(_vp), C.POINTER(_vp), C.POINTER(_i64), _i, _i, _vp,
                                      C.POINTER(C.c_size_t)]),
    "ss_flac_streaminfo": (_i, [_vp, C.c_size_t, _vp]),
    "ss_flac_probe": (_i, [_vp, C.c_size_t, _vp]),
    "ss_flac_unpack": (_i, [_vp, C.c_size_t, _i64, _vp, _vp, _i64, _vp]),
    "ss_flac_restore_host": (_i, [_vp, _vp, _i64, _vp, _i, _i, _vp, _vp]),
    "ss_flac_restore": (_i, [_vp, _vp, _vp, _i64, _i64, _vp, _i, _i, _vp, _i64, _vp, C.POINTER(C.c_size_t)]),
    "ss_pcm_scatter": (_i, [_vp, _vp, _i64, _vp, _i, C.POINTER(_vp), C.POINTER(_i64), _i]),
    "ss_pcm_pack_s16": (_i, [_vp, _vp, _i64, _vp]),
    "ss_pcm_decode_host": (_i, [_vp, _i, _i, _i64, _vp]),
    "ss_pcm_pack_s16_host": (_i, [_vp, _i64, _vp]),
    "ss_pcm_emit_count": (_i64, [_i64, _i, _i, _i, _i]),
    "ss_pcm_emit": (_i, [_vp, _vp, _i, _vp, _i64]),
    "ss_pcm_emit_host": (_i, [_vp, _i, _vp, _i64]),
    "ss_pcm_encode_host": (_i, [_vp, _i64, _i, _vp]),
    "ss_vad_scan": (_i, [_vp, _vp, _i, _vp]),
    "ss_vad_scan_host": (_i, [_vp, _i, _vp]),
    "ss_row_max_logprob": (_i, [_vp, _vp, _i, _i, _i, _i, _i, _vp]),
    "ss_log_softmax": (_i, [_vp, _vp, _i, _i, _i, _i, _i, _vp]),
    "ss_encoder_forward": (_i, [_vp, _vp, _vp, _i, _i, _i, _vp]),
    "ss_encoder_stream_reset": (_i, [_vp]),
    "ss_encoder_stream_set_tail": (_i, [_vp, _i]),
    "ss_encoder_stream_set_deferred": (_i, [_vp, _i]),
    "ss_encoder_stream_status": (_i, [_vp, _vp, _vp]),
    "ss_debug_enc_step_inject_timeout": (_i, [_vp]),
    "ss_encoder_stream_forward": (_i, [_vp, _vp, _vp, _i, _i, _i, _vp, C.POINTER(C.c_int32), C.POINTER(C.c_int32)]),
    "ss_ctc_greedy": (_i, [_vp, _vp, _i, _vp, _i, _vp, _vp, _vp, _vp, _vp]),
    "ss_stream_pool_create": (_i, [_vp, _i, _i, C.POINTER(_vp)]),
    "ss_stream_pool_destroy": (None, [_vp]),
    "ss_stream_pool_reset": (_i, [_vp, _i]),
    "ss_stream_pool_set_tail": (_i, [_vp, _i, _i]),
    "ss_encoder_stream_forward_batch": (_i, [_vp, _vp, _vp, _i, C.POINTER(C.c_int32), C.POINTER(_vp), C.POINTER(C.c_int32),
                                             C.POINTER(C.c_int32), C.POINTER(C.c_int32), _vp, C.POINTER(C.c_int32),
                                             C.POINTER(C.c_int32)]),
    "ss_stream_pool_ctc": (_i, [_vp, _vp, _vp, _i, _i, C.POINTER(C.c_int32), _vp, _vp, _vp, _vp, _vp]),
    "ss_stream_pool_stats": (_i, [_vp, C.POINTER(_i64), C.POINTER(_i64)]),
    "ss_mt_begin": (_i, [_vp, _vp, _vp, _i]),
    "ss_mt_set_persistent": (_i, [_vp, _i]),
    "ss_model_set_pack_invariant": (_i, [_vp, _i]),
    "ss_model_get_pack_invariant": (_i, [_vp]),
    "ss_debug_canon": (_i, [_i]),
    "ss_mt_get_persistent": (_i, [_vp]),
    "ss_debug_mt_inject_timeout": (_i, [_vp]),
    "ss_mt_append": (_i, [_vp, _vp, _vp, _i, _i, _i, _i, _vp, _vp, _i]),
    "ss_mt_truncate": (_i, [_vp, _i]),
    "ss_mt_greedy": (_i, [_vp, _vp, _vp, _i, C.POINTER(C.c_int32), _i, _i, _i, C.POINTER(C.c_int32), C.POINTER(_i),
                          _vp, C.POINTER(_i)]),
    "ss_t2u_units": (_i, [_vp, _vp, _vp, _i, _i, _i, _vp, _vp, _vp, _vp, _i]),
    "ss_vocoder_create": (_i, [C.POINTER(SSVocoderConfig), _vp, C.c_size_t, C.POINTER(C.c_char_p),
                               C.POINTER(_i64), C.POINTER(_i64), _i, C.POINTER(_vp)]),
    "ss_vocoder_destroy": (None, [_vp]),
    "ss_vocoder_set_bf16x3": (_i, [_vp, _i]),
    "ss_vocoder_set_f16": (_i, [_vp, _i]),
    "ss_vocoder_forward": (_i, [_vp, _vp, _vp, _i, _i, _vp, _vp, _i64, _vp, C.POINTER(_i64)]),
    "ss_vocoder_num_speakers": (_i, [_vp]),
    "ss_vocoder_forward_spkr": (_i, [_vp, _vp, _vp, _i, _i, _vp, _vp, _i64, _vp, C.POINTER(_i64), C.c_int32]),
    "ss_batch_vocoder_forward_spkr": (_i, [_vp, _vp, _i, _vp, C.POINTER(C.c_int32), _i, _vp, _vp, _i64, _vp,
                                           C.POINTER(_i64), C.POINTER(_i64), C.POINTER(C.c_int32)]),
    "ss_batch_vocoder_tail_spkr": (_i, [_vp, _vp, _i, _vp, C.POINTER(C.c_int32), C.POINTER(C.c_int32), C.POINTER(C.c_int32),
                                        C.POINTER(C.c_int32), _i, _vp, _i64, C.POINTER(C.c_int32), C.POINTER(C.c_int32),
                                        C.POINTER(_i64), C.POINTER(_i64), C.POINTER(C.c_int32)]),
    "ss_batch_fbank_cmvn": (_i, [_vp, _vp, _i, _vp, C.POINTER(_i64), C.POINTER(C.c_int32), _f, _vp, C.POINTER(C.c_int32)]),
    "ss_batch_cmvn": (_i, [_vp, _vp, _vp, _i64, _vp]),
    "ss_batch_encoder_forward": (_i, [_vp, _vp, _i, _vp, C.POINTER(C.c_int32), _i, _i, _vp, C.POINTER(C.c_int32)]),
    "ss_batch_ctc_greedy": (_i, [_vp, _vp, _i, _i, _vp, C.POINTER(C.c_int32), _vp, _vp, _vp, _vp]),
    "ss_batch_mt_greedy": (_i, [_vp, _vp, _i, _vp, C.POINTER(C.c_int32), C.POINTER(C.c_int32), _i,
                                C.POINTER(C.c_int32), _i, C.POINTER(C.c_int32), _vp, _i]),
    "ss_batch_mt_beam": (_i, [_vp, _vp, _i, _i, _vp, C.POINTER(C.c_int32), C.POINTER(C.c_int32), _i, _f, _i,
                              C.POINTER(C.c_int32), _i, C.POINTER(C.c_int32), C.POINTER(_f), C.POINTER(_f), _vp, _i]),
    "ss_batch_mt_continue": (_i, [_vp, _vp, _i, _vp, C.POINTER(C.c_int32), C.POINTER(C.c_int32), C.POINTER(C.c_int32),
                                  C.POINTER(C.c_int32), _i, C.POINTER(C.c_int32), _i, C.POINTER(C.c_int32), _vp, _i,
                                  C.POINTER(C.c_int32)]),
    "ss_batch_mt_continue_plan": (_i, [_i, C.POINTER(C.c_int32), C.POINTER(C.c_int32), C.POINTER(C.c_int32),
                                       C.POINTER(C.c_int32), _i, _i, _i, _i, _i, _i, C.POINTER(C.c_int32), C.POINTER(C.c_int32),
                                       _i64, C.POINTER(_i64)]),
    "ss_batch_mt_beam_continue": (_i, [_vp, _vp, _i, _i, _vp, C.POINTER(C.c_int32), C.POINTER(C.c_int32), C.POINTER(C.c_int32),
                                       C.POINTER(C.c_int32), _i, _f, _i, C.POINTER(C.c_int32), _i, C.POINTER(C.c_int32),
                                       C.POINTER(_f), C.POINTER(_f), _vp, _i]),
    "ss_batch_mt_beam_continue_plan": (_i, [_i, _i, C.POINTER(C.c_int32), C.POINTER(C.c_int32), C.POINTER(C.c_int32),
                                            C.POINTER(C.c_int32), _i, _i, _i, _i, _i, _i, _i, C.POINTER(C.c_int32),
                                            C.POINTER(C.c_int32), _i64, C.POINTER(_i64)]),
    "ss_batch_fbank_frames": (_i, [_vp, _vp, _i, C.POINTER(_vp), C.POINTER(C.c_int32), C.POINTER(C.c_int32), _f,
                                   C.POINTER(_vp)]),
    "ss_batch_fbank_frames_sr": (_i, [_vp, _vp, _i, C.POINTER(_vp), C.POINTER(C.c_int32), C.POINTER(C.c_int32), C.POINTER(C.c_int32),
                                      C.POINTER(_vp), C.POINTER(C.c_int32), C.POINTER(C.c_int32), C.POINTER(C.c_int32), _f,
                                      C.POINTER(_vp)]),
    "ss_fbank_sr_rows": (_i, [_i64, _i, _i, _i, C.POINTER(C.c_int32), C.POINTER(C.c_int32)]),
    "ss_batch_t2u_units": (_i, [_vp, _vp, _i, _vp, _i, C.POINTER(C.c_int32), _i, _i, _vp, _vp, _vp]),
    "ss_batch_vocoder_forward": (_i, [_vp, _vp, _i, _vp, C.POINTER(C.c_int32), _i, _vp, _vp, _i64, _vp,
                                      C.POINTER(_i64), C.POINTER(_i64)]),
    "ss_batch_t2u_units_pad": (_i, [_vp, _vp, _i, _vp, _i, C.POINTER(C.c_int32), C.POINTER(C.c_int32), _i, _i, _vp, _vp, _vp]),
    "ss_batch_mt_features": (_i, [_vp, _vp, _i, _vp, C.POINTER(C.c_int32), C.POINTER(C.c_int32), C.POINTER(C.c_int32),
                                  C.POINTER(C.c_int32), _vp, _i]),
    "ss_batch_vocoder_tail": (_i, [_vp, _vp, _i, _vp, C.POINTER(C.c_int32), C.POINTER(C.c_int32), C.POINTER(C.c_int32),
                                   C.POINTER(C.c_int32), _i, _vp, _i64, C.POINTER(C.c_int32), C.POINTER(C.c_int32),
                                   C.POINTER(_i64), C.POINTER(_i64)]),
    "ss_prof_enable": (_i, [_i]),
    "ss_prof_enable_hi": (_i, [_i]),
    "ss_prof_reset": (_i, []),
    "ss_prof_read": (_i, [_i, C.POINTER(C.c_double), C.POINTER(C.c_double), C.POINTER(_i64), C.POINTER(C.c_double)]),
    "ss_prof_totals": (_i, [_i, C.POINTER(C.c_double), C.POINTER(C.c_double), C.POINTER(_i64)]),
    "ss_prof_read_issued": (_i, [_i, C.POINTER(C.c_double)]),
    "ss_prof_shape_log": (_i, [_i]),
    "ss_prof_shape_dump": (_i, [C.c_char_p, _i]),
    "ss_prof_num_classes": (_i, []),
    "ss_prof_class_name": (C.c_char_p, [_i]),
    "ss_debug_force_tile": (_i, [_i, _i, _i]),
    "ss_op_ffn_fused": (_i, [_vp, _vp, _i, _vp, _i, _vp, _vp, _vp, _vp, _vp, _vp, _f, _vp, _vp, _i, _i, _i]),
    "ss_debug_ffn": (_i, [_i, _i, _i]),
    "ss_debug_rtlin": (_i, [_i, _i]),
    "ss_debug_conv_c64": (_i, [_i]),
    "ss_debug_conv_c32": (_i, [_i]),
    "ss_debug_conv_c16": (_i, [_i]),
    "ss_debug_enc_step_launches": (_i64, []),
    "ss_debug_scratch_audit": (_i, [_vp, C.POINTER(C.c_size_t), C.POINTER(C.c_size_t)]),
    "ss_op_ln_linear": (_i, [_vp, _vp, _i, _vp, _vp, _vp, _vp, _vp, _i, _vp, _i, _i, _i, _i, _i, _f, _i]),
    "ss_debug_last_logits": (_i, [_vp, _vp, _vp, _i64, C.POINTER(_i), C.POINTER(_i)]),
    "ss_debug_sk_errors": (_i, []),
    "ss_debug_attention_split": (_i, [_i]),
    "ss_debug_attention_q16": (_i, [_i]),
    "ss_op_conv_gemm": (_i, [_vp, _vp, _i, _vp, _vp, _vp, _i, _vp, _i, _vp, _i, _i, _i, _i, _i, _i, _i, _i, _i, _i,
                             _i, _f, _i, _f, _f, _i]),
    "ss_op_conv_gemm_ex": (_i, [_vp, C.POINTER(SSOpConvArgs)]),
    "ss_op_conv_pair": (_i, [_vp, _vp, _i, _vp, _vp, _vp, _vp, _vp, _i, _vp, _i, _f, _vp, _i, _f, _i, _i, _i, _i, _i, _f, _vp, _i]),
    "ss_op_resblock_fused": (_i, [_vp, _vp, _i, _vp, _vp, _vp, _vp, _vp, _vp, _i, _vp, _i, _f, _i, _i, _i, _f, _vp, _i]),
    "ss_debug_slab": (_i, [_i, C.c_longlong]),
    "ss_op_conv_f16": (_i, [_vp, _vp, _vp, _vp, _vp, _vp, _vp, _vp, _i, _i, _i, _i, _i, _f, _i, _f, _vp, _i]),
    "ss_op_layernorm": (_i, [_vp, _vp, _i, _vp, _i, _vp, _vp, _i, _i, _f]),
    "ss_op_attention": (_i, [_vp, _vp, _i, _vp, _i, _vp, _i, _vp, _i, _i, _i, _i, _f, _i, _i, _vp, _i, _vp, _vp]),
    "ss_op_attention_ex": (_i, [_vp, C.POINTER(SSOpAttnArgs)]),
    "ss_op_attention_pool": (_i, [_vp, C.POINTER(SSOpPoolAttnArgs)]),
    "ss_debug_attention_no_mfma": (_i, [_i]),
    "ss_op_dwconv_bn_silu": (_i, [_vp, _vp, _i, _vp, _i, _vp, _i, _vp, _vp, _vp, _vp, _f, _i, _i, _i]),
    "ss_op_masked_argmax": (_i, [_vp, _vp, _i, _i, _i, _i, _i, _i, _i, _vp, _vp, _i, _i, _vp, _i]),
    "ss_op_ctc_collapse": (_i, [_vp, _vp, _i, _i, _i, _vp, _vp, _vp, _vp, _i]),
    "ss_op_dur_predict": (_i, [_vp, _vp, _vp, _i, _vp, _vp, _vp, _i]),
    "ss_op_repeat_rows": (_i, [_vp, _vp, _vp, _i, _i, _vp, _i, _vp, _i]),
    "ss_op_embed_tokens": (_i, [_vp, _vp, _vp, _vp, _f, _i, _vp, _i, _i, _i, _i, _i]),
    "ss_op_embed_tokens_rows": (_i, [_vp, _vp, _vp, _vp, _i, _f, _i, _vp, _vp, _i, _i, _i, _i]),
    "ss_op_upsample_add_pos": (_i, [_vp, _vp, _i, _i, _vp, _f, _vp, _i]),
    "ss_op_gather_rows": (_i, [_vp, _vp, _vp, _i, _vp, _i, _i]),
    "ss_op_scatter_rows": (_i, [_vp, _vp, _vp, _i, _vp, _i, _i, _i, _i]),
    "ss_op_conv_post_tanh": (_i, [_vp, _vp, _i, _i, _vp, _vp, _f, _vp, _vp, _i]),
    "ss_op_conv_post_tanh_crop": (_i, [_vp, _vp, _i, _vp, _vp, _f, _vp, _vp, _i, _i]),
    "ss_op_spkr_pre_add": (_i, [_vp, _vp, _vp, _i, _i, _vp, _vp, _i, _vp, _i, _i, _i, _i, _f]),
    "ss_op_beam_topk": (_i, [_vp, _vp, _i, _i, _i, _i, _i, _vp, _vp, _vp, _vp, _i, _i, _i, _f, _vp, _vp]),
    "ss_op_beam_merge": (_i, [_vp, C.POINTER(SSOpBeamState), _i, _i, _i, _i, _i, _i, _i, _i]),
    "ss_op_beam_prefix_score": (_i, [_vp, _vp, _i, _i, _vp, _i, _i, _f, _vp]),
    "ss_op_beam_prefix_chain": (_i, [_vp, _vp, _vp, _vp, _i, _i, _vp, _vp]),
}

_lib = None


SS_ERR_ARG = 2
SS_ERR_CAPACITY = 4
SS_ERR_SCRATCH_CAP = 5
SS_ERR_STREAM_REPEAT = 8


class StreamSpeechHipError(RuntimeError):

    def __init__(self, msg, code=None):
        super().__init__(msg)
        self.code = code


def load():
    global _lib
    if _lib is not None:
        return _lib
    if not os.path.exists(LIB_PATH):
        raise StreamSpeechHipError(
            f"{LIB_PATH} not found: build it with streamspeech_amd/csrc/build.sh "
            "(or __graft_entry__.build()).  There is no CPU fallback for the product path.")
    import torch
    lib = C.CDLL(LIB_PATH)
    for name, (res, args) in SIGNATURES.items():
        try:
            fn = getattr(lib, name)
        except AttributeError as e:
            raise StreamSpeechHipError(f"{LIB_PATH} does not export {name}") from e
        fn.restype = res
        fn.argtypes = args
    if lib.ss_abi_version() != 2:
        raise StreamSpeechHipError("ABI version mismatch")
    _lib = lib
    return lib


def check(rc: int, what: str = ""):
    if rc != 0:
        msg = load().ss_error_string(rc).decode()
        raise StreamSpeechHipError(f"{what} failed: {msg} (code {rc})", rc)
```

Before: 6347.

## Fuse vocoder resblock conv pairs into one Winograd kernel with halo recompute

Result: no change. 6380, median of 6 (+0.5%).

```diff
diff --git a/include/streamspeech_hip.h b/include/streamspeech_hip.h
--- a/include/streamspeech_hip.h
+++ b/include/streamspeech_hip.h
@@ -432,6 +432,7 @@
   int32_t same_rows;
 } ss_op_conv_args;
 int ss_op_conv_gemm_ex(void* stream, const ss_op_conv_args* a);
+int ss_op_conv_wino_pair(void* stream, const ss_op_conv_args* c1, const ss_op_conv_args* c2);
 int ss_op_conv_pair(void* stream, const float* dA, int lda, const float* dW1, const float* db1, const float* dW2, const float* db2,
                     float* dC, int ldc, const float* dR2, int ldr2, float div, float* dC2, int ldc2, float c2_slope, int C, int taps,
                     int dil, int M, int in_len, float slope, const int32_t* d_segs, int nseg);
diff --git a/streamspeech_amd/csrc/conv_c64w.hip b/streamspeech_amd/csrc/conv_c64w.hip
--- a/streamspeech_amd/csrc/conv_c64w.hip
+++ b/streamspeech_amd/csrc/conv_c64w.hip
@@ -10,7 +10,7 @@
 #define CW_TIMING 0
 #endif
 #if CW_TIMING
-__device__ unsigned long long g_cw_dbg[1024 * 8];
+__device__ unsigned long long g_cw_dbg[1024 * 12];
 #define CW_STAMP(k) do { if (t == 0) { const unsigned long long _n = __builtin_amdgcn_s_memtime(); cw_acc[k] += _n - cw_last; cw_last = _n; } } while (0)
 #else
 #define CW_STAMP(k) do { } while (0)
@@ -51,11 +51,13 @@
   }
 }
 
-template <int DIL, int CH, int TAIL>
-__global__ __launch_bounds__(CH >= 128 ? 512 : 256, CH >= 128 ? 1 : CH == 64 ? 2 : 3) void conv_c64w_kernel(const GemmArgs p, const int groups, const int slab_rows) {
+template <int DIL, int CH, int TAIL, bool PAIR>
+__device__ __forceinline__ void cw_body(const GemmArgs& p, const GemmArgs& p2, const int groups, const int slab_rows, const int halo) {
 #if __HIP_DEVICE_COMPILE__
+  static_assert(!PAIR || CH == 64 || CH == 128, "the fused pair exists at 64 and 128 channels");
   constexpr int CS = CH == 256 ? 128 : CH;
   constexpr int KH = CH / CS;
+  constexpr int KHL = PAIR ? 2 : KH;
   constexpr int C = CH, LDA = CS + 4, CT = CH >= 64 ? 4 : CH / 16, CB = CS / 16, RING = 2 * CT, TPR = CS / 4;
   constexpr int NT = CH >= 128 ? 512 : 256, RPP = NT / TPR;
   constexpr int NP = (CW_MAXROWS + RPP - 1) / RPP, NPC = CH == 256 ? 10 : NP < 20 ? NP : 20, BME = cw_bme(DIL), NPAIR = BME / 2;
@@ -71,16 +73,20 @@
   const int r = lane & 15, g = lane >> 4;
   const int Kw = groups * 4 * C;
 
-  SlabWalk<GemmArgs> w(p, s_blk, BME);
+  const GemmArgs& pe = PAIR ? p2 : p;
+  const int out_rows = PAIR ? BME - 2 * halo : BME;
+  SlabWalk<GemmArgs> w(pe, s_blk, out_rows);
   __syncthreads();
   const int nblocks = w.nblocks();
   const float slope = p.in_act == ACT_LRELU ? p.in_slope : 1.0f;
+  [[maybe_unused]] const float slope2 = p2.in_act == ACT_LRELU ? p2.in_slope : 1.0f;
 
   const __amdgpu_buffer_rsrc_t rsW = __builtin_amdgcn_make_buffer_rsrc((void*)p.W, 0, CW_NUM_RECORDS, 0x00020000);
+  [[maybe_unused]] const __amdgpu_buffer_rsrc_t rsW2 = __builtin_amdgcn_make_buffer_rsrc((void*)p2.W, 0, CW_NUM_RECORDS, 0x00020000);
   const int vo = (r * Kw + 4 * g) * 4;
-  auto wload = [&](int idx, int cc, int ct, int kh) -> f32x4 {
+  auto wload = [&](const __amdgpu_buffer_rsrc_t rs, int idx, int cc, int ct, int kh) -> f32x4 {
     const int so = __builtin_amdgcn_readfirstlane(((col0 + ct * 16) * Kw + idx * C + kh * CS + cc * 16) * 4);
-    const u32x4 v = __builtin_amdgcn_raw_buffer_load_b128(rsW, vo, so, 0);
+    const u32x4 v = __builtin_amdgcn_raw_buffer_load_b128(rs, vo, so, 0);
     return f32x4{__uint_as_float(v[0]), __uint_as_float(v[1]), __uint_as_float(v[2]), __uint_as_float(v[3])};
   };
 
@@ -89,7 +95,7 @@
   if (blk >= nblocks) return;
   f32x4 ring[RING];
 #pragma unroll
-  for (int q = 0; q < RING; ++q) ring[q] = wload(q / CT, 0, q % CT, 0);
+  for (int q = 0; q < RING; ++q) ring[q] = wload(rsW, q / CT, 0, q % CT, 0);
 
   int toff[2];
   bool pv[2];
@@ -100,28 +106,30 @@
     const int pc = pv[i] ? pp : NPAIR - 1;
     toff[i] = 2 * DIL * (pc / DIL) + pc % DIL;
   }
+  [[maybe_unused]] int toff2[2];
+  [[maybe_unused]] bool pv2[2];
+  if constexpr (PAIR) {
+#pragma unroll
+    for (int i = 0; i < 2; ++i) {
+      const int pp = wave * 32 + i * 16 + r, np2 = out_rows / 2;
+      pv2[i] = pp < np2;
+      toff2[i] = 2 * (pv2[i] ? pp : np2 - 1) + halo - p2.pad;
+    }
+  }
 
 #if CW_TIMING
-  unsigned long long cw_acc[4] = {0, 0, 0, 0}, cw_last = __builtin_amdgcn_s_memtime(), cw_begin = cw_last, cw_blocks = 0;
+  unsigned long long cw_acc[6] = {0, 0, 0, 0, 0, 0}, cw_last = __builtin_amdgcn_s_memtime(), cw_begin = cw_last, cw_blocks = 0;
 #endif
   for (; blk < nblocks; blk += blk_stride) {
 #if CW_TIMING
     ++cw_blocks;
 #endif
-    w.locate(blk, p.in_len);
+    w.locate(blk, pe.in_len);
     const int m0 = w.m0, seg_lo = w.seg_lo, seg_hi = w.seg_hi;
-    const int m_hi = p.nseg > 0 ? seg_hi : min(seg_hi, p.M);
-    const bool edge = (m0 - p.pad < seg_lo) || (m0 - p.pad + slab_rows > seg_hi);
-    f32x4 acc[4][2][CT];
-#pragma unroll
-    for (int f = 0; f < 4; ++f)
-#pragma unroll
-      for (int i = 0; i < 2; ++i)
-#pragma unroll
-        for (int j = 0; j < CT; ++j) acc[f][i][j] = f32x4{0.f, 0.f, 0.f, 0.f};
-#pragma unroll 1
-    for (int kh = 0; kh < KH; ++kh) {
-    const int kh_wrap = kh + 1 < KH ? kh + 1 : 0;
+    const int m_hi = pe.nseg > 0 ? seg_hi : min(seg_hi, pe.M);
+    const int m1 = PAIR ? m0 - halo : m0;
+    const bool edge = (m1 - p.pad < seg_lo) || (m1 - p.pad + slab_rows > seg_hi);
+    auto stage = [&](const int kh) __attribute__((always_inline)) {
     __syncthreads();
     CW_STAMP(kh == 0 ? 3 : 1);
 #pragma unroll 1
@@ -130,7 +138,7 @@
 #pragma unroll
       for (int u = 0; u < NPC; ++u) {
         const int rho = t / TPR + RPP * (u0 + u);
-        const int gc = min(max(m0 - p.pad + rho, seg_lo), seg_hi - 1);
+        const int gc = min(max(m1 - p.pad + rho, seg_lo), seg_hi - 1);
         pre[u] = *reinterpret_cast<const f32x4*>(p.A + (size_t)gc * p.lda + kh * CS + (t % TPR) * 4);
       }
       float* dst = sA + (t / TPR + RPP * u0) * LDA + (t % TPR) * 4;
@@ -139,7 +147,7 @@
         const int rho = t / TPR + RPP * (u0 + u);
         f32x4 v = pre[u];
         if (edge) {
-          const int gin = m0 - p.pad + rho;
+          const int gin = m1 - p.pad + rho;
           const bool ok = gin >= seg_lo && gin < seg_hi;
 #pragma unroll
           for (int e = 0; e < 4; ++e) v[e] = ok ? v[e] : 0.f;
@@ -151,15 +159,70 @@
     }
     __syncthreads();
     CW_STAMP(0);
-
-    const float* pa0 = sA + toff[0] * LDA + 4 * g;
-    const float* pa1 = sA + toff[1] * LDA + 4 * g;
-    auto rd = [&](const float* base, int j, int cc) -> f32x4 { return *reinterpret_cast<const f32x4*>(base + j * DIL * LDA + cc * 16); };
+    };
+    if constexpr (PAIR) stage(0);
+    f32x4 acc[4][2][CT];
+#pragma unroll
+    for (int f = 0; f < 4; ++f)
+#pragma unroll
+      for (int i = 0; i < 2; ++i)
+#pragma unroll
+        for (int j = 0; j < CT; ++j) acc[f][i][j] = f32x4{0.f, 0.f, 0.f, 0.f};
+#pragma unroll 1
+    for (int kh = 0; kh < KHL; ++kh) {
+    const int kh_wrap = kh + 1 < KHL ? kh + 1 : 0;
+    if constexpr (!PAIR) {
+      stage(kh);
+    } else if (kh != 0) {
+      __syncthreads();
+      int lh = lane;
+      asm volatile("" : "+v"(lh));
+      const int colh_ = col0 + (lh >> 4) * 4;
+      f32x4 b1[CT];
+#pragma unroll
+      for (int j = 0; j < CT; ++j) b1[j] = f32x4{0.f, 0.f, 0.f, 0.f};
+      if (p.bias) {
+#pragma unroll
+        for (int j = 0; j < CT; ++j) b1[j] = *reinterpret_cast<const f32x4*>(p.bias + colh_ + j * 16);
+      }
+#pragma unroll
+      for (int i = 0; i < 2; ++i) {
+        const int g0 = m1 + toff[i];
+        const bool ok0 = g0 >= seg_lo && g0 < seg_hi, ok1 = g0 + DIL >= seg_lo && g0 + DIL < seg_hi;
+        float* d0 = sA + toff[i] * LDA + colh_;
+#pragma unroll
+        for (int j = 0; j < CT; ++j) {
+          f32x4 y0 = (acc[0][i][j] + acc[1][i][j]) + acc[2][i][j];
+          f32x4 y1 = (acc[1][i][j] - acc[2][i][j]) - acc[3][i][j];
+          y0 += b1[j];
+          y1 += b1[j];
+#pragma unroll
+          for (int e = 0; e < 4; ++e) {
+            y0[e] = ok0 ? fmaxf(y0[e], y0[e] * slope2) : 0.f;
+            y1[e] = ok1 ? fmaxf(y1[e], y1[e] * slope2) : 0.f;
+          }
+          if (pv[i]) {
+            *reinterpret_cast<f32x4*>(d0 + j * 16) = y0;
+            *reinterpret_cast<f32x4*>(d0 + DIL * LDA + j * 16) = y1;
+          }
+#pragma unroll
+          for (int f = 0; f < 4; ++f) acc[f][i][j] = f32x4{0.f, 0.f, 0.f, 0.f};
+        }
+      }
+      __syncthreads();
+      CW_STAMP(4);
+    }
+    const __amdgpu_buffer_rsrc_t rs_cur = (PAIR && kh) ? rsW2 : rsW, rs_wrap = (PAIR && !kh) ? rsW2 : rsW;
+    const int khw = PAIR ? 0 : kh, khw_wrap = PAIR ? 0 : kh_wrap;
+    const int dstr = (PAIR && DIL != 1 && kh) ? LDA : DIL * LDA;
+    const float* pa0 = sA + ((PAIR && kh) ? toff2[0] : toff[0]) * LDA + 4 * g;
+    const float* pa1 = sA + ((PAIR && kh) ? toff2[1] : toff[1]) * LDA + 4 * g;
+    auto rd = [&](const float* base, int j, int cc) -> f32x4 { return *reinterpret_cast<const f32x4*>(base + j * dstr + cc * 16); };
     auto xform = [&](int op, const f32x4 a, const f32x4 b) -> f32x4 { return op == 1 ? a + b : op == 0 ? a : a - b; };
     f32x4 xa[2];
     xa[0] = xform(-1, rd(pa0, 0, 0), rd(pa0, 2, 0));
     xa[1] = xform(-1, rd(pa1, 0, 0), rd(pa1, 2, 0));
-    auto group = [&](auto KIND, const int grp, const int kind_next, const float* pn0, const float* pn1, const int grp_next, const int kh_next) __attribute__((always_inline)) {
+    auto group = [&](auto KIND, const int grp, const int kind_next, const float* pn0, const float* pn1, const int grp_next, const int kh_next, const __amdgpu_buffer_rsrc_t rs_next) __attribute__((always_inline)) {
       constexpr int K = decltype(KIND)::value, NC = cw_nc(K), NS = CB * NC;
       static_assert(NS % 2 == 0 && NS >= 2, "ring slots keep their parity across groups");
 #pragma unroll
@@ -172,8 +235,8 @@
           na1 = rd(pa1, cw_ja(K, nn), ccn); nb1 = rd(pa1, cw_jb(K, nn), ccn);
         } else {
           const int jb = kind_next == 0 ? 2 : 1;
-          na0 = rd(pn0, 0, 0); nb0 = *reinterpret_cast<const f32x4*>(pn0 + jb * (DIL * LDA));
-          na1 = rd(pn1, 0, 0); nb1 = *reinterpret_cast<const f32x4*>(pn1 + jb * (DIL * LDA));
+          na0 = rd(pn0, 0, 0); nb0 = *reinterpret_cast<const f32x4*>(pn0 + jb * dstr);
+          na1 = rd(pn1, 0, 0); nb1 = *reinterpret_cast<const f32x4*>(pn1 + jb * dstr);
         }
         f32x4 wf[CT];
 #pragma unroll
@@ -181,8 +244,8 @@
           const int q = ss * CT + j;
           wf[j] = ring[q % RING];
           const int s2 = ss + 2;
-          if (s2 < NS) ring[q % RING] = wload(grp * 4 + cw_slot(K, s2 % NC), s2 / NC, j, kh);
-          else ring[q % RING] = wload(grp_next * 4 + (s2 == NS ? 0 : (kind_next == 1 ? 3 : 1)), 0, j, kh_next);
+          if (s2 < NS) ring[q % RING] = wload(rs_cur, grp * 4 + cw_slot(K, s2 % NC), s2 / NC, j, khw);
+          else ring[q % RING] = wload(rs_next, grp_next * 4 + (s2 == NS ? 0 : (kind_next == 1 ? 3 : 1)), 0, j, kh_next);
         }
 #pragma unroll
         for (int e = 0; e < 4; ++e)
@@ -206,15 +269,16 @@
 #pragma unroll 1
     for (int grp = 0; grp < groups_full; ++grp) {
       const bool more = grp + 1 < groups;
-      const float* pn0 = more ? pa0 + 3 * DIL * LDA : pa0;
-      const float* pn1 = more ? pa1 + 3 * DIL * LDA : pa1;
-      group(std::integral_constant<int, 0>{}, grp, (more && grp + 1 == groups_full) ? tail : 0, pn0, pn1, more ? grp + 1 : 0, more ? kh : kh_wrap);
+      const float* pn0 = more ? pa0 + 3 * dstr : pa0;
+      const float* pn1 = more ? pa1 + 3 * dstr : pa1;
+      group(std::integral_constant<int, 0>{}, grp, (more && grp + 1 == groups_full) ? tail : 0, pn0, pn1, more ? grp + 1 : 0, more ? khw : khw_wrap,
+            (PAIR && !more) ? rs_wrap : rs_cur);
       pa0 = pn0;
       pa1 = pn1;
     }
-    if constexpr (TAIL == 1) group(std::integral_constant<int, 1>{}, groups_full, 0, pa0, pa1, 0, kh_wrap);
-    if constexpr (TAIL == 2) group(std::integral_constant<int, 2>{}, groups_full, 0, pa0, pa1, 0, kh_wrap);
-    CW_STAMP(1);
+    if constexpr (TAIL == 1) group(std::integral_constant<int, 1>{}, groups_full, 0, pa0, pa1, 0, khw_wrap, rs_wrap);
+    if constexpr (TAIL == 2) group(std::integral_constant<int, 2>{}, groups_full, 0, pa0, pa1, 0, khw_wrap, rs_wrap);
+    CW_STAMP((PAIR && kh) ? 5 : 1);
     }
 
     int le = lane;
@@ -230,44 +294,56 @@
         y[(i * 2) * CT + j] = (acc[0][i][j] + acc[1][i][j]) + acc[2][i][j];
         y[(i * 2 + 1) * CT + j] = (acc[1][i][j] - acc[2][i][j]) - acc[3][i][j];
       }
-      mrow[i * 2] = m0 + toff[i];
-      mrow[i * 2 + 1] = m0 + toff[i] + DIL;
+      const int et = PAIR ? toff2[i] - (halo - p2.pad) : toff[i];
+      mrow[i * 2] = m0 + et;
+      mrow[i * 2 + 1] = m0 + et + (PAIR ? 1 : DIL);
     }
 #pragma unroll
     for (int n = 0; n < 4 * CT; ++n) asm volatile("" : "+v"(y[n]));
     f32x4 bb[CT];
 #pragma unroll
     for (int j = 0; j < CT; ++j) bb[j] = f32x4{0.f, 0.f, 0.f, 0.f};
-    if (p.bias) {
-#pragma unroll
-      for (int j = 0; j < CT; ++j) bb[j] = *reinterpret_cast<const f32x4*>(p.bias + cole + j * 16);
-    }
-    slab_epi_batch(p, y, bb, [&](int q, int n) -> size_t {
-      return (size_t)min(mrow[n / CT], m_hi - 1) * (q == 0 ? p.ldr : p.ldr2) + cole + (n % CT) * 16;
+    if (pe.bias) {
+#pragma unroll
+      for (int j = 0; j < CT; ++j) bb[j] = *reinterpret_cast<const f32x4*>(pe.bias + cole + j * 16);
+    }
+    slab_epi_batch(pe, y, bb, [&](int q, int n) -> size_t {
+      return (size_t)min(mrow[n / CT], m_hi - 1) * (q == 0 ? pe.ldr : pe.ldr2) + cole + (n % CT) * 16;
     });
 #pragma unroll
     for (int q = 0; q < 4; ++q) {
-      if (pv[q / 2] && mrow[q] < m_hi) {
-#pragma unroll
-        for (int j = 0; j < CT; ++j) slab_epi_store<CH >= 128>(p, mrow[q], cole + j * 16, y[q * CT + j]);
+      if ((PAIR ? pv2[q / 2] : pv[q / 2]) && mrow[q] < m_hi) {
+#pragma unroll
+        for (int j = 0; j < CT; ++j) slab_epi_store<CH >= 128>(pe, mrow[q], cole + j * 16, y[q * CT + j]);
       }
     }
     CW_STAMP(2);
   }
 #if CW_TIMING
   if (t == 0) {
-    unsigned long long* d = g_cw_dbg + (size_t)(blockIdx.x & 1023) * 8;
-    d[0] = cw_acc[0]; d[1] = cw_acc[1]; d[2] = cw_acc[2]; d[3] = cw_acc[3]; d[4] = cw_blocks; d[5] = cw_begin; d[6] = __builtin_amdgcn_s_memtime(); d[7] = 1;
-  }
-#endif
-#endif
+    unsigned long long* d = g_cw_dbg + (size_t)(blockIdx.x & 1023) * 12;
+#pragma unroll
+    for (int k = 0; k < 6; ++k) d[k] = cw_acc[k];
+    d[6] = cw_blocks; d[7] = cw_begin; d[8] = __builtin_amdgcn_s_memtime(); d[9] = 1;
+  }
+#endif
+#endif
+}
+
+template <int DIL, int CH, int TAIL>
+__global__ __launch_bounds__(CH >= 128 ? 512 : 256, CH >= 128 ? 1 : CH == 64 ? 2 : 3) void conv_c64w_kernel(const GemmArgs p, const int groups, const int slab_rows) {
+  cw_body<DIL, CH, TAIL, false>(p, p, groups, slab_rows, 0);
+}
+template <int DIL, int CH, int TAIL>
+__global__ __launch_bounds__(CH >= 128 ? 512 : 256, CH >= 128 ? 1 : 2) void conv_cw_pair_kernel(const GemmArgs p, const GemmArgs p2, const int groups, const int slab_rows, const int halo) {
+  cw_body<DIL, CH, TAIL, true>(p, p2, groups, slab_rows, halo);
 }
 
 #if CW_TIMING
 extern "C" int ss_debug_cw_timing(unsigned long long* h_out, int cap_wgs) {
   const int n = cap_wgs < 1024 ? cap_wgs : 1024;
-  if (hipMemcpyFromSymbol(h_out, HIP_SYMBOL(g_cw_dbg), (size_t)n * 8 * sizeof(unsigned long long)) != hipSuccess) return -1;
-  static unsigned long long zeros[1024 * 8];
+  if (hipMemcpyFromSymbol(h_out, HIP_SYMBOL(g_cw_dbg), (size_t)n * 12 * sizeof(unsigned long long)) != hipSuccess) return -1;
+  static unsigned long long zeros[1024 * 12];
   (void)hipMemcpyToSymbol(HIP_SYMBOL(g_cw_dbg), zeros, sizeof(zeros));
   return n;
 }
@@ -357,6 +433,79 @@
   if (!conv_c64_eligible(a) || !conv_c64w_eligible(a)) return SS_ERR_ARG;
   return launch_cw<64>(a, stream);
 }
+
+static int cw_pair_halo(int taps, int dil) { const int pad2 = (taps - 1) / 2; return (pad2 + 2 * dil - 1) / (2 * dil) * (2 * dil); }
+int conv_cw_pair_out_rows(int taps, int dil) { return cw_bme(dil) - 2 * cw_pair_halo(taps, dil); }
+static int cw_pair_bit(int taps, int dil) { return 3 * (taps <= 3 ? 0 : taps <= 7 ? 1 : 2) + (dil == 1 ? 0 : dil == 3 ? 1 : 2); }
+
+bool conv_cw_pair_eligible(const GemmArgs& c1, const GemmArgs& c2, int ch) {
+  if (ch == 64) {
+    if (!conv_c64_eligible(c1) || !conv_c64w_eligible(c1) || !conv_c64_eligible(c2) || !conv_c64w_eligible(c2)) return false;
+  } else if (ch == 128) {
+    if (!conv_wide_winograd_eligible(c1, 128) || !conv_wide_winograd_eligible(c2, 128)) return false;
+  } else {
+    return false;
+  }
+  if (c1.taps != c2.taps || c1.taps % 2 == 0 || c2.dil != 1 || c1.Wf16 || c2.Wf16) return false;
+  if (c1.M != c2.M || c1.in_len != c2.in_len || c1.nseg != c2.nseg || c1.segs != c2.segs) return false;
+  if (c1.act != ACT_NONE || c1.alpha != 1.0f || c1.R || c1.R2 || c1.div > 0.f || c1.C2) return false;
+  if (c1.A == c2.C || c1.A == c2.C2) return false;
+  return conv_cw_pair_out_rows(c1.taps, c1.dil) >= 2 * c1.dil;
+}
+bool conv_cw_pair_wanted(const GemmArgs& c1, const GemmArgs& c2, int ch) {
+  const Dispatch& d = disp();
+  if (!(ch == 64 ? d.c64_pair_on : ch == 128 ? d.c128_pair_on : 0)) return false;
+  if (!(((ch == 64 ? d.c64_pair_mask : d.c128_pair_mask) >> cw_pair_bit(c1.taps, c1.dil)) & 1)) return false;
+  return conv_cw_pair_eligible(c1, c2, ch);
+}
+
+template <int DIL, int CH, int TAIL>
+static int launch_cw_pair_t(GemmArgs a, GemmArgs a2, hipStream_t stream) {
+  const int groups = cw_groups(a);
+  const int slab_rows = cw_bme(DIL) + 3 * groups * DIL;
+  const int halo = cw_pair_halo(a.taps, DIL), out_rows = cw_bme(DIL) - 2 * halo;
+  const size_t lds = cw_lds(a, CH);
+  SS_MAX_LDS_ONCE((&conv_cw_pair_kernel<DIL, CH, TAIL>), CH >= 128 ? 160 * 1024 : 96 * 1024);
+  SkWorkspace* st = nullptr;
+  int rc = sk_workspace_acquire(stream, &st);
+  if (rc != SS_OK) return rc;
+  const int grid = slab_grid(CH >= 128 ? 1 : 2, st->cus, a2.M, out_rows, a2.nseg);
+  GemmArgs book = a2;
+  book.algo_flops = (a.algo_flops > 0 ? a.algo_flops : 2.0 * a.M * a.N * a.taps * a.Cin) + (a2.algo_flops > 0 ? a2.algo_flops : 2.0 * a2.M * a2.N * a2.taps * a2.Cin);
+  book.algo_bytes = 4.0 * ((double)a.N * a.taps * a.Cin + (double)a2.N * a2.taps * a2.Cin + (a.bias ? a.N : 0) + (a2.bias ? a2.N : 0) +
+                           (double)a.in_len * a.Cin + (double)a2.M * a2.N * (1 + (a2.R ? 1 : 0) + (a2.R2 ? 1 : 0)));
+  ProfRec rec{}; bool prof = false;
+  rc = prof_begin(book, stream, CH == 64 ? PROF_CONV_C64W : PROF_CONV_C128W, rec, prof);
+  if (rc != SS_OK) return rc;
+  a.W = a.Wwino;
+  a2.W = a2.Wwino;
+  hipLaunchKernelGGL((conv_cw_pair_kernel<DIL, CH, TAIL>), dim3(grid), dim3(CH >= 128 ? 512 : 256), lds, stream, a, a2, groups, slab_rows, halo);
+  SS_LAUNCH_CHECK();
+  return prof_end(stream, rec, prof);
+}
+
+template <int CH>
+static int launch_cw_pair(const GemmArgs& a, const GemmArgs& a2, hipStream_t stream) {
+  const int key = a.dil * 10 + a.taps % 3;
+  switch (key) {
+    case 10: return launch_cw_pair_t<1, CH, 0>(a, a2, stream);
+    case 11: return launch_cw_pair_t<1, CH, 1>(a, a2, stream);
+    case 12: return launch_cw_pair_t<1, CH, 2>(a, a2, stream);
+    case 30: return launch_cw_pair_t<3, CH, 0>(a, a2, stream);
+    case 31: return launch_cw_pair_t<3, CH, 1>(a, a2, stream);
+    case 32: return launch_cw_pair_t<3, CH, 2>(a, a2, stream);
+    case 50: return launch_cw_pair_t<5, CH, 0>(a, a2, stream);
+    case 51: return launch_cw_pair_t<5, CH, 1>(a, a2, stream);
+    case 52: return launch_cw_pair_t<5, CH, 2>(a, a2, stream);
+    default: return SS_ERR_ARG;
+  }
+}
+
+int launch_conv_cw_pair(const GemmArgs& c1, const GemmArgs& c2, hipStream_t stream) {
+  const int ch = c1.N;
+  if ((ch != 64 && ch != 128) || !conv_cw_pair_eligible(c1, c2, ch)) return SS_ERR_ARG;
+  return ch == 64 ? launch_cw_pair<64>(c1, c2, stream) : launch_cw_pair<128>(c1, c2, stream);
+}
 void conv_c32w_debug(int enable) { if (enable >= 0) dispatch_edit([enable](Dispatch& d) { d.c32w_on = enable ? 1 : 0; }); }
 bool conv_c32w_enabled() { return disp().c32w_on != 0; }
 bool conv_c32w_eligible(const GemmArgs& a) {
diff --git a/streamspeech_amd/csrc/debug_ops.hip b/streamspeech_amd/csrc/debug_ops.hip
--- a/streamspeech_amd/csrc/debug_ops.hip
+++ b/streamspeech_amd/csrc/debug_ops.hip
@@ -40,6 +40,28 @@
   a.segs = x->segs; a.nseg = x->nseg; a.max_seg_out = x->max_seg_out; a.same_rows = x->same_rows;
   if (a.W && a.N > 0 && a.taps > 0) RET(op_bind_wino(a, stream));
   return launch_conv_gemm(a, (hipStream_t)stream);
+}
+extern "C" int ss_op_conv_wino_pair(void* stream, const ss_op_conv_args* x1, const ss_op_conv_args* x2) {
+  if (!x1 || !x2 || !x1->W || !x2->W) return SS_ERR_ARG;
+  static thread_local std::map<std::pair<hipStream_t, int>, DevBuf> wino_tmps;
+  GemmArgs g[2];
+  for (int i = 0; i < 2; ++i) {
+    const ss_op_conv_args* x = i ? x2 : x1;
+    GemmArgs& a = g[i];
+    a.A = x->A; a.W = x->W; a.bias = x->bias; a.R = x->R; a.R2 = x->R2; a.C = x->C; a.C2 = x->C2;
+    a.lda = x->lda; a.ldc = x->ldc; a.ldr = x->ldr; a.ldr2 = x->ldr2; a.ldc2 = x->ldc2;
+    a.M = x->M; a.N = x->N; a.Cin = x->Cin; a.taps = x->taps; a.dil = x->dil; a.stride = x->stride; a.pad = x->pad;
+    a.in_len = x->in_len; a.chunk = x->chunk;
+    a.in_act = x->in_act; a.in_slope = x->in_slope; a.act = x->act; a.act_slope = x->act_slope; a.alpha = x->alpha; a.div = x->div;
+    a.c2_slope = x->c2_slope; a.glu = x->glu;
+    a.segs = x->segs; a.nseg = x->nseg; a.max_seg_out = x->max_seg_out; a.same_rows = x->same_rows;
+    if ((a.N != 64 && a.N != 128) || a.Cin != a.N || a.taps < 3 || a.taps > 64) return SS_ERR_ARG;
+    DevBuf& tmp = wino_tmps[std::make_pair((hipStream_t)stream, i)];
+    RET(tmp.ensure((size_t)a.N * ((a.taps + 2) / 3) * 4 * a.N * sizeof(float)));
+    RET(launch_wino_pack(a.W, tmp.f(), a.N, a.taps, (hipStream_t)stream));
+    a.Wwino = tmp.f();
+  }
+  return launch_conv_cw_pair(g[0], g[1], (hipStream_t)stream);
 }
 extern "C" int ss_op_conv_pair(void* stream, const float* dA, int lda, const float* dW1, const float* db1, const float* dW2,
                                const float* db2, float* dC, int ldc, const float* dR2, int ldr2, float div, float* dC2, int ldc2,
diff --git a/streamspeech_amd/csrc/dispatch.hpp b/streamspeech_amd/csrc/dispatch.hpp
--- a/streamspeech_amd/csrc/dispatch.hpp
+++ b/streamspeech_amd/csrc/dispatch.hpp
@@ -12,6 +12,8 @@
   int c64w_on = 1, c128w_on = 1, c256w_on = 1, c32w_on = 1;
   int c64w_min_k = 3;
   long long c128w_min_rows = 65536, c256w_min_rows = 32768;
+  int c64_pair_on = 1, c128_pair_on = 1;
+  int c64_pair_mask = 0x01f, c128_pair_mask = 0x0db;
   int slab_grid_cap = 0;
   int sk_groups = 0;
   int ffn_force_g = 0;
diff --git a/streamspeech_amd/csrc/gemm.hip b/streamspeech_amd/csrc/gemm.hip
--- a/streamspeech_amd/csrc/gemm.hip
+++ b/streamspeech_amd/csrc/gemm.hip
@@ -816,6 +816,9 @@
   d.c64_min_rows = L("SS_CONV_C64_MIN_ROWS", d.c64_min_rows);
   d.c64w_on = I("SS_CONV_C64_WINOGRAD", 1); d.c128w_on = I("SS_CONV_C128_WINOGRAD", 1); d.c256w_on = I("SS_CONV_C256_WINOGRAD", 1);
   d.c32w_on = I("SS_CONV_C32_WINOGRAD", 1); d.c64w_min_k = I("SS_CONV_C64_WINOGRAD_MIN_K", 3);
+  d.c64_pair_on = I("SS_CONV_C64_PAIR", d.c64_pair_on); d.c128_pair_on = I("SS_CONV_C128_PAIR", d.c128_pair_on);
+  auto X = [](const char* k, int dflt) { const char* e = getenv(k); return e ? (int)strtol(e, nullptr, 0) : dflt; };
+  d.c64_pair_mask = X("SS_CONV_C64_PAIR_MASK", d.c64_pair_mask); d.c128_pair_mask = X("SS_CONV_C128_PAIR_MASK", d.c128_pair_mask);
   d.c128w_min_rows = L("SS_CONV_C128_MIN_ROWS", d.c128w_min_rows); d.c256w_min_rows = L("SS_CONV_C256_MIN_ROWS", d.c256w_min_rows);
   if (getenv("SS_FFN_WM")) { d.ffn_wm = I("SS_FFN_WM", 3); d.ffn_wm_forced = 1; }
   d.ffn_fusion = I("SS_NO_FFN_FUSION", 0) ? 0 : 1; d.ffn_min_rows = I("SS_FFN_MIN_ROWS", d.ffn_min_rows);
diff --git a/streamspeech_amd/csrc/gemm.hpp b/streamspeech_amd/csrc/gemm.hpp
--- a/streamspeech_amd/csrc/gemm.hpp
+++ b/streamspeech_amd/csrc/gemm.hpp
@@ -152,6 +152,10 @@
 int launch_conv_c128w(const GemmArgs& a, hipStream_t stream);
 void conv_c128w_debug(int enable);
 bool conv_c128w_enabled();
+bool conv_cw_pair_eligible(const GemmArgs& c1, const GemmArgs& c2, int ch);
+bool conv_cw_pair_wanted(const GemmArgs& c1, const GemmArgs& c2, int ch);
+int conv_cw_pair_out_rows(int taps, int dil);
+int launch_conv_cw_pair(const GemmArgs& c1, const GemmArgs& c2, hipStream_t stream);
 int launch_conv_c256w(const GemmArgs& a, hipStream_t stream);
 void conv_c256w_debug(int enable);
 bool conv_c256w_enabled();
diff --git a/streamspeech_amd/csrc/vocoder.hip b/streamspeech_amd/csrc/vocoder.hip
--- a/streamspeech_amd/csrc/vocoder.hip
+++ b/streamspeech_amd/csrc/vocoder.hip
@@ -332,6 +332,7 @@
       const bool fuse = !pa && !per_conv && !disp().no_pair_fusion && kr == 3 &&
                         conv_pair_eligible(C, kr, c.resblock_dilations[j][2], C, C, gnseg, gM);
       const float* cur = b.bs;
+      const float* res = b.br;
       for (int dd = 0; dd < 3; ++dd) {
         const int idx = (i * c.n_res + j) * 3 + dd;
         if (fuse) {
@@ -343,12 +344,11 @@
           cur = out;
           continue;
         }
-        const float* rin = dd == 0 ? b.bs : b.br;
+        const float* rin = dd == 0 ? b.bs : res;
         const float* rin_act = dd == 0 ? b.bsa : b.bra;
         GemmArgs a1 = mk(pa ? rin_act : rin, C, v->rb_c1[idx], C, kr, c.resblock_dilations[j][dd], b.bt, C);
         if (pa) { a1.act = ACT_LRELU; a1.act_slope = 0.1f; }
         else { a1.in_act = ACT_LRELU; a1.in_slope = 0.1f; }
-        RET(conv(a1, scale));
         GemmArgs a2 = mk(b.bt, C, v->rb_c2[idx], C, kr, 1, dd < 2 ? b.br : b.bx, C);
         if (!pa) { a2.in_act = ACT_LRELU; a2.in_slope = 0.1f; }
         a2.R = rin;
@@ -359,7 +359,19 @@
           a2.div = (j == c.n_res - 1) ? (float)c.n_res : 0.f;
           if (pa_next && j == c.n_res - 1) a2.C2 = b.bxa;
         }
+        if (!pa && !f16 && ((c64 && C == 64) || (c128 && C == 128)) && canon_mode() == CANON_NONE && !disp().force_bm) {
+          GemmArgs g1 = a1, g2 = a2;
+          g1.M = g1.in_len = g2.M = g2.in_len = gM; g1.segs = g2.segs = gsegs; g1.nseg = g2.nseg = gnseg;
+          if (g2.C == rin) g2.C = b.br2;
+          if (conv_cw_pair_wanted(g1, g2, C)) {
+            RET(launch_conv_cw_pair(g1, g2, s));
+            res = g2.C;
+            continue;
+          }
+        }
+        RET(conv(a1, scale));
         RET(conv(a2, scale));
+        res = a2.C;
       }
     }
   }
diff --git a/streamspeech_amd/lib.py b/streamspeech_amd/lib.py
--- a/streamspeech_amd/lib.py
+++ b/streamspeech_amd/lib.py
@@ -251,6 +251,7 @@
     "ss_op_conv_gemm": (_i, [_vp, _vp, _i, _vp, _vp, _vp, _i, _vp, _i, _vp, _i, _i, _i, _i, _i, _i, _i, _i, _i, _i,
                              _i, _f, _i, _f, _f, _i]),
     "ss_op_conv_gemm_ex": (_i, [_vp, C.POINTER(SSOpConvArgs)]),
+    "ss_op_conv_wino_pair": (_i, [_vp, C.POINTER(SSOpConvArgs), C.POINTER(SSOpConvArgs)]),
     "ss_op_conv_pair": (_i, [_vp, _vp, _i, _vp, _vp, _vp, _vp, _vp, _i, _vp, _i, _f, _vp, _i, _f, _i, _i, _i, _i, _i, _f, _vp, _i]),
     "ss_op_resblock_fused": (_i, [_vp, _vp, _i, _vp, _vp, _vp, _vp, _vp, _vp, _i, _vp, _i, _f, _i, _i, _i, _f, _vp, _i]),
     "ss_debug_slab": (_i, [_i, C.c_longlong]),
```
